# Manta-Network/manta-rs

Measured on AMD Instinct MI355X. Metric: G1 MSM Mscalar/s at 2^20, higher is better.
Workload: dtype u32; 1 GPU; 2^20 BLS12-381 G1 variable-base MSM per GPU, uniform scalars resident in HBM; curve=BLS12-381, log_n=20, window_bits=17, msms_in_flight=3

## Files before the change

include/mantagpu.h:

```cpp
#ifndef MANTAGPU_H
#define MANTAGPU_H
#include <stddef.h>
#include <stdint.h>

#ifdef __cplusplus
extern "C" {
#endif

typedef enum { MG_BN254 = 0, MG_BLS12_381 = 1 } mg_curve_t;

enum {
    MG_SUCCESS = 0,
    MG_ERROR_INVALID_ARGUMENT = 1,
    MG_ERROR_HIP = 2,
    MG_ERROR_OUT_OF_MEMORY = 3,
    MG_ERROR_DOMAIN_TOO_LARGE = 4,
    MG_ERROR_STATE = 5,
    MG_ERROR_CHECKSUM = 6
};

typedef struct mg_bases mg_bases;
typedef struct mg_msm_job mg_msm_job;
typedef struct mg_ctx mg_ctx;

int mg_init(int device);
const char *mg_strerror(int status);
const char *mg_last_error(void);
int mg_device_count(int *count);
int mg_malloc(void **dptr, size_t bytes);
int mg_free(void *dptr);
int mg_memcpy_h2d(void *dptr, const void *hptr, size_t bytes);
int mg_memcpy_d2h(void *hptr, const void *dptr, size_t bytes);
int mg_device_synchronize(void);
int mg_host_alloc(void **hptr, size_t bytes);
int mg_host_free(void *hptr);
int mg_set_kernel_timing(int on);
float mg_last_accumulate_ms(void);
float mg_last_accumulate_mhz(void);
int mg_clock_probe(unsigned iters, double *memtime_mhz, double *mad_issue_per_us_per_simd, double *ms);
int mg_last_ntt_ms(float out4[4]);
int mg_last_prove_phases_ms(float out10[10]);
int mg_last_pass_host_ms(float out3[3]);
int mg_hw_queues(int out2[2]);

int mg_bases_create(mg_curve_t curve, int group, const uint64_t *affine_mont, size_t n, int on_device,
                    int precompute_window_bits, mg_bases **out);
int mg_bases_create_sharded(mg_curve_t curve, int group, const uint64_t *affine_mont, size_t n, const int *devices,
                            int n_devices, int precompute_window_bits, mg_bases **out);
int mg_bases_num_shards(const mg_bases *bases);
int mg_bases_shard(const mg_bases *bases, int shard, int *device, size_t *lo, size_t *hi);
void mg_bases_destroy(mg_bases *bases);
size_t mg_bases_device_bytes(const mg_bases *bases);
int mg_msm(const mg_bases *bases, const uint64_t *scalars_canonical, size_t n, uint64_t *out_affine_mont);
#define MG_SCALARS_MONT 1
#define MG_SCALARS_SPARSE 2
int mg_msm_launch(const mg_bases *bases, const uint64_t *d_scalars, size_t n, int scalar_flags, int window_bits,
                  mg_msm_job **job);
int mg_msm_launch_sharded(const mg_bases *bases, const uint64_t *const *d_scalars_per_shard, int scalar_flags,
                          int window_bits, mg_msm_job **job);
int mg_msm_finish(mg_msm_job *job, uint64_t *out_affine_mont);
int mg_msm_result_to_device(mg_msm_job *job, uint64_t *d_out_xyzz, void *stream);
size_t mg_xyzz_limbs(mg_curve_t curve, int group);
int mg_xyzz_sum(mg_curve_t curve, int group, const uint64_t *xyzz, size_t n, uint64_t *out_affine_mont);
int mg_points_sum(mg_curve_t curve, int group, const uint64_t *affine_mont, size_t n, uint64_t *out_affine_mont);
int mg_fixed_base_mul(mg_curve_t curve, int group, const uint64_t *base_affine_mont, const uint64_t *d_scalars,
                      size_t n, uint64_t *d_out_affine_mont);
#define MG_EC_ADD_MIXED 0
#define MG_EC_ADD 1
#define MG_EC_DOUBLE 2
#define MG_EC_MUL 3
#define MG_EC_SUB_MIXED 4
#define MG_EC_MUL_FIXED 5
int mg_ec_elementwise(mg_curve_t curve, int group, int op, const uint64_t *a_affine, const uint64_t *b, size_t n,
                      uint64_t *out_affine);
#define MG_FIELD_ADD 0
#define MG_FIELD_SUB 1
#define MG_FIELD_MUL 2
#define MG_FIELD_SQR 3
#define MG_FIELD_NEG 4
#define MG_FIELD_FROM_CANONICAL 5
#define MG_FIELD_TO_CANONICAL 6
#define MG_FIELD_INV 7
int mg_field_op(int field, int op, int repr, int lazy_a, int lazy_b, const uint64_t *a, const uint64_t *b, size_t n,
                uint64_t *out);
#define MG_FPR_MUL 0
#define MG_FPR_SQR 1
#define MG_FPR_MUL_ADD 2
#define MG_FPR_SUB2_6 3
#define MG_FPR_SUB2_12 4
int mg_fpr_raw_op(int field, int op, int coding, const uint32_t *a, const uint32_t *b, const uint32_t *c, const uint32_t *d,
                  size_t n, uint32_t *out);
int mg_fpr_column_plan(int field, int kind, uint32_t *flush, uint64_t *peak, int *cols, int *limb_bits, int *flushed_routines);
int mg_msm_digits(mg_curve_t curve, const uint64_t *scalars, size_t batch, size_t n_scalars, int scalar_flags, int window_bits,
                  int table_mode, size_t n, const uint32_t *map, size_t n_sets, size_t set_len, int compact, uint32_t *keys,
                  uint32_t *vals, uint32_t *count, uint32_t layout[4]);
int mg_sort_pairs(const uint32_t *keys, const uint32_t *vals, size_t n, int end_bit, const uint32_t *count, uint32_t lowmask,
                  uint32_t inv_from, uint32_t *keys_out, uint32_t *vals_out);
int mg_group_ntt(mg_curve_t curve, int group, const uint64_t *points_affine, unsigned log_n, int inverse, uint64_t *out_affine);
int mg_point_serialize(mg_curve_t curve, int group, const uint64_t *affine_mont, int compressed, uint8_t *out);

int mg_ntt(mg_curve_t curve, uint64_t *data_mont, unsigned log_n, int inverse, int coset);
int mg_ntt_device(mg_curve_t curve, uint64_t *d_data_mont, unsigned log_n, int inverse, int coset);

typedef struct {
    uint64_t n_vars;
    uint64_t n_inputs;
    uint64_t h_len;
    const uint64_t *alpha_g1, *beta_g1, *delta_g1;
    const uint64_t *beta_g2, *delta_g2;
    const uint64_t *a_query;
    const uint64_t *b_g1_query;
    const uint64_t *b_g2_query;
    const uint64_t *h_query;
    const uint64_t *l_query;
} mg_pk_view;

typedef struct {
    const uint32_t *row_ptr;
    const uint32_t *col;
    const uint64_t *val;
    uint64_t nnz;
} mg_csr;

typedef struct mg_pk_out {
    uint64_t *alpha_g1, *beta_g1, *delta_g1;
    uint64_t *beta_g2, *gamma_g2, *delta_g2;
    uint64_t *gamma_abc_g1;
    uint64_t *a_query, *b_g1_query, *b_g2_query, *h_query, *l_query;
} mg_pk_out;
int mg_groth16_setup(mg_curve_t curve, const mg_csr *a, const mg_csr *b, const mg_csr *c, uint64_t num_constraints,
                     uint64_t n_vars, uint64_t n_inputs, const uint64_t *toxic_mont ,
                     const uint64_t *g1_generator, const uint64_t *g2_generator, const mg_pk_out *out);

int mg_qap_columns(mg_curve_t curve, int group, size_t n_terms, const uint64_t *const *bases_affine,
                   const mg_csr *const *mats, uint64_t m, uint64_t n_cols, uint32_t entries_per_lane,
                   uint64_t *out_affine);

typedef struct {
    uint64_t n_g1, n_g2;
    const uint64_t *tau_powers_g1, *tau_powers_g2, *alpha_tau_powers_g1, *beta_tau_powers_g1, *beta_g2;
} mg_kzg_view;

int mg_mpc_initialize(mg_curve_t curve, const mg_kzg_view *powers, const mg_csr *a, const mg_csr *b, const mg_csr *c,
                      uint64_t num_constraints, uint64_t n_vars, uint64_t n_inputs, uint64_t h_len,
                      const uint64_t *g1_generator, const uint64_t *g2_generator, const mg_pk_out *out);

int mg_ctx_create(mg_curve_t curve, const mg_pk_view *pk, mg_ctx **out);
#define MG_EXCHANGE_HOST 0u
#define MG_EXCHANGE_RCCL 1u
typedef struct mg_tuning {
    uint32_t struct_size;
    int32_t graph_mode;
    int32_t graph_mode_batch;
    int32_t prove_streams;
    int32_t linear_chains;
    int32_t coalesce_inflight;
    int32_t coalesce_gather_us;
    int32_t batch_inflight;
    int32_t queue_aware;
    int32_t msm_dedicated_queues;
    int32_t window_bits_narrow;
    int32_t window_bits_wide;
    int32_t window_bits_h;
    int32_t window_bits_g2;
    int64_t full_table_bytes;
} mg_tuning;
int mg_tuning_init(mg_tuning *t);
int mg_get_tuning(mg_tuning *t);
int mg_set_tuning(const mg_tuning *t);
const char *const *mg_tuning_env_names(void);

typedef struct mg_ctx_opts {
    uint32_t struct_size;
    uint32_t exchange;
    int64_t full_table_bytes;
    const int *devices;
    int32_t n_devices;
    int32_t shard, n_shards;
    uint32_t task_mask;
    const mg_tuning *tuning;
} mg_ctx_opts;
int mg_ctx_opts_init(mg_ctx_opts *opts);
int mg_ctx_create_ex(mg_curve_t curve, const mg_pk_view *pk, const mg_ctx_opts *opts , mg_ctx **out);
int mg_ctx_create_from_bytes_ex(mg_curve_t curve, const uint8_t *bytes, size_t len, const uint8_t *checksum32,
                                const mg_ctx_opts *opts, mg_ctx **out);
int mg_ctx_create_sharded(mg_curve_t curve, const mg_pk_view *pk, const int *devices, int n_devices, mg_ctx **out);
int mg_ctx_create_from_bytes_sharded(mg_curve_t curve, const uint8_t *bytes, size_t len, const int *devices,
                                     int n_devices, mg_ctx **out);
int mg_ctx_create_shard(mg_curve_t curve, const mg_pk_view *pk, int shard, int n_shards, mg_ctx **out);
#define MG_TASK_A 1u
#define MG_TASK_B_G1 2u
#define MG_TASK_B_G2 4u
#define MG_TASK_L 8u
#define MG_TASK_H 16u
int mg_ctx_create_task(mg_curve_t curve, const mg_pk_view *pk, unsigned task_mask, mg_ctx **out);
typedef struct mg_partials_job mg_partials_job;
size_t mg_partials_slot_limbs(const mg_ctx *ctx);
int mg_groth16_partials_launch(const mg_ctx *ctx, uint64_t k, const uint64_t *z_mont, uint64_t *d_out, void *stream,
                               mg_partials_job **job);
int mg_groth16_partials_finish(mg_partials_job *job);
int mg_groth16_assemble(const mg_ctx *ctx, uint64_t k, int n_parts, const uint64_t *parts, const uint64_t *r_mont,
                        const uint64_t *s_mont, uint8_t *proofs_out);
int mg_ctx_create_from_bytes(mg_curve_t curve, const uint8_t *bytes, size_t len, mg_ctx **out);
int mg_ctx_create_from_bytes_checked(mg_curve_t curve, const uint8_t *bytes, size_t len, const uint8_t checksum[32],
                                     mg_ctx **out);
int mg_blake3(const uint8_t *data, size_t len, uint8_t out32[32]);
int mg_blake2s256(const uint8_t *data, size_t len, uint8_t out32[32]);
int mg_blake2s(const uint8_t *data, size_t len, size_t out_len, uint8_t *out);
int mg_aes256_gcm(const uint8_t key[32], const uint8_t nonce[12], const uint8_t *in, size_t len, int decrypt, uint8_t *out,
                  int *ok);
int mg_ctx_set_r1cs(mg_ctx *ctx, const mg_csr *a, const mg_csr *b, const mg_csr *c, uint64_t num_constraints);
int mg_groth16_prove(const mg_ctx *ctx, const uint64_t *z_mont, const uint64_t r_mont[4], const uint64_t s_mont[4],
                     uint8_t *proof_out);
int mg_groth16_prove_batch(const mg_ctx *ctx, uint64_t k, const uint64_t *z_mont, const uint64_t *r_mont,
                           const uint64_t *s_mont, uint8_t *proofs_out);
int mg_witness_map(const mg_ctx *ctx, const uint64_t *z_mont, uint64_t *h_out_mont);
#define MG_R1CS_SATISFIED UINT64_MAX
int mg_ctx_r1cs_check(const mg_ctx *ctx, uint64_t k, const uint64_t *z_mont, uint64_t *first_unsatisfied,
                      uint64_t *n_unsatisfied);
int mg_r1cs_check(mg_curve_t curve, const mg_csr *a, const mg_csr *b, const mg_csr *c, uint64_t num_constraints,
                  uint64_t n_vars, uint64_t k, const uint64_t *z_mont, uint64_t *first_unsatisfied, uint64_t *n_unsatisfied);
uint64_t mg_ctx_domain_size(const mg_ctx *ctx);
int mg_ctx_table_bytes(const mg_ctx *ctx, uint64_t out2[2]);
uint64_t mg_ctx_num_variables(const mg_ctx *ctx);
uint64_t mg_ctx_num_inputs(const mg_ctx *ctx);
int mg_ctx_num_shards(const mg_ctx *ctx);
void mg_ctx_destroy(mg_ctx *ctx);

typedef struct mg_vk mg_vk;
int mg_vk_create(mg_curve_t curve, const uint64_t *alpha_g1, const uint64_t *beta_g2, const uint64_t *gamma_g2,
                 const uint64_t *delta_g2, const uint64_t *gamma_abc_g1, uint64_t n_inputs, mg_vk **out);
int mg_vk_create_from_bytes(mg_curve_t curve, const uint8_t *bytes, size_t len, mg_vk **out);
size_t mg_vk_encoded_size(const mg_vk *vk);
int mg_vk_encode(const mg_vk *vk, uint8_t *out);
int mg_vk_alpha_beta(const mg_vk *vk, uint8_t *out );
uint64_t mg_vk_num_inputs(const mg_vk *vk);
void mg_vk_destroy(mg_vk *vk);
int mg_groth16_verify(const mg_vk *vk, const uint64_t *inputs_mont, const uint64_t *proof_points, int *ok);
int mg_groth16_verify_batch(const mg_vk *vk, uint64_t k, const uint64_t *inputs_mont, const uint64_t *proof_points,
                            const uint64_t *rand128, int *ok);
#define MG_VERIFY_EACH_CHUNK 1024u
int mg_pairing_check_each(mg_curve_t curve, const uint64_t *g1_affine, const uint64_t *g2_affine, size_t group_size,
                          size_t n_groups, uint8_t *ok);
int mg_groth16_verify_each(const mg_vk *vk, uint64_t k, const uint64_t *inputs_mont, const uint64_t *proof_points,
                           uint8_t *ok);
int mg_pairing_check(mg_curve_t curve, const uint64_t *g1_affine, const uint64_t *g2_affine, size_t n, int *ok);
#define MG_PAIRING_MUL12 0
#define MG_PAIRING_SQR12 1
#define MG_PAIRING_CYC_SQR12 2
#define MG_PAIRING_ELL 3
// ... 144 lines not shown
```

manta_rs_amd/api.py:

```python
from __future__ import annotations

import ctypes
import os

import numpy as np

_HERE = os.path.dirname(os.path.abspath(__file__))
LIB_PATH = os.environ.get("MANTA_LIB") or os.path.join(_HERE, "lib", "libmantagpu.so")

BN254, BLS12_381 = 0, 1
FQ_LIMBS = {BN254: 4, BLS12_381: 6}


class MantaGpuError(RuntimeError):

    def __init__(self, status, where=""):
        self.status = status
        detail = LIB.mg_last_error().decode() if status == 2 else ""
        super().__init__(f"{where}: {LIB.mg_strerror(status).decode()} ({status}) {detail}")


def _load():
    if not os.path.exists(LIB_PATH):
        raise ImportError(
            f"{LIB_PATH} not found: the MI355X HIP library is the product and there is no CPU fallback. "
            "Run `python -c 'import __graft_entry__ as g; g.build()'` (or `make -C manta_rs_amd/csrc`).")
    try:
        import torch
    except Exception:
        pass
    lib = ctypes.CDLL(LIB_PATH, mode=ctypes.RTLD_GLOBAL)
    lib.mg_strerror.restype = ctypes.c_char_p
    lib.mg_last_error.restype = ctypes.c_char_p
    lib.mg_bases_device_bytes.restype = ctypes.c_size_t
    lib.mg_ctx_domain_size.restype = ctypes.c_uint64
    lib.mg_ctx_num_variables.restype = ctypes.c_uint64
    lib.mg_ctx_num_inputs.restype = ctypes.c_uint64
    lib.mg_last_accumulate_ms.restype = ctypes.c_float
    lib.mg_last_accumulate_mhz.restype = ctypes.c_float
    lib.mg_vk_encoded_size.restype = ctypes.c_size_t
    lib.mg_vk_num_inputs.restype = ctypes.c_uint64
    lib.mg_xyzz_limbs.restype = ctypes.c_size_t
    lib.mg_partials_slot_limbs.restype = ctypes.c_size_t
    return lib


LIB = _load()
_vp = ctypes.c_void_p
_sz = ctypes.c_size_t

EXPORTS = [
    "mg_init", "mg_strerror", "mg_last_error", "mg_device_count", "mg_malloc", "mg_free", "mg_memcpy_h2d",
    "mg_memcpy_d2h", "mg_device_synchronize", "mg_host_alloc", "mg_host_free", "mg_set_kernel_timing", "mg_last_accumulate_ms", "mg_bases_create", "mg_bases_destroy", "mg_bases_device_bytes",
    "mg_msm", "mg_msm_launch", "mg_msm_finish", "mg_points_sum", "mg_fixed_base_mul", "mg_ec_elementwise", "mg_point_serialize", "mg_ntt",
    "mg_msm_digits", "mg_sort_pairs",
    "mg_ntt_device", "mg_groth16_setup", "mg_ctx_create", "mg_ctx_create_from_bytes", "mg_ctx_set_r1cs", "mg_groth16_prove", "mg_groth16_prove_batch", "mg_witness_map", "mg_ctx_domain_size", "mg_ctx_table_bytes",
    "mg_ctx_destroy", "mg_bases_create_sharded", "mg_bases_num_shards", "mg_bases_shard", "mg_msm_launch_sharded",
    "mg_ctx_create_sharded", "mg_ctx_create_from_bytes_sharded", "mg_ctx_num_variables", "mg_ctx_num_inputs",
    "mg_ctx_num_shards", "mg_field_op", "mg_vk_create", "mg_vk_create_from_bytes", "mg_vk_encoded_size", "mg_vk_encode",
    "mg_vk_alpha_beta", "mg_vk_num_inputs", "mg_vk_destroy", "mg_groth16_verify", "mg_groth16_verify_batch", "mg_pairing_check", "mg_proof_decode", "mg_group_ntt",
    "mg_msm_result_to_device", "mg_xyzz_limbs", "mg_xyzz_sum", "mg_ctx_create_shard", "mg_partials_slot_limbs",
    "mg_groth16_partials_launch", "mg_groth16_partials_finish", "mg_groth16_assemble", "mg_blake3", "mg_ctx_create_from_bytes_checked",
    "mg_last_ntt_ms", "mg_hw_queues", "mg_last_prove_phases_ms", "mg_clock_probe", "mg_last_accumulate_mhz", "mg_ctx_create_task",
    "mg_ctx_opts_init", "mg_ctx_create_ex", "mg_ctx_create_from_bytes_ex", "mg_last_pass_host_ms",
    "mg_tuning_init", "mg_get_tuning", "mg_set_tuning", "mg_tuning_env_names",
    "mg_points_decode", "mg_points_check", "mg_points_encode", "mg_proofs_decode",
    "mg_ppot_points_decode", "mg_ppot_points_encode", "mg_blake2b512",
    "mg_poseidon_create", "mg_poseidon_destroy", "mg_poseidon_permute", "mg_poseidon_hash", "mg_poseidon_hash_device",
    "mg_merkle_tree", "mg_merkle_forest_roots", "mg_merkle_forest_append",
    "mg_edwards_decode", "mg_edwards_encode", "mg_edwards_check", "mg_edwards_mul", "mg_edwards_add",
    "mg_note_cipher_create", "mg_note_cipher_destroy", "mg_notes_encrypt", "mg_notes_decrypt",
    "mg_utxo_model_create", "mg_utxo_model_destroy", "mg_utxos_mint", "mg_utxos_open", "mg_viewing_keys",
    "mg_blake2s256", "mg_schnorr_challenges", "mg_signatures_verify", "mg_signatures_sign",
    "mg_blake2s", "mg_aes256_gcm", "mg_address_partitions", "mg_merkle_shard_indices",
    "mg_light_notes_encrypt", "mg_light_notes_open", "mg_outgoing_notes_encrypt", "mg_outgoing_notes_open",
    "mg_qap_columns", "mg_mpc_initialize", "mg_fpr_raw_op", "mg_fpr_column_plan",
    "mg_pairing_check_each", "mg_groth16_verify_each", "mg_pairing_op",
    "mg_ctx_r1cs_check", "mg_r1cs_check",
]


def _chk(rc, where):
    if rc != 0:
        raise MantaGpuError(rc, where)


def _p(a):
    return None if a is None else a.ctypes.data_as(_vp)


def _u64(a):
    return np.ascontiguousarray(a, dtype=np.uint64)


def _addr(x):
    if x is None:
        return None
    if isinstance(x, ctypes.c_void_p):
        return x
    if hasattr(x, "ptr"):
        return _addr(x.ptr)
    return _vp(int(x))


def init(device=0):
    _chk(LIB.mg_init(int(device)), "mg_init")


def device_count():
    c = ctypes.c_int(0)
    _chk(LIB.mg_device_count(ctypes.byref(c)), "mg_device_count")
    return c.value


def set_kernel_timing(on):
    _chk(LIB.mg_set_kernel_timing(int(bool(on))), "mg_set_kernel_timing")


def last_accumulate_ms():
    return float(LIB.mg_last_accumulate_ms())


def last_accumulate_mhz():
    return float(LIB.mg_last_accumulate_mhz())


def clock_probe(iters=200000):
    a, b, c = ctypes.c_double(0), ctypes.c_double(0), ctypes.c_double(0)
    _chk(LIB.mg_clock_probe(ctypes.c_uint(iters), ctypes.byref(a), ctypes.byref(b), ctypes.byref(c)), "mg_clock_probe")
    return a.value, b.value, c.value


def last_ntt_ms():
    v = (ctypes.c_float * 4)()
    _chk(LIB.mg_last_ntt_ms(v), "mg_last_ntt_ms")
    return [float(x) for x in v]


def hw_queues():
    v = (ctypes.c_int * 2)()
    _chk(LIB.mg_hw_queues(v), "mg_hw_queues")
    return int(v[0]), int(v[1])


def last_prove_phases_ms():
    v = (ctypes.c_float * 10)()
    _chk(LIB.mg_last_prove_phases_ms(v), "mg_last_prove_phases_ms")
    names = ("upload_z", "witness_map", "msm_a", "msm_b_g1", "msm_b_g2", "msm_l", "msm_h", "part_a_upload_to_join", "g2_chain_upload_to_end",
             "host_assembly_after_gpu")
    return {n: round(float(x), 4) for n, x in zip(names, v)}


def last_pass_host_ms():
    v = (ctypes.c_float * 3)()
    _chk(LIB.mg_last_pass_host_ms(v), "mg_last_pass_host_ms")
    return {"enqueue": round(float(v[0]), 4), "wait_gpu": round(float(v[1]), 4), "assemble": round(float(v[2]), 4)}


def synchronize():
    _chk(LIB.mg_device_synchronize(), "mg_device_synchronize")


class PinnedArray:

    def __init__(self, shape, dtype=np.uint64):
        self.nbytes = int(np.prod(shape)) * np.dtype(dtype).itemsize
        ptr = _vp()
        _chk(LIB.mg_host_alloc(ctypes.byref(ptr), _sz(self.nbytes)), "mg_host_alloc")
        self._ptr = ptr
        buf = (ctypes.c_uint8 * self.nbytes).from_address(ptr.value)
        self.array = np.frombuffer(buf, dtype=dtype).reshape(shape)

    @classmethod
    def like(cls, arr):
        arr = np.ascontiguousarray(arr)
        p = cls(arr.shape, arr.dtype)
        p.array[...] = arr
        return p

    def free(self):
        if self._ptr is not None and self._ptr.value:
            self.array = None
            LIB.mg_host_free(self._ptr)
            self._ptr = None

    def __del__(self):
        try:
            self.free()
        except Exception:
            pass


class DeviceBuffer:

    def __init__(self, nbytes):
        self.nbytes = int(nbytes)
        ptr = _vp()
        _chk(LIB.mg_malloc(ctypes.byref(ptr), _sz(self.nbytes)), "mg_malloc")
        self.ptr = ptr

    @classmethod
    def from_numpy(cls, arr):
        arr = np.ascontiguousarray(arr)
        b = cls(arr.nbytes)
        _chk(LIB.mg_memcpy_h2d(b.ptr, _p(arr), _sz(arr.nbytes)), "mg_memcpy_h2d")
        return b

    def to_numpy(self, dtype=np.uint64, shape=None):
# ... 142 lines not shown

def aes256_gcm_decrypt(key: bytes, nonce: bytes, sealed: bytes):
    key, nonce, sealed = bytes(key), bytes(nonce), bytes(sealed)
    if len(key) != 32 or len(nonce) != 12 or len(sealed) < 16:
        raise ValueError("aes256_gcm: a 32-byte key, a 12-byte nonce and at least the 16 bytes of a tag")
    out = ctypes.create_string_buffer(max(1, len(sealed) - 16))
    ok = ctypes.c_int(0)
    _chk(LIB.mg_aes256_gcm(key, nonce, sealed, _sz(len(sealed)), 1, out, ctypes.byref(ok)), "mg_aes256_gcm")
    return out.raw[:len(sealed) - 16], bool(ok.value)


def xyzz_limbs(curve, group) -> int:
    return int(LIB.mg_xyzz_limbs(curve, group))


def xyzz_sum(curve, group, xyzz) -> np.ndarray:
    pts = _u64(xyzz).reshape(-1, xyzz_limbs(curve, group))
    out = np.zeros(affine_limbs(curve, group), dtype=np.uint64)
    _chk(LIB.mg_xyzz_sum(curve, group, _p(pts), _sz(pts.shape[0]), _p(out)), "mg_xyzz_sum")
    return out


def points_sum(curve, group, points):
    pts = _u64(points)
    out = np.zeros(affine_limbs(curve, group), dtype=np.uint64)
    _chk(LIB.mg_points_sum(curve, group, _p(pts), _sz(pts.shape[0]), _p(out)), "mg_points_sum")
    return out


def fixed_base_mul(curve, group, base, d_scalars: DeviceBuffer, n) -> DeviceBuffer:
    out = DeviceBuffer(n * affine_limbs(curve, group) * 8)
    _chk(LIB.mg_fixed_base_mul(curve, group, _p(_u64(base)), d_scalars.ptr, _sz(n), out.ptr), "mg_fixed_base_mul")
    return out


EC_ADD_MIXED, EC_ADD, EC_DOUBLE, EC_MUL, EC_SUB_MIXED, EC_MUL_FIXED = range(6)


def group_ntt(curve, group, points, inverse=False) -> np.ndarray:
    pts = _u64(points)
    n = pts.shape[0]
    lg = n.bit_length() - 1
    assert 1 << lg == n and pts.shape[1] == affine_limbs(curve, group)
    out = np.zeros_like(pts)
    _chk(LIB.mg_group_ntt(curve, group, _p(pts), lg, int(bool(inverse)), _p(out)), "mg_group_ntt")
    return out


def ec_elementwise(curve, group, op, a, b=None) -> np.ndarray:
    a = _u64(a)
    n = a.shape[0]
    out = np.zeros_like(a)
    bb = _p(_u64(b)) if b is not None else None
    _chk(LIB.mg_ec_elementwise(curve, group, op, _p(a), bb, _sz(n), _p(out)), "mg_ec_elementwise")
    return out


FIELD_IDS = {"bn254_fr": 0, "bn254_fq": 1, "bls381_fr": 2, "bls381_fq": 3}
FIELD_OPS = {"add": 0, "sub": 1, "mul": 2, "sqr": 3, "neg": 4, "from_canonical": 5, "to_canonical": 6, "inv": 7}


def field_op(field, op, a, b=None, repr=0, lazy_a=0, lazy_b=0) -> np.ndarray:
    a = _u64(a)
    nl = 6 if field == "bls381_fq" else 4
    assert a.ndim == 2 and a.shape[1] == nl, a.shape
    out = np.zeros_like(a)
    bb = None if b is None else _u64(b)
    assert bb is None or bb.shape == a.shape
    _chk(LIB.mg_field_op(FIELD_IDS[field], FIELD_OPS[op], int(repr), int(lazy_a), int(lazy_b), _p(a), _p(bb), _sz(a.shape[0]),
                         _p(out)), "mg_field_op")
    return out


FPR_OPS = {"mul": 0, "sqr": 1, "mul_add": 2, "sub2_6": 3, "sub2_12": 4}
FPR_LIMBS = {"bn254_fr": (9, 29), "bn254_fq": (9, 29), "bls381_fr": (9, 29), "bls381_fq": (13, 30)}


def fpr_raw_op(field, op, a, b=None, c=None, d=None, chain=False) -> np.ndarray:
    K = FPR_LIMBS[field][0]
    arrs = [None if x is None else np.ascontiguousarray(x, dtype=np.uint32) for x in (a, b, c, d)]
    need = {"sqr": 1, "mul": 2, "sub2_6": 3, "sub2_12": 3, "mul_add": 4}[op]
    for x in arrs[:need]:
        assert x is not None and x.ndim == 2 and x.shape == arrs[0].shape and x.shape[1] == K, (op, None if x is None else x.shape)
    out = np.zeros_like(arrs[0])
    _chk(LIB.mg_fpr_raw_op(FIELD_IDS[field], FPR_OPS[op], int(bool(chain)), _p(arrs[0]), _p(arrs[1]), _p(arrs[2]), _p(arrs[3]),
                           _sz(arrs[0].shape[0]), _p(out)), "mg_fpr_raw_op")
    return out


PAIRING_OPS = {"mul12": 0, "sqr12": 1, "cyc_sqr12": 2, "ell": 3, "frob12_1": 4, "frob12_2": 5, "frob12_3": 6, "conj12": 7, "inv12": 8,
               "exp_by_x": 9, "final_exp": 10, "fq_inv_euclid": 11, "fq_half": 12, "fq2_mul": 13, "fq2_mul_xi": 14, "fq_lincomb": 15}
PAIRING_LINCOMB_OPERANDS = 10


def pairing_op(curve, op, a, b=None, coeffs=None) -> np.ndarray:
    N = 2 * FQ_LIMBS[curve]
    a = np.ascontiguousarray(a, dtype=np.uint32)
    n = a.shape[0]
    if op == "fq_lincomb":
        assert a.shape == (n, PAIRING_LINCOMB_OPERANDS, N), a.shape
        coeffs = np.ascontiguousarray(coeffs, dtype=np.int16)
        assert coeffs.shape == (n, PAIRING_LINCOMB_OPERANDS), coeffs.shape
        out = np.zeros((n, N), dtype=np.uint32)
    else:
        wa = {"fq_inv_euclid": N, "fq_half": N, "fq2_mul": 2 * N, "fq2_mul_xi": 2 * N}.get(op, 12 * N)
        assert a.shape == (n, wa), (op, a.shape)
        coeffs = None
        out = np.zeros_like(a)
    wb = {"mul12": 12 * N, "ell": 6 * N, "fq2_mul": 2 * N}.get(op)
    if wb is not None:
        b = np.ascontiguousarray(b, dtype=np.uint32)
        assert b.shape == (n, wb), (op, b.shape)
    else:
        b = None
    _chk(LIB.mg_pairing_op(curve, PAIRING_OPS[op], _p(a), _p(b), _p(coeffs), _sz(n), _p(out)), "mg_pairing_op")
    return out


def fpr_column_plan(field, kind) -> dict:
    flush, peak = np.zeros(25, dtype=np.uint32), np.zeros(25, dtype=np.uint64)
    cols, lb, fr = ctypes.c_int(0), ctypes.c_int(0), ctypes.c_int(0)
    _chk(LIB.mg_fpr_column_plan(FIELD_IDS[field], FPR_OPS[kind], _p(flush), _p(peak), ctypes.byref(cols), ctypes.byref(lb),
                                ctypes.byref(fr)), "mg_fpr_column_plan")
    return dict(flush=[int(x) for x in flush[:cols.value]], peak=[int(x) for x in peak[:cols.value]], limb_bits=lb.value,
                flushed_routines=bool(fr.value))


def _u32_buffer(a, n, name):
    out = np.zeros(n, dtype=np.uint32) if a is None else np.array(a, dtype=np.uint32).reshape(-1)
    assert out.shape == (n,), "%s: %d elements, expected %d" % (name, out.size, n)
    return out


def msm_digits(curve, scalars, c, n, mont=False, table_mode=0, map=None, n_sets=1, set_len=None, compact=False, keys=None, vals=None):
    sc = _u64(scalars)
    if sc.ndim == 2:
        sc = sc[None]
    assert sc.ndim == 3 and sc.shape[2] == 4, sc.shape
    batch, n_scalars = sc.shape[0], sc.shape[1]
    bits = 254 if curve == BN254 else 255
    W = (bits + c - 1) // c if c > 0 else 0
    size = batch * W * n
    k, v = _u32_buffer(keys, size, "keys"), _u32_buffer(vals, size, "vals")
    mp = None if map is None else np.ascontiguousarray(map, dtype=np.uint32)
    assert mp is None or mp.shape == (n,), mp.shape
    count = ctypes.c_uint32(0)
    layout = (ctypes.c_uint32 * 4)()
    _chk(LIB.mg_msm_digits(curve, _p(sc), _sz(batch), _sz(n_scalars), int(bool(mont)), int(c), int(table_mode), _sz(n), _p(mp), _sz(n_sets),
                           _sz(n if set_len is None else set_len), int(bool(compact)), _p(k), _p(v), ctypes.byref(count) if compact else None,
                           layout), "mg_msm_digits")
    assert layout[0] == W
    return dict(W=int(layout[0]), B=int(layout[1]), seg_keys=int(layout[2]), invalid=int(layout[3]), keys=k, vals=v,
                count=int(count.value) if compact else None)


def sort_pairs(keys, vals, end_bit, count=None, lowmask=0xFFFFFFFF, inv_from=0xFFFFFFFF, keys_out=None, vals_out=None):
    k = np.ascontiguousarray(keys, dtype=np.uint32).reshape(-1)
    v = np.ascontiguousarray(vals, dtype=np.uint32).reshape(-1)
    n = k.shape[0]
    assert v.shape == (n,)
    ko, vo = _u32_buffer(keys_out, n, "keys_out"), _u32_buffer(vals_out, n, "vals_out")
    cnt = None if count is None else ctypes.byref(ctypes.c_uint32(count))
    _chk(LIB.mg_sort_pairs(_p(k), _p(v), _sz(n), int(end_bit), cnt, ctypes.c_uint32(lowmask), ctypes.c_uint32(inv_from), _p(ko), _p(vo)),
         "mg_sort_pairs")
    return ko, vo


def point_serialize(curve, group, point, compressed=True):
    nb = FQ_LIMBS[curve] * 8 * (2 if group == 2 else 1) * (1 if compressed else 2)
    out = ctypes.create_string_buffer(nb)
    _chk(LIB.mg_point_serialize(curve, group, _p(_u64(point)), int(compressed), out), "mg_point_serialize")
    return out.raw


class Radix2EvaluationDomain:

    def __init__(self, curve, size):
        self.curve = curve
        self.log_size = max(0, (int(size) - 1).bit_length())
        self.size = 1 << self.log_size

    def _run(self, data, inverse, coset):
        d = np.array(data, dtype=np.uint64, copy=True)
        assert d.shape == (self.size, 4)
        _chk(LIB.mg_ntt(self.curve, _p(d), self.log_size, int(inverse), int(coset)), "mg_ntt")
        return d

    def fft(self, data):
        return self._run(data, False, False)

    def ifft(self, data):
        return self._run(data, True, False)

    def coset_fft(self, data):
        return self._run(data, False, True)

    def coset_ifft(self, data):
        return self._run(data, True, True)

    def fft_device(self, dbuf: DeviceBuffer, inverse=False, coset=False):
        _chk(LIB.mg_ntt_device(self.curve, dbuf.ptr, self.log_size, int(inverse), int(coset)), "mg_ntt_device")


class _PkView(ctypes.Structure):
    _fields_ = [("n_vars", ctypes.c_uint64), ("n_inputs", ctypes.c_uint64), ("h_len", ctypes.c_uint64)] + [
        (k, _vp) for k in ("alpha_g1", "beta_g1", "delta_g1", "beta_g2", "delta_g2", "a_query", "b_g1_query",
                           "b_g2_query", "h_query", "l_query")]


class _Csr(ctypes.Structure):
    _fields_ = [("row_ptr", _vp), ("col", _vp), ("val", _vp), ("nnz", ctypes.c_uint64)]


class R1CS:

    def __init__(self, curve, A, B, C, num_constraints, num_instance, z):
        self.curve, self.A, self.B, self.C = curve, A, B, C
        self.num_constraints, self.num_instance = int(num_constraints), int(num_instance)
        self.z = _u64(z)

    @classmethod
    def from_circuit(cls, c):
        return cls(c.curve, c.A, c.B, c.C, c.m, c.P, c.z)

    def which_is_unsatisfied(self):
        first, _ = r1cs_check(self.curve, self.A, self.B, self.C, self.num_constraints, self.z.size // 4, self.z)
        return None if first[0] < 0 else int(first[0])

    def is_satisfied(self) -> bool:
        return self.which_is_unsatisfied() is None


class _PkOut(ctypes.Structure):
    _fields_ = [(n, _vp) for n in ("alpha_g1", "beta_g1", "delta_g1", "beta_g2", "gamma_g2", "delta_g2", "gamma_abc_g1",
                                   "a_query", "b_g1_query", "b_g2_query", "h_query", "l_query")]


class ProvingKey:
    pass


def groth16_setup(r1cs: "R1CS", n_vars, toxic_mont, g1_generator, g2_generator) -> ProvingKey:
    curve, m, P, V = r1cs.curve, r1cs.num_constraints, r1cs.num_instance, int(n_vars)
    D = 1
    while D < m + P:
        D <<= 1
    w1, w2 = affine_limbs(curve, 1), affine_limbs(curve, 2)
    pk = ProvingKey()
    pk.curve, pk.V, pk.P, pk.D, pk.h_len = curve, V, P, D, D - 1
    shapes = {"alpha_g1": (1, w1), "beta_g1": (1, w1), "delta_g1": (1, w1), "beta_g2": (1, w2), "gamma_g2": (1, w2),
              "delta_g2": (1, w2), "gamma_abc_g1": (P, w1), "a_query": (V, w1), "b_g1_query": (V, w1),
              "b_g2_query": (V, w2), "h_query": (D - 1, w1), "l_query": (V - P, w1)}
    for k, sh in shapes.items():
        setattr(pk, k, np.zeros(sh, dtype=np.uint64))
    out = _PkOut(*[_p(getattr(pk, k)) for k, _ in _PkOut._fields_])
    ms = []
    for M in (r1cs.A, r1cs.B, r1cs.C):
        rp = np.ascontiguousarray(M.row_ptr, dtype=np.uint32)
        col = np.ascontiguousarray(M.col, dtype=np.uint32)
        val = _u64(M.val)
        ms.append((rp, col, val, _Csr(_p(rp), _p(col), _p(val), len(col))))
    tox = _u64(toxic_mont).reshape(5, 4)
    _chk(LIB.mg_groth16_setup(curve, ctypes.byref(ms[0][3]), ctypes.byref(ms[1][3]), ctypes.byref(ms[2][3]),
                              ctypes.c_uint64(m), ctypes.c_uint64(V), ctypes.c_uint64(P), _p(tox), _p(_u64(g1_generator)),
                              _p(_u64(g2_generator)), ctypes.byref(out)), "mg_groth16_setup")
    return pk


def _csr(M):
    rp = np.ascontiguousarray(M.row_ptr, dtype=np.uint32)
    col = np.ascontiguousarray(M.col, dtype=np.uint32)
    val = _u64(M.val)
    return (rp, col, val), _Csr(_p(rp), _p(col), _p(val), len(col))


R1CS_SATISFIED = (1 << 64) - 1


def _r1cs_verdicts(first, count):
    return np.where(first == np.uint64(R1CS_SATISFIED), np.int64(-1), first.astype(np.int64)), count.astype(np.int64)


def r1cs_check(curve, A, B, C, m, n_vars, zs):
    zs = _u64(zs)
    n_vars = int(n_vars)
    if n_vars > 0 and zs.size % (n_vars * 4):
        raise ValueError(f"assignments hold {zs.size} u64 words, no multiple of n_vars x 4 = {n_vars * 4}")
    k = zs.size // (n_vars * 4) if n_vars > 0 else 0
    keep = [_csr(M) for M in (A, B, C)]
    first, count = np.zeros(k, dtype=np.uint64), np.zeros(k, dtype=np.uint64)
    _chk(LIB.mg_r1cs_check(curve, ctypes.byref(keep[0][1]), ctypes.byref(keep[1][1]), ctypes.byref(keep[2][1]),
                           ctypes.c_uint64(int(m)), ctypes.c_uint64(n_vars), ctypes.c_uint64(k), _p(zs), _p(first), _p(count)),
         "mg_r1cs_check")
    return _r1cs_verdicts(first, count)


def qap_columns(curve, group, bases, mats, n_cols, entries_per_lane=0) -> np.ndarray:
    bases = [_u64(b) for b in bases]
    if len(bases) != len(mats):
        raise ValueError("qap_columns: one basis per matrix")
    m = len(mats[0].row_ptr) - 1 if mats else 0
    for b, M in zip(bases, mats):
        if b.ndim != 2 or b.shape != (m, affine_limbs(curve, group)) or len(M.row_ptr) != m + 1:
            raise ValueError("qap_columns: every basis is [m, limbs] and every matrix has m rows")
    keep = [_csr(M) for M in mats]
    bp = (ctypes.c_void_p * max(len(bases), 1))(*[b.ctypes.data for b in bases])
# ... 936 lines not shown
```

manta_rs_amd/csrc/capi.cpp:

```cpp
#include "../../include/mantagpu.h"
#include "engine.h"
#include "staging.h"
#include "tuning.h"
#include <cstddef>
#include "prover.h"
#include "verify.h"
#include "edwards.h"
#include "utxo.h"
#include "schnorr.h"
#include "light_note.h"
#include <cstring>
#include <new>
#include <vector>

using namespace mg;

struct BasesShard {
    GroupEngine *eng;
    BaseSet *bs;
    int device;
    size_t lo, hi;
};
struct mg_bases {
    std::vector<BasesShard> sh;
// ... 270 lines not shown
        hipSetDevice(j.device);
        int rc2 = j.eng->msm_finish(j.ws, &hp);
        if (rc2) j.eng->msm_abandon(j.ws);
        else e0->hp_add(&total, &hp);
        if (!rc) rc = rc2;
        j.eng->ws_release(j.ws);
        if (j.d_tmp) hipFree(j.d_tmp);
    }
    if (!rc && out_affine && e0) e0->hp_to_affine(&total, (u32 *)out_affine);
    delete job;
    return rc;
    MG_CATCH
}
MG_API int mg_msm_result_to_device(mg_msm_job *job, uint64_t *d_out_xyzz, void *stream) {
    MG_TRY
    if (!job || job->sh.size() != 1 || !d_out_xyzz) return MG_ERROR_INVALID_ARGUMENT;
    JobShard &j = job->sh[0];
    DeviceGuard guard;
    MG_HIP(hipSetDevice(j.device));
    int rc = j.eng->msm_fold_device(j.ws, (u32 *)d_out_xyzz, (size_t)j.eng->xyzz_words());
    if (rc) return rc;
    hipStream_t ms = msm_stream_of(j.ws);
    MG_HIP(hipEventRecord(j.ws->done, ms));
    if ((hipStream_t)stream != ms) MG_HIP(hipStreamWaitEvent((hipStream_t)stream, j.ws->done, 0));
    return MG_SUCCESS;
    MG_CATCH
}
MG_API size_t mg_xyzz_limbs(mg_curve_t curve, int group) {
    GroupEngine *e = get_engine((int)curve, group);
    return e ? (size_t)e->xyzz_words() / 2 : 0;
}
MG_API int mg_xyzz_sum(mg_curve_t curve, int group, const uint64_t *xyzz, size_t n, uint64_t *out_affine) {
    MG_TRY
    GroupEngine *e = get_engine((int)curve, group);
    if (!e || !xyzz || !out_affine) return MG_ERROR_INVALID_ARGUMENT;
    HostPoint acc, t;
    e->hp_set_inf(&acc);
    for (size_t i = 0; i < n; ++i) {
        e->hp_from_xyzz(&t, (const u32 *)xyzz + i * (size_t)e->xyzz_words());
        e->hp_add(&acc, &t);
    }
    e->hp_to_affine(&acc, (u32 *)out_affine);
    return MG_SUCCESS;
    MG_CATCH
}
MG_API int mg_msm(const mg_bases *b, const uint64_t *scalars, size_t n, uint64_t *out_affine) {
    MG_TRY
    if (!b || !scalars || !out_affine || b->sh.empty()) return MG_ERROR_INVALID_ARGUMENT;
    if (n > b->n) n = b->n;
    if (n == 0) {
        std::memset(out_affine, 0, (size_t)b->sh[0].eng->affine_words() * 4);
        return MG_SUCCESS;
    }
    mg_msm_job *job = nullptr;
    int rc = launch_shards(b, nullptr, scalars, n, 0, 0, &job);
    if (!rc) rc = mg_msm_finish(job, out_affine);
    return rc;
    MG_CATCH
}
MG_API int mg_points_sum(mg_curve_t curve, int group, const uint64_t *affine, size_t n, uint64_t *out_affine) {
    MG_TRY
    GroupEngine *e = get_engine((int)curve, group);
    if (!e || !affine || !out_affine) return MG_ERROR_INVALID_ARGUMENT;
    HostPoint acc, t;
    e->hp_set_inf(&acc);
    const u32 *w = (const u32 *)affine;
    for (size_t i = 0; i < n; ++i) {
        e->hp_from_affine(&t, w + i * (size_t)e->affine_words());
        e->hp_add(&acc, &t);
    }
    e->hp_to_affine(&acc, (u32 *)out_affine);
    return MG_SUCCESS;
    MG_CATCH
}
MG_API int mg_fixed_base_mul(mg_curve_t curve, int group, const uint64_t *base_affine, const uint64_t *d_scalars,
                             size_t n, uint64_t *d_out_affine) {
    MG_TRY
    GroupEngine *e = get_engine((int)curve, group);
    if (!e || !base_affine || !d_scalars || !d_out_affine || n == 0) return MG_ERROR_INVALID_ARGUMENT;
    return e->fixed_base_mul((const u32 *)base_affine, (const u32 *)d_scalars, n, (u32 *)d_out_affine, nullptr);
    MG_CATCH
}
MG_API int mg_ec_elementwise(mg_curve_t curve, int group, int op, const uint64_t *a_affine, const uint64_t *b,
                             size_t n, uint64_t *out_affine) {
    MG_TRY
    GroupEngine *e = get_engine((int)curve, group);
    if (!e) return MG_ERROR_INVALID_ARGUMENT;
    return e->ec_elementwise(op, (const u32 *)a_affine, (const u32 *)b, n, (u32 *)out_affine);
    MG_CATCH
}
MG_API int mg_group_ntt(mg_curve_t curve, int group, const uint64_t *points_affine, unsigned log_n, int inverse,
                        uint64_t *out_affine) {
    MG_TRY
    GroupEngine *e = get_engine((int)curve, group);
    FrEngine *fr = get_ntt_engine((int)curve);
    if (!e || !fr || !points_affine || !out_affine) return MG_ERROR_INVALID_ARGUMENT;
    const u32 *tw = nullptr;
    u64 ninv[4];
    int rc = fr->domain_twiddles(log_n, inverse != 0, &tw, ninv);
    if (rc) return rc;
    return e->group_ntt((const u32 *)points_affine, log_n, tw, inverse ? (const u32 *)ninv : nullptr, (u32 *)out_affine);
    MG_CATCH
}
MG_API int mg_point_serialize(mg_curve_t curve, int group, const uint64_t *affine, int compressed, uint8_t *out) {
    MG_TRY
    GroupEngine *e = get_engine((int)curve, group);
    if (!e || !affine || !out) return MG_ERROR_INVALID_ARGUMENT;
    HostPoint p;
    e->hp_from_affine(&p, (const u32 *)affine);
    e->hp_serialize(&p, out, compressed != 0);
    return MG_SUCCESS;
    MG_CATCH
}

namespace mg {
int field_op(int field, int op, int repr, int lazy_a, int lazy_b, const u32 *a, const u32 *b, size_t n, u32 *out);
}
MG_API int mg_field_op(int field, int op, int repr, int lazy_a, int lazy_b, const uint64_t *a, const uint64_t *b, size_t n,
                       uint64_t *out) {
    MG_TRY
    return field_op(field, op, repr, lazy_a, lazy_b, (const u32 *)a, (const u32 *)b, n, (u32 *)out);
    MG_CATCH
}

namespace mg {
int fpr_raw_op(int field, int op, int coding, const u32 *a, const u32 *b, const u32 *c, const u32 *d, size_t n, u32 *out);
int fpr_column_plan_host(int field, int kind, u32 *flush, u64 *peak, int *cols, int *limb_bits, int *flushed_routines);
}
MG_API int mg_fpr_raw_op(int field, int op, int coding, const uint32_t *a, const uint32_t *b, const uint32_t *c, const uint32_t *d, size_t n,
                         uint32_t *out) {
    MG_TRY
    return fpr_raw_op(field, op, coding, a, b, c, d, n, out);
    MG_CATCH
}
MG_API int mg_fpr_column_plan(int field, int kind, uint32_t *flush, uint64_t *peak, int *cols, int *limb_bits, int *flushed_routines) {
    MG_TRY
    return fpr_column_plan_host(field, kind, flush, peak, cols, limb_bits, flushed_routines);
    MG_CATCH
}

MG_API int mg_msm_digits(mg_curve_t curve, const uint64_t *scalars, size_t batch, size_t n_scalars, int scalar_flags, int window_bits,
                         int table_mode, size_t n, const uint32_t *map, size_t n_sets, size_t set_len, int compact, uint32_t *keys,
                         uint32_t *vals, uint32_t *count, uint32_t layout[4]) {
    MG_TRY
    GroupEngine *e = get_engine((int)curve, 1);
    const size_t lim = (size_t)1 << 31;
    if (!e || batch >= lim || n_scalars >= lim || n >= lim || n_sets >= lim || set_len >= lim || (scalar_flags & ~MG_SCALARS_MONT))
        return MG_ERROR_INVALID_ARGUMENT;
    const MsmDigitsCall c{(const u32 *)scalars, (u32)batch, (u32)n_scalars, (scalar_flags & MG_SCALARS_MONT) ? SCALARS_MONT : SCALARS_CANONICAL,
                          window_bits, table_mode, (u32)n, map, (u32)n_sets, (u32)set_len, compact != 0, keys, vals, count, layout};
    return e->msm_digits(c);
    MG_CATCH
}
MG_API int mg_sort_pairs(const uint32_t *keys, const uint32_t *vals, size_t n, int end_bit, const uint32_t *count, uint32_t lowmask,
                         uint32_t inv_from, uint32_t *keys_out, uint32_t *vals_out) {
    MG_TRY
    if (!keys || !vals || !keys_out || !vals_out || end_bit < 1 || end_bit > 32 || n >= ((size_t)1 << 32) || (count && *count > n))
        return MG_ERROR_INVALID_ARGUMENT;
    if (n == 0) return MG_SUCCESS;
    hipStream_t s = setup_stream();
    if (!s) return MG_ERROR_OUT_OF_MEMORY;
    const size_t pb = n * 4, tb = sort_pairs_temp_bytes(n);
    DevBlock m;
    if (const int rc = m.alloc({pb, pb, pb, pb, tb, count ? 4u : 0u}, "mg_sort_pairs")) return rc;
    const void *const src[5] = {keys, vals, keys_out, vals_out, count};
    hipError_t e = hipSuccess;
    for (int i = 0; i < 5 && e == hipSuccess; ++i)
        if (src[i]) e = hipMemcpyAsync(m.dev(i < 4 ? i : 5), src[i], i < 4 ? pb : 4, hipMemcpyHostToDevice, s);
    int rc = MG_OK;
    if (e == hipSuccess)
        rc = sort_pairs(m.dev<u32>(0), m.dev<u32>(2), m.dev<u32>(1), m.dev<u32>(3), n, end_bit, m.dev(4), tb, s, m.dev<u32>(5), lowmask, inv_from);
    if (e == hipSuccess && !rc) e = hipMemcpyAsync(keys_out, m.dev(2), pb, hipMemcpyDeviceToHost, s);
    if (e == hipSuccess && !rc) e = hipMemcpyAsync(vals_out, m.dev(3), pb, hipMemcpyDeviceToHost, s);
    const hipError_t e2 = hipStreamSynchronize(s);
    if (e == hipSuccess) e = e2;
    return rc ? rc : e == hipSuccess ? MG_SUCCESS : hip_status(e, "mg_sort_pairs");
    MG_CATCH
}

MG_API int mg_ntt_device(mg_curve_t curve, uint64_t *d_data, unsigned log_n, int inverse, int coset) {
    MG_TRY
    if (!d_data) return MG_ERROR_INVALID_ARGUMENT;
    NttEngine *n = get_ntt_engine((int)curve);
    if (!n) return MG_ERROR_INVALID_ARGUMENT;
    int rc = n->transform((u32 *)d_data, log_n, inverse != 0, coset != 0, setup_stream());
    if (rc) return rc;
    MG_HIP(setup_sync());
    return MG_SUCCESS;
    MG_CATCH
}
MG_API int mg_ntt(mg_curve_t curve, uint64_t *data, unsigned log_n, int inverse, int coset) {
    MG_TRY
    if (!data || log_n > 32) return MG_ERROR_INVALID_ARGUMENT;
    const size_t bytes = ((size_t)1 << log_n) * 32;
    DevBlock m;
    int rc = m.alloc({bytes}, "mg_ntt");
    if (rc) return rc;
    void *d = m.dev(0);
    if (memcpy_sync(d, data, bytes, hipMemcpyHostToDevice) != hipSuccess) rc = MG_ERROR_HIP;
    if (!rc) rc = mg_ntt_device(curve, (uint64_t *)d, log_n, inverse, coset);
    if (!rc && memcpy_sync(data, d, bytes, hipMemcpyDeviceToHost) != hipSuccess) rc = MG_ERROR_HIP;
    return rc;
    MG_CATCH
}

struct mg_ctx {
    Prover *p;
};
MG_API int mg_ctx_create(mg_curve_t curve, const mg_pk_view *pk, mg_ctx **out) {
    MG_TRY
    if (!pk || !out) return MG_ERROR_INVALID_ARGUMENT;
    Prover *p = nullptr;
    int rc = prover_create((int)curve, pk, &p);
    if (rc) return rc;
    *out = new mg_ctx{p};
    return MG_SUCCESS;
    MG_CATCH
}
MG_API int mg_ctx_create_sharded(mg_curve_t curve, const mg_pk_view *pk, const int *devices, int n_devices, mg_ctx **out) {
    MG_TRY
    if (!pk || !out || !devices) return MG_ERROR_INVALID_ARGUMENT;
    Prover *p = nullptr;
    int rc = prover_create_sharded((int)curve, pk, devices, n_devices, &p);
    if (rc) return rc;
    *out = new mg_ctx{p};
    return MG_SUCCESS;
    MG_CATCH
}
MG_API int mg_ctx_create_shard(mg_curve_t curve, const mg_pk_view *pk, int shard, int n_shards, mg_ctx **out) {
    MG_TRY
    if (!out || shard < 0 || n_shards < 1) return MG_ERROR_INVALID_ARGUMENT;
    Prover *p = nullptr;
    int rc = prover_create_shard((int)curve, pk, (u32)shard, (u32)n_shards, &p);
    if (rc) return rc;
    *out = new mg_ctx{p};
    return MG_SUCCESS;
    MG_CATCH
}
MG_API int mg_ctx_create_task(mg_curve_t curve, const mg_pk_view *pk, unsigned task_mask, mg_ctx **out) {
    MG_TRY
    if (!out) return MG_ERROR_INVALID_ARGUMENT;
    Prover *p = nullptr;
    int rc = prover_create_task((int)curve, pk, (u32)task_mask, &p);
    if (rc) return rc;
    *out = new mg_ctx{p};
    return MG_SUCCESS;
    MG_CATCH
}
static_assert(sizeof(mg_tuning) == sizeof(Tuning) && offsetof(mg_tuning, full_table_bytes) == offsetof(Tuning, full_table_bytes) &&
                  offsetof(mg_tuning, window_bits_g2) == offsetof(Tuning, window_bits_g2),
              "mg_tuning (mantagpu.h) and mg::Tuning (tuning.h) are the same struct");
static int tuning_from_abi(const mg_tuning *in, Tuning &t) {
    if (!in || in->struct_size < 8 || in->struct_size > 4096) return MG_ERROR_INVALID_ARGUMENT;
    t = tuning();
    std::memcpy(&t, in, std::min<size_t>(in->struct_size, sizeof(t)));
    return normalize_tuning(t) == MG_OK ? MG_SUCCESS : MG_ERROR_INVALID_ARGUMENT;
}
MG_API int mg_tuning_init(mg_tuning *t) {
    if (!t) return MG_ERROR_INVALID_ARGUMENT;
    const Tuning d = tuning_defaults();
    std::memcpy(t, &d, sizeof(d));
    return MG_SUCCESS;
}
MG_API int mg_get_tuning(mg_tuning *t) {
    MG_TRY
    if (!t) return MG_ERROR_INVALID_ARGUMENT;
    const Tuning d = tuning();
    std::memcpy(t, &d, sizeof(d));
    return MG_SUCCESS;
    MG_CATCH
}
MG_API int mg_set_tuning(const mg_tuning *t) {
    MG_TRY
    Tuning v;
    const int rc = tuning_from_abi(t, v);
    if (rc) return rc;
    return set_tuning(v) == MG_OK ? MG_SUCCESS : MG_ERROR_INVALID_ARGUMENT;
    MG_CATCH
}
MG_API const char *const *mg_tuning_env_names(void) { return tuning_env_names(); }
static int opts_from_abi(const mg_ctx_opts *in, ProverOptions &o, Tuning &tn) {
    if (!in) return MG_SUCCESS;
    mg_ctx_opts t;
    mg_ctx_opts_init(&t);
    if (in->struct_size < 8 || in->struct_size > 4096) return MG_ERROR_INVALID_ARGUMENT;
    std::memcpy(&t, in, std::min<size_t>(in->struct_size, sizeof(t)));
    if (t.n_devices < 0 || (t.n_devices > 0 && !t.devices) || t.shard < 0 || t.n_shards < 0) return MG_ERROR_INVALID_ARGUMENT;
    o.devices = t.n_devices > 0 ? t.devices : nullptr;
    o.n_devices = t.n_devices;
    o.shard = (u32)t.shard;
    o.n_shards = t.n_shards > 0 ? (u32)t.n_shards : 1;
    o.task_mask = t.task_mask ? t.task_mask : 0x1f;
    o.full_table_bytes = t.full_table_bytes;
    o.exchange = (int)t.exchange;
    if (t.tuning) {
        const int rc = tuning_from_abi(t.tuning, tn);
        if (rc) return rc;
        o.tuning = &tn;
    }
    return MG_SUCCESS;
}
MG_API int mg_ctx_opts_init(mg_ctx_opts *o) {
    if (!o) return MG_ERROR_INVALID_ARGUMENT;
    std::memset(o, 0, sizeof(*o));
    o->struct_size = (uint32_t)sizeof(*o);
    o->exchange = MG_EXCHANGE_HOST;
// ... 575 lines not shown
```

manta_rs_amd/csrc/engine.h:

```cpp
#pragma once
#include <hip/hip_runtime.h>
#include "status.h"
#include <shared_mutex>
#include <atomic>
#include <cstddef>
#include <cstdint>
#include <mutex>
#include <vector>

namespace mg {

typedef uint32_t u32;
typedef uint64_t u64;

#ifdef MG_NO_PRIO
#define MG_PRIO_HIGH() ((void)0)
#else
#define MG_PRIO_HIGH() __builtin_amdgcn_s_setprio(3)
#endif
#define MG_PRIO_FOR(F) MG_PRIO_HIGH()

void set_last_hip_error(hipError_t e, const char *expr, const char *file, int line);
inline int hip_status(hipError_t e, const char *what, const char *file = __builtin_FILE(), int line = __builtin_LINE()) {
    set_last_hip_error(e, what, file, line);
    return e == hipErrorOutOfMemory ? MG_ERR_OOM : MG_ERR_HIP;
}
#define MG_HIP(expr)                                                                                              \
    do {                                                                                                          \
        hipError_t e_ = (expr);                                                                                   \
        if (e_ != hipSuccess) return mg::hip_status(e_, #expr);                                                   \
    } while (0)
void set_last_error_text(const char *text);
void set_kernel_timing(bool on);
bool kernel_timing();
struct LastTimes {
    float accumulate_ms = 0.f;
    float accumulate_mhz = 0.f;
    float ntt_ms[4] = {};
    float pass_host_ms[3] = {};
    float prove_ms[10] = {};
};
LastTimes &last_times();
constexpr int MAX_DEVICES = 16;
int current_device();
std::shared_mutex &capture_mutex();
struct HeavyOp {
    HeavyOp();
    ~HeavyOp();
    HeavyOp(const HeavyOp &) = delete;
    HeavyOp &operator=(const HeavyOp &) = delete;
};
hipStream_t setup_stream();
inline hipError_t memcpy_sync(void *dst, const void *src, size_t bytes, hipMemcpyKind kind) {
    hipStream_t s = setup_stream();
    if (!s) return hipErrorOutOfMemory;
    const hipError_t e = hipMemcpyAsync(dst, src, bytes, kind, s);
    return e == hipSuccess ? hipStreamSynchronize(s) : e;
}
inline hipError_t setup_sync() {
    hipStream_t s = setup_stream();
    return s ? hipStreamSynchronize(s) : hipErrorOutOfMemory;
}
inline int sync_status(hipStream_t s, hipError_t e, const char *what, const char *file = __builtin_FILE(), int line = __builtin_LINE()) {
    const hipError_t e2 = hipStreamSynchronize(s);
    if (e == hipSuccess) e = e2;
    return e == hipSuccess ? MG_OK : hip_status(e, what, file, line);
}
hipStream_t stream_pool_get();
void stream_pool_put(hipStream_t s);
hipStream_t stream_pool_get_normal();
void stream_pool_put_normal(hipStream_t s);
struct GraphClient {
    GraphClient();
    ~GraphClient();
    GraphClient(const GraphClient &) = delete;
    GraphClient &operator=(const GraphClient &) = delete;
};
int graph_clients_alive();
hipStream_t stream_pool_get_dedicated();
void stream_pool_put_dedicated(hipStream_t s);
struct StreamSet {
    hipStream_t main = nullptr, g2 = nullptr, z3 = nullptr;
    int id = -1, dev = 0;
    bool z3_high = false;
};
bool stream_sets_ready();
int stream_queue_counts(int *normal, int *high);
bool stream_set_acquire(StreamSet &s, bool z3_high);
void stream_set_release(StreamSet &s);
int streams_share_queue(hipStream_t a, hipStream_t b, unsigned *mem, unsigned *token_counter);
const char *last_error_string();

struct DeviceScope {
    int prev = 0;
    bool switched = false;
    explicit DeviceScope(int dev) {
        if (hipGetDevice(&prev) == hipSuccess && prev != dev) switched = hipSetDevice(dev) == hipSuccess;
    }
    ~DeviceScope() {
        if (switched) hipSetDevice(prev);
    }
    DeviceScope(const DeviceScope &) = delete;
    DeviceScope &operator=(const DeviceScope &) = delete;
};

struct DeviceGuard {
    int prev = 0;
    DeviceGuard() { hipGetDevice(&prev); }
    ~DeviceGuard() { hipSetDevice(prev); }
    DeviceGuard(const DeviceGuard &) = delete;
    DeviceGuard &operator=(const DeviceGuard &) = delete;
};

struct DevBuf {
    void *p = nullptr;
    size_t cap = 0;
    int reserve(size_t bytes);
    void release();
    template <class T> T *as() const { return (T *)p; }
};

enum { SCALARS_CANONICAL = 0, SCALARS_MONT = 1, SCALARS_WORK = 2 };

struct MsmPlan {
    int c = 0;
    int W = 0;
    u32 B = 0;
    int Wb = 0;
    bool precomp = false;
    bool full = false;
    u32 L = 0;
};

struct BaseSet {
    int curve = 0, group = 1;
    int device = 0;
    size_t n = 0;
    size_t n_orig = 0;
    u32 *d_map = nullptr;
    u32 *d_pts = nullptr;
    int pre_c = 0, pre_W = 0;
    bool full = false;
    u32 n_sets = 1;
    size_t set_len = 0;
    static constexpr u32 MAX_SETS = 4;
    u32 set_first[MAX_SETS + 1] = {};
    size_t bytes = 0;
};

enum MsmTailKind : u32 { TAIL_WINDOW_SUMS = 0, TAIL_X_SUMS = 1, TAIL_TWO_LEVELS = 2 };
struct MsmTail {
    static constexpr int MAX_EXTRA = 8;
    MsmTailKind kind = TAIL_WINDOW_SUMS;
    u32 T1 = 0, nP = 0, segs = 0;
    u32 tail_shift = 0, n_extra = 0, extra_shift[MAX_EXTRA] = {};
    size_t extra_off_pts = 0;
    const u32 *d_tail = nullptr;
};

struct MsmWorkspace {
    DevBuf keys_in, keys_out, vals_in, vals_out, sort_tmp, buckets, pkeys[2], ppts[2], redA, redS, misc;
    DevBuf count;
    DevBuf front, extra;
    DevBuf folded;
    unsigned long long *h_clk = nullptr;
    DevBuf scratch;
    void *h_stage = nullptr;
    size_t h_stage_cap = 0;
    hipStream_t stream = nullptr;
    hipStream_t run_on = nullptr;
    hipStream_t solo = nullptr;
    bool use_solo = false;
    hipStream_t side_stream = nullptr;
    hipEvent_t side_fork = nullptr, side_join = nullptr;
    hipEvent_t done = nullptr;
    hipEvent_t t0 = nullptr, t1 = nullptr;
    bool timed = false;
    bool in_graph_slot = false;
    bool capturing = false;
    bool notify = false;
    u32 *h_flag = nullptr;
    u32 *d_token = nullptr;
    float accumulate_ms = 0.f;
    MsmPlan plan;
    MsmTail tail;
    u32 batch = 1;
    int pending = 0;
    int device = 0;
    ~MsmWorkspace();
};

inline hipStream_t msm_stream_of(const MsmWorkspace *ws) {
    return ws->run_on ? ws->run_on : (ws->use_solo && ws->solo ? ws->solo : ws->stream);
}

struct MsmDigitsCall {
    const u32 *scalars;
    u32 batch, n_scalars;
    int scalar_mode, c, table_mode;
    u32 n;
    const u32 *map;
    u32 n_sets, set_len;
    bool compact;
    u32 *keys, *vals;
    u32 *count;
    u32 *layout;
};

struct QapEntries {
    const u32 *col;
    const u32 *src;
    const u64 *val;
    size_t n;
};

struct HostPoint {
    u64 w[4 * 12];
};

class GroupEngine {
  public:
    virtual ~GroupEngine() {}
    virtual int curve() const = 0;
    virtual int group() const = 0;
    virtual int affine_words() const = 0;
    virtual int xyzz_words() const = 0;
    virtual int scalar_bits() const = 0;
    virtual int base_record_bytes() const = 0;

    virtual int bases_create(const u32 *pts, size_t n, bool src_on_device, int precompute_c, BaseSet **out,
                             bool drop_infinity = false, u32 n_sets = 1) = 0;
    virtual void bases_destroy(BaseSet *) = 0;

    virtual MsmPlan plan_for(const BaseSet *bs, size_t n, int c_override, u32 batch = 1) const = 0;
    virtual int msm_launch(const BaseSet *bs, const u32 *d_scalars, size_t n, int scalar_mode, int c_override,
                           MsmWorkspace *ws, u32 batch = 1, size_t scalar_stride_words = 0, bool sparse = false) = 0;
    virtual int msm_finish(MsmWorkspace *ws, HostPoint *out, bool already_synced = false) = 0;

    virtual int msm_fold_device(MsmWorkspace *ws, u32 *d_out, size_t out_stride_words, hipStream_t on = nullptr) = 0;
    virtual int msm_digits(const MsmDigitsCall &c) = 0;

    virtual void hp_set_inf(HostPoint *p) const = 0;
    virtual void hp_from_affine(HostPoint *p, const u32 *affine_words) const = 0;
    virtual void hp_from_xyzz(HostPoint *p, const u32 *xyzz_words) const = 0;
    virtual void hp_add(HostPoint *acc, const HostPoint *o) const = 0;
    virtual void hp_neg(HostPoint *p) const = 0;
    virtual void hp_mul(HostPoint *p, const u64 *k4) const = 0;
    virtual void hp_mul2(const HostPoint *p, const u64 *k1, const HostPoint *q, const u64 *k2, HostPoint *out) const = 0;
    virtual void *hp_table_create(const HostPoint *base) const = 0;
    virtual void hp_table_mul(const void *table, const u64 *k4, HostPoint *out) const = 0;
    virtual void hp_table_free(void *table) const = 0;
    virtual void hp_to_affine(const HostPoint *p, u32 *affine_words) const = 0;
    virtual void hp_serialize(const HostPoint *p, unsigned char *out, bool compressed) const = 0;
    virtual int point_bytes(bool compressed) const = 0;

    virtual int fixed_base_mul(const u32 *base_affine_host, const u32 *d_scalars, size_t n, u32 *d_out_affine,
                               hipStream_t s) = 0;
    virtual int ec_elementwise(int op, const u32 *a_host, const u32 *b_host, size_t n, u32 *out_affine_host) = 0;
    virtual int ec_mul_xyzz_begin(const u32 *a_affine_host, const u32 *k_canonical_host, size_t n, MsmWorkspace *ws,
                                  const u32 *glv_beta_std = nullptr) = 0;
    virtual const u32 *ec_mul_xyzz_device(MsmWorkspace *ws, size_t n, bool glv = false) const = 0;
    virtual int group_ntt(const u32 *in_affine_host, unsigned lg, const u32 *d_twiddles_mont, const u32 *n_inv_canonical,
                          u32 *out_affine_host) = 0;
    virtual int group_ntt_device(const u32 *d_in_affine, unsigned lg, const u32 *d_twiddles_mont, const u32 *n_inv_canonical,
                                 u32 *d_out_affine) = 0;
    virtual int sub_device(const u32 *d_a_affine, const u32 *d_b_affine, size_t n, u32 *d_out_affine) = 0;
    virtual int qap_columns(const u32 *d_bases_affine, size_t n_bases, const QapEntries &entries, u64 n_cols, u32 entries_per_lane,
                            u32 *out_affine_host) = 0;
    virtual void scalar_one_mont(u64 out[4]) const = 0;
    virtual u64 qap_max_columns() const = 0;

    MsmWorkspace *ws_acquire();
    void ws_release(MsmWorkspace *);
    static void msm_abandon(MsmWorkspace *ws) {
        hipStreamSynchronize(msm_stream_of(ws));
        if (ws->side_stream) hipStreamSynchronize(ws->side_stream);
        ws->pending = 0;
    }

    static constexpr size_t MAX_IDLE_WS = 24;

  protected:
    std::mutex ws_mu_;
    std::vector<MsmWorkspace *> ws_free_;
};

GroupEngine *make_engine_bn254_g1();
GroupEngine *make_engine_bn254_g2();
GroupEngine *make_engine_bls381_g1();
GroupEngine *make_engine_bls381_g2();
GroupEngine *get_engine(int curve, int group);

size_t sort_pairs_temp_bytes(size_t n);
bool sort_pairs_takes_device_count(int end_bit);
int sort_pairs(const u32 *keys_in, u32 *keys_out, const u32 *vals_in, u32 *vals_out, size_t n, int end_bit,
               void *tmp, size_t tmp_bytes, hipStream_t s, const u32 *d_count = nullptr, u32 lowmask = 0xffffffffu,
               u32 inv_from = 0xffffffffu);

}
```

manta_rs_amd/csrc/msm_digits.h:

```cpp
#pragma once
#include "msm_common.h"

namespace mg {

template <class FrC>
__global__ __launch_bounds__(1024) void digits_kernel(const u32 *__restrict__ scalars, u32 n, int c, int W, u32 B,
                                                     int precomp, u32 tstride, int mont, u32 invalid,
                                                     u32 *__restrict__ keys, u32 *__restrict__ vals,
                                                     const u32 *__restrict__ map, u32 n_scalars,
                                                     size_t scalar_stride, u32 seg_keys, u32 *__restrict__ count,
                                                     u32 n_sets = 1, u32 set_len = 0, u32 i_first = 0) {
    MG_PRIO_HIGH();
    const u32 i = i_first + blockIdx.x * blockDim.x + threadIdx.x;
    scalars += (size_t)blockIdx.y * scalar_stride;
    u32 src = (i < n) ? (map ? map[i] : i) : 0xffffffffu;
    u32 set = 0;
    if (n_sets > 1 && i < n) {
        set = src / set_len;
        src -= set * set_len;
    }
    const u32 key0 = (blockIdx.y * n_sets + set) * seg_keys;
    const bool have = i < n && src < n_scalars;
    u32 s[8] = {0, 0, 0, 0, 0, 0, 0, 0};
    if (have && mont == 2) {
        typedef FpR<FrC> R;
        const Fp<FrC> f = R::load(scalars + (size_t)src * R::K).to_canonical();
#pragma unroll
        for (int j = 0; j < 8; ++j) s[j] = f.v[j];
    } else if (have) {
        const uint4 *p = reinterpret_cast<const uint4 *>(scalars + (size_t)src * 8);
        uint4 a = p[0], b = p[1];
        s[0] = a.x, s[1] = a.y, s[2] = a.z, s[3] = a.w, s[4] = b.x, s[5] = b.y, s[6] = b.z, s[7] = b.w;
        if (mont) {
            Fp<FrC> f;
#pragma unroll
            for (int j = 0; j < 8; ++j) f.v[j] = s[j];
            f = Fp<FrC>::from_mont(f);
#pragma unroll
            for (int j = 0; j < 8; ++j) s[j] = f.v[j];
        }
    }
    for (int it = 0; it < 6; ++it) {
        u32 t[8], bw = 0;
#pragma unroll
        for (int j = 0; j < 8; ++j) {
            const u64 d = (u64)s[j] - FrC::P[j] - bw;
            t[j] = (u32)d;
            bw = (u32)(d >> 63);
        }
        if (!__any(!bw)) break;
        if (!bw) {
#pragma unroll
            for (int j = 0; j < 8; ++j) s[j] = t[j];
        }
    }
    u32 flip = 0;
    {
        u32 t[8], bw = 0;
#pragma unroll
        for (int j = 0; j < 8; ++j) {
            const u64 d = (u64)FrC::P[j] - s[j] - bw;
            t[j] = (u32)d;
            bw = (u32)(d >> 63);
        }
        bool lt = false;
#pragma unroll
        for (int j = 0; j < 8; ++j) lt = t[j] != s[j] ? t[j] < s[j] : lt;
        if (!bw && lt) {
            flip = 1;
#pragma unroll
            for (int j = 0; j < 8; ++j) s[j] = t[j];
        }
    }
    const u32 mask = (1u << c) - 1;
    auto next_digit = [&](u32 (&t)[8], u32 &carry, u32 &neg) -> u32 {
        u32 d = (t[0] & mask) + carry;
#pragma unroll
        for (int j = 0; j < 7; ++j) t[j] = __funnelshift_r(t[j], t[j + 1], c);
        t[7] >>= c;
        neg = d > B;
        carry = neg;
        return neg ? (1u << c) - d : d;
    };
    if (!count) {
        if (i >= n) return;
        keys += (size_t)blockIdx.y * W * n;
        vals += (size_t)blockIdx.y * W * n;
        u32 carry = 0, neg;
        for (int w = 0; w < W; ++w) {
            const u32 d = next_digit(s, carry, neg);
            const size_t o = (size_t)w * n + i;
            keys[o] = d ? key0 + (precomp == 2 ? 0u : precomp ? (d - 1) : ((u32)w * B + d - 1)) : invalid;
            vals[o] = d ? ((precomp == 2 ? ((u32)w * tstride + i) * B + (d - 1) : precomp ? ((u32)w * tstride + i) : i) | ((neg ^ flip) << 31)) : 0;
        }
        return;
    }
    const int lane = threadIdx.x & 63;
    u32 total = 0;
    {
        u32 t[8], carry = 0, neg;
#pragma unroll
        for (int j = 0; j < 8; ++j) t[j] = s[j];
        for (int w = 0; w < W; ++w) total += (u32)__popcll(__ballot(next_digit(t, carry, neg) != 0));
    }
    __shared__ u32 wave_tot[16], block_base;
    const int wv = threadIdx.x >> 6, nwv = blockDim.x >> 6;
    if (lane == 0) wave_tot[wv] = total;
    __syncthreads();
    if (threadIdx.x == 0) {
        u32 t = 0;
        for (int q = 0; q < nwv; ++q) t += wave_tot[q];
        block_base = t ? atomicAdd(count, t) : 0;
    }
    __syncthreads();
    u32 base = block_base;
    for (int q = 0; q < wv; ++q) base += wave_tot[q];
    const unsigned long long lt = (1ull << lane) - 1ull;
    u32 carry = 0, neg;
    for (int w = 0; w < W; ++w) {
        const u32 d = next_digit(s, carry, neg);
        const unsigned long long m = __ballot(d != 0);
        if (d) {
            const u32 o = base + (u32)__popcll(m & lt);
            keys[o] = key0 + (precomp == 2 ? 0u : precomp ? (d - 1) : ((u32)w * B + d - 1));
            vals[o] = (precomp == 2 ? ((u32)w * tstride + i) * B + (d - 1) : precomp ? ((u32)w * tstride + i) : i) | ((neg ^ flip) << 31);
        }
        base += (u32)__popcll(m);
    }
}

}
```

manta_rs_amd/csrc/msm_engine.h:

```cpp
#pragma once
#include "group_ops.h"
#include "msm_digits.h"
#include "msm_accumulate.h"
#include "msm_reduce.h"
#include "qap_columns.h"

namespace mg {


static __global__ __launch_bounds__(256) void stage_and_notify_kernel(const u32 *__restrict__ src0, u32 *__restrict__ dst0, u32 n0,
                                                                      const u32 *__restrict__ src1, u32 *__restrict__ dst1, u32 n1,
                                                                      u32 *__restrict__ flag) {
    for (u32 i = threadIdx.x; i < n0; i += 256) dst0[i] = src0[i];
    for (u32 i = threadIdx.x; i < n1; i += 256) dst1[i] = src1[i];
    __threadfence_system();
    __syncthreads();
    if (threadIdx.x == 0 && flag) {
        __atomic_store_n(flag, 1u, __ATOMIC_RELEASE);
        __threadfence_system();
    }
}
struct ZeroRanges {
    u32 *p[3];
    u32 n[3];
};
template <class F> __global__ __launch_bounds__(256) void zero_ranges(ZeroRanges r) {
    const u32 stride = gridDim.x * 256u, i0 = blockIdx.x * 256u + threadIdx.x;
#pragma unroll
    for (int t = 0; t < 3; ++t)
        for (u32 i = i0; i < r.n[t]; i += stride) r.p[t][i] = 0u;
}

static int ab_knob_in(const char *name, int lo, int hi, int dflt) {
    const int v = ab_knob(name, dflt);
    return v < lo ? lo : (v > hi ? hi : v);
}
struct MsmKnobs {
    int msm_L = ab_knob("MANTA_MSM_L", 0);
    int acc_round_waves = ab_knob("MANTA_ACC_ROUND_WAVES", -1);
    int coop_tiles = ab_knob("MANTA_COOP_TILES", 64);
    u32 coop_waves = (u32)ab_knob("MANTA_COOP_WAVES", 512);
    u32 merge_g = [](int v) { return (u32)(v >= 1 && v <= 64 ? v : 0); }(ab_knob("MANTA_MERGE_G", 0));
    int lgS0 = ab_knob_in("MANTA_RED_S0", 1, 8, 2), lgS = ab_knob_in("MANTA_RED_S", -1, 8, -1), lgSP = ab_knob_in("MANTA_RED_SP", 1, 8, 3);
    u32 min_items = (u32)ab_knob_in("MANTA_RED_MIN", 128, 1 << 30, 16384);
    u32 min_items_batch = (u32)ab_knob_in("MANTA_RED_MIN_BATCH", 128, 1 << 30, ab_knob("MANTA_RED_MIN", -1) >= 0 ? (int)min_items : 2048);
    bool side = ab_knob_in("MANTA_RED_SIDE", 0, 1, 1) != 0;
    bool sort_low = ab_knob("MANTA_SORT_LOW", 1) != 0;
    int acc_single = ab_knob("MANTA_ACC_SINGLE", 1);
    u32 digits_threads = [](int v) { return (u32)(v == 256 || v == 512 || v == 1024 ? v : 256); }(ab_knob("MANTA_DIGITS_THREADS", 0));
    bool z3_sort = ab_knob("MANTA_Z3_SORT", 0) != 0;
};
static const MsmKnobs &msm_knobs() {
    static const MsmKnobs k;
    return k;
}

template <class Curve, int CURVE_ID, int GROUP> class GroupEngineT : public GroupOpsT<Curve, CURVE_ID, GROUP> {
  public:
    typedef GroupOpsT<Curve, CURVE_ID, GROUP> Ops;
    using typename Ops::F;
    using typename Ops::FIO;
    using typename Ops::HP;
    using typename Ops::FrC;
    using Ops::AW;
    using Ops::XW;
    using Ops::AW_IO;
    using Ops::XW_IO;
    using Ops::hp;
    static constexpr bool SAME = std::is_same<F, FIO>::value;
    static constexpr int AWS = SAME ? AW : (AW + 7) / 8 * 8;

    int base_record_bytes() const override { return AWS * 4; }

    int bases_create(const u32 *pts_in, size_t n_in, bool src_on_device, int pre_c, BaseSet **out,
                     bool drop_infinity = false, u32 n_sets = 1) override {
        if (!pts_in || !n_in || !out || n_sets == 0 || n_in % n_sets) return MG_ERR_ARG;
        const u32 *pts = pts_in;
        size_t n = n_in;
        std::vector<u32> compact, map;
        if (drop_infinity && !src_on_device && compact_infinity(pts_in, n_in, compact, map)) {
            pts = compact.data();
            n = map.size();
        }
        prime_occupancy();
        BaseSet *bs = new BaseSet();
        struct Guard {
            GroupEngineT *eng;
            BaseSet *bs;
            u32 *win_pts;
            ~Guard() {
                if (win_pts) hipFree(win_pts);
                if (bs) eng->bases_destroy(bs);
            }
        } guard{this, bs, nullptr};
        bs->curve = CURVE_ID;
        bs->group = GROUP;
        bs->device = current_device();
        bs->n = n;
        bs->n_orig = n_in;
        bs->n_sets = n_sets;
        bs->set_len = n_in / n_sets;
        set_query_ranges(bs, map.data(), map.size());
        if (!map.empty()) {
            if (hipMalloc((void **)&bs->d_map, map.size() * 4) != hipSuccess ||
                memcpy_sync(bs->d_map, map.data(), map.size() * 4, hipMemcpyHostToDevice) != hipSuccess)
                return MG_ERR_OOM;
        }
        const bool full = pre_c < 0;
        if (full) pre_c = -pre_c;
        int W = 1;
        if (pre_c > 0) {
            W = windows_of(pre_c);
            bs->pre_c = pre_c;
            bs->pre_W = W;
            bs->full = full;
        }
        const u32 FB = full ? 1u << (pre_c - 1) : 1u;
        if (full && (pre_c < 2 || pre_c > 12 || (size_t)W * n * FB >= ((size_t)1 << 31))) return MG_ERR_ARG;
        bs->bytes = (size_t)W * n * FB * AWS * 4;
        hipError_t e = hipMalloc((void **)&bs->d_pts, bs->bytes);
        u32 *&win_pts = guard.win_pts;
        if (e == hipSuccess && full) e = hipMalloc((void **)&win_pts, (size_t)W * n * AWS * 4);
        if (e != hipSuccess) return hip_failure(e, "hipMalloc(bases)", MG_ERR_OOM);
        u32 *const dst = full ? win_pts : bs->d_pts;
        int rc;
        if ((rc = upload_bases(pts, n, src_on_device, dst)) || (W > 1 && (rc = precompute_windows(dst, n, pre_c, W))) ||
            (full && (rc = expand_full_tables(win_pts, bs->d_pts, n, W, FB))))
            return rc;
        guard.bs = nullptr;
        *out = bs;
        return MG_OK;
    }
    static void set_query_ranges(BaseSet *bs, const u32 *map, size_t map_len) {
        const size_t n = bs->n;
        const u32 n_sets = bs->n_sets;
        if (n_sets <= 1 || n_sets > BaseSet::MAX_SETS) return;
        for (u32 q = 0; q <= n_sets; ++q) {
            const size_t first = (size_t)q * bs->set_len;
            bs->set_first[q] = !map_len ? (u32)(first < n ? first : n) : (u32)(std::lower_bound(map, map + map_len, (u32)first) - map);
        }
        bs->set_first[n_sets] = (u32)n;
    }
    static int windows_of(int c) { return (FrC::BITS + c - 1) / c; }
    static int hip_failure(hipError_t e, const char *what, int rc) { set_last_hip_error(e, what, __FILE__, __LINE__); return rc; }
    static bool compact_infinity(const u32 *pts, size_t n, std::vector<u32> &compact, std::vector<u32> &map) {
        auto finite = [&](size_t i) { return std::any_of(pts + i * AW_IO, pts + (i + 1) * AW_IO, [](u32 x) { return x != 0; }); };
        size_t kept = 0;
        for (size_t i = 0; i < n; ++i) kept += finite(i);
        if (kept == n) return false;
        compact.reserve(kept * AW_IO), map.reserve(kept);
        for (size_t i = 0; i < n; ++i)
            if (finite(i)) compact.insert(compact.end(), pts + i * AW_IO, pts + (i + 1) * AW_IO), map.push_back((u32)i);
        if (!kept) compact.assign(AW_IO, 0u), map.assign(1, 0u);
        return true;
    }
    int upload_bases(const u32 *pts, size_t n, bool src_on_device, u32 *dst) {
        hipError_t e = hipSuccess;
        if (SAME) {
            e = memcpy_sync(dst, pts, n * AW * 4, src_on_device ? hipMemcpyDeviceToDevice : hipMemcpyHostToDevice);
        } else {
            u32 *stage = nullptr;
            const u32 *src = pts;
            if (!src_on_device) {
                e = hipMalloc((void **)&stage, n * AW_IO * 4);
                if (e == hipSuccess) e = memcpy_sync(stage, pts, n * AW_IO * 4, hipMemcpyHostToDevice);
                src = stage;
            }
            if (e == hipSuccess) {
                hipLaunchKernelGGL((bases_to_internal<F>), dim3(cdiv(n, 256)), dim3(256), 0, setup_stream(), src, n, dst, (u32)AWS);
                e = setup_sync();
            }
            if (stage) hipFree(stage);
        }
        return e == hipSuccess ? MG_OK : hip_failure(e, "upload/convert bases", MG_ERR_HIP);
    }
    int precompute_windows(u32 *dst, size_t n, int pre_c, int W) {
        u32 *tmp = nullptr;
        const size_t cnt = (size_t)(W - 1) * n;
        hipError_t e = hipMalloc((void **)&tmp, cnt * XW * 4);
        if (e != hipSuccess) return hip_failure(e, "hipMalloc(precompute tmp)", MG_ERR_OOM);
        hipLaunchKernelGGL((precompute_chain<F>), dim3(cdiv(n, 256)), dim3(256), 0, setup_stream(), dst, (u32)AWS, (u32)n,
                           pre_c, W, tmp);
        xyzz_to_affine_launch<F>(setup_stream(), tmp, cnt, dst + n * AWS, AWS);
        e = setup_sync();
        hipFree(tmp);
        return e == hipSuccess ? MG_OK : hip_failure(e, "precompute kernels", MG_ERR_HIP);
    }
    int expand_full_tables(const u32 *win_pts, u32 *final_pts, size_t n, int W, u32 FB) {
        const size_t pairs = (size_t)W * n;
        size_t slice = ((size_t)512 << 20) / ((size_t)FB * XW * 4);
        if (slice < 256) slice = 256;
        if (slice > pairs) slice = pairs;
        u32 *tmp = nullptr;
        hipError_t e = hipMalloc((void **)&tmp, slice * FB * XW * 4);
        constexpr int KBF = 64;
        for (size_t j0 = 0; e == hipSuccess && j0 < pairs; j0 += slice) {
            const size_t cntp = pairs - j0 < slice ? pairs - j0 : slice;
            hipLaunchKernelGGL((full_table_chain<F>), dim3(cdiv(cntp, 256)), dim3(256), 0, setup_stream(), win_pts, (u32)AWS, j0, (u32)cntp, FB,
                               tmp);
            xyzz_to_affine_launch<F, KBF>(setup_stream(), tmp, cntp * FB, final_pts + j0 * FB * AWS, AWS);
            e = hipGetLastError();
        }
        if (e == hipSuccess) e = setup_sync();
        else (void)setup_sync();
        if (tmp) hipFree(tmp);
        return e == hipSuccess ? MG_OK : hip_status(e, "full-table kernels");
    }
    void bases_destroy(BaseSet *bs) override {
        if (!bs) return;
        if (bs->d_map) hipFree(bs->d_map);
        if (bs->d_pts) hipFree(bs->d_pts);
        delete bs;
    }

    MsmPlan plan_for(const BaseSet *bs, size_t n, int c_override, u32 batch = 1) const override {
        MsmPlan p;
        if (bs->pre_c > 0) {
            p.c = bs->pre_c;
            p.W = bs->pre_W;
            p.precomp = true;
            p.full = bs->full;
            p.Wb = 1;
        } else {
            int lg = 0;
            while (((size_t)1 << lg) < n) ++lg;
            int c = c_override > 0 ? c_override : (lg <= 8 ? 5 : lg <= 12 ? 8 : lg <= 15 ? 10 : lg <= 18 ? 12 : lg <= 19 ? 14 : 16);
            p.c = c;
            p.W = windows_of(c);
            p.Wb = p.W;
        }
        p.B = 1u << (p.c - 1);
        const size_t M = n * (size_t)p.W * batch;
        size_t L;
        if (M < ((size_t)8 << 20)) {
            L = M / (192 * 1024);
            if (L < 6) L = 6;
            if (p.full) L = 3;
        } else {
            const size_t round = 128 * 1024, lmax = batch > 1 ? 96 : 192;
            const size_t rounds = (M + round * lmax - 1) / (round * lmax);
            L = (M + round * rounds - 1) / (round * rounds);
        }
        if (msm_knobs().msm_L > 0) L = (size_t)msm_knobs().msm_L;
        p.L = (u32)L;
        return p;
    }

    u32 acc_round_lanes(bool batched, bool single = false) {
        const int knob = msm_knobs().acc_round_waves;
        if (knob == 0) return 0;
        const int dev = current_device();
        if (dev < 0 || dev >= 64 || !occ_[dev].cus.load(std::memory_order_acquire)) return 0;
        u32 w = single && occ_[dev].blocks_single ? occ_[dev].blocks_single : occ_[dev].blocks;
        if (knob > 0) w = (u32)knob < w ? (u32)knob : w;
        else if (batched && w > 2) w = 2;
        return w * 256u * occ_[dev].cus.load(std::memory_order_relaxed);
    }
    struct Occ {
        u32 blocks = 0, blocks_single = 0;
        std::atomic<u32> cus{0};
    } occ_[64];
    void prime_occupancy() {
        const int dev = current_device();
        if (dev < 0 || dev >= 64 || occ_[dev].cus.load(std::memory_order_acquire)) return;
        int nb = 0, cus = 0;
        if (hipOccupancyMaxActiveBlocksPerMultiprocessor(&nb, accumulate_chunks<F, false>, 256, 0) != hipSuccess ||
            hipDeviceGetAttribute(&cus, hipDeviceAttributeMultiprocessorCount, dev) != hipSuccess || nb < 1 || cus < 1) {
            (void)hipGetLastError();
            return;
        }
        int nbs = 0;
        if (hipFuncSetAttribute(reinterpret_cast<const void *>(&accumulate_single<F>), hipFuncAttributeMaxDynamicSharedMemorySize,
                                (int)AccSingle<F>::LDS_BYTES) != hipSuccess ||
// ... 51 lines not shown
            int lo = 0, hi = 0;
            if (hipDeviceGetStreamPriorityRange(&lo, &hi) != hipSuccess ||
                hipStreamCreateWithPriority(&side_stream_, hipStreamNonBlocking, hi) != hipSuccess)
                side_stream_ = nullptr;
        }
        return side_stream_;
    }
    std::mutex side_mu_;
    hipStream_t side_stream_ = nullptr;

    int msm_launch(const BaseSet *bs, const u32 *d_scalars, size_t n, int scalar_mode, int c_override,
                   MsmWorkspace *ws, u32 batch = 1, size_t scalar_stride_words = 0, bool sparse = false) override {
        if (!bs || !d_scalars || !ws || n == 0 || n > bs->n_orig || batch == 0 || batch > 65535) return MG_ERR_ARG;
        if (bs->curve != CURVE_ID || bs->group != GROUP) return MG_ERR_ARG;
        const u32 nsets = bs->n_sets;
        if (nsets > 1 && n > bs->set_len) return MG_ERR_ARG;
        const size_t n_scalars = n;
        if (bs->d_map || n > bs->n || nsets > 1) n = bs->n;
        Launch r{bs, d_scalars, ws, msm_stream_of(ws), nullptr, n, n_scalars, scalar_stride_words, scalar_mode, batch, nsets, batch > 1,
                 sparse, plan_for(bs, n, c_override, batch)};
        int rc;
        if ((rc = launch_reserve(r))) return rc;
        launch_digits(r);
        if ((rc = launch_sort(r)) || (rc = launch_accumulate(r))) return rc;
        launch_merge(r);
        if ((rc = launch_front_levels(r)) || (rc = launch_scan_tail(r)) || (rc = launch_stage(r))) return rc;
        if (!ws->capturing) MG_HIP(hipEventRecord(ws->done, r.s));
        MG_HIP(hipGetLastError());
        ws->plan = r.pl, ws->tail = r.tail, ws->batch = r.batch;
        ws->pending = 1;
        return MG_OK;
    }

    static int stage_reserve(MsmWorkspace *ws, size_t bytes) {
        if (ws->h_stage_cap >= bytes) return MG_OK;
        if (ws->h_stage) hipHostFree(ws->h_stage);
        ws->h_stage = nullptr;
        ws->h_stage_cap = 0;
        size_t cap = bytes < 65536 ? 65536 : bytes;
        MG_HIP(hipHostMalloc(&ws->h_stage, cap, hipHostMallocDefault));
        ws->h_stage_cap = cap;
        return MG_OK;
    }

    int msm_finish(MsmWorkspace *ws, HostPoint *out, bool already_synced = false) override {
        if (!ws || !ws->pending) return MG_ERR_STATE;
        if (!already_synced) MG_HIP(hipEventSynchronize(ws->done));
        ws->pending = 0;
        if (ws->timed && !already_synced) {
            float ms = 0.f;
            if (hipEventElapsedTime(&ms, ws->t0, ws->t1) == hipSuccess) last_times().accumulate_ms = ms;
            const unsigned long long ck[2] = {((volatile unsigned long long *)ws->h_clk)[0], ((volatile unsigned long long *)ws->h_clk)[1]};
            int khz = 0, dev = 0;
            if (ck[1] && hipGetDevice(&dev) == hipSuccess &&
                hipDeviceGetAttribute(&khz, hipDeviceAttributeWallClockRate, dev) == hipSuccess)
                last_times().accumulate_mhz = (float)((double)ck[0] / (double)ck[1] * (double)khz / 1e3);
        }
        const MsmPlan &pl = ws->plan;
        const MsmTail &t = ws->tail;
        const u32 Wb = (u32)pl.Wb, segs = t.segs, T1 = t.T1, nP = t.nP;
        const u32 *st = (const u32 *)ws->h_stage;
        for (u32 q = 0; q < ws->batch; ++q) {
            HP total = HP::inf();
            for (int w = (int)((q + 1) * Wb) - 1; w >= (int)(q * Wb); --w) {
                HP win;
                if (t.kind == TAIL_WINDOW_SUMS) {
                    win = HP::from_xyzz_words(st + (size_t)w * XW_IO);
                } else if (t.kind == TAIL_X_SUMS) {
                    const HP X = HP::from_xyzz_words(st + ((size_t)w * 2 + 0) * XW_IO);
                    const HP sumS = HP::from_xyzz_words(st + ((size_t)w * 2 + 1) * XW_IO);
                    win = HP::add(sumS, HP::mul_pow2(X, 6));
                } else {
                    const u32 *A1 = st + ((size_t)w * T1) * XW_IO;
                    const u32 *S1 = st + ((size_t)segs * T1 + (size_t)w * T1) * XW_IO;
                    const u32 *P0 = st + ((size_t)segs * 2 * T1 + (size_t)w * nP) * XW_IO;
                    HP sumS = HP::inf(), run = HP::inf(), uA = HP::inf();
                    for (int u = (int)T1 - 1; u >= 0; --u) {
                        sumS = HP::add(sumS, HP::from_xyzz_words(S1 + (size_t)u * XW_IO));
                        if (u >= 1) {
                            run = HP::add(run, HP::from_xyzz_words(A1 + (size_t)u * XW_IO));
                            uA = HP::add(uA, run);
                        }
                    }
                    HP X = HP::add(sumS, HP::mul_pow2(uA, 6));
                    HP sumP = HP::inf();
                    for (u32 u = 0; u < nP; ++u) sumP = HP::add(sumP, HP::from_xyzz_words(P0 + (size_t)u * XW_IO));
                    win = HP::add(sumP, HP::mul_pow2(X, 6));
                }
                if (t.tail_shift) win = HP::mul_pow2(win, t.tail_shift);
                for (u32 e = 0; e < t.n_extra; ++e) {
                    const HP x = HP::from_xyzz_words(st + (t.extra_off_pts + (size_t)e * segs + (size_t)w) * XW_IO);
                    win = HP::add(win, t.extra_shift[e] ? HP::mul_pow2(x, t.extra_shift[e]) : x);
                }
                if (w != (int)((q + 1) * Wb) - 1) total = HP::mul_pow2(total, (unsigned)pl.c);
                total = HP::add(total, win);
            }
            hp(out + q) = total;
        }
        return MG_OK;
    }

    int msm_fold_device(MsmWorkspace *ws, u32 *d_out, size_t out_stride_words, hipStream_t on = nullptr) override {
        if (!ws || !ws->pending || !d_out || !ws->tail.d_tail) return MG_ERR_STATE;
        const MsmTail &t = ws->tail;
        if (ws->plan.Wb != 1) return MG_ERR_STATE;
        FoldDesc d{t.d_tail, ws->extra.as<u32>(), t.kind, t.T1, t.nP, t.segs, t.n_extra, t.tail_shift, {}};
        for (u32 e = 0; e < t.n_extra; ++e) d.extra_shift[e] = t.extra_shift[e];
        hipLaunchKernelGGL((fold_windows<F>), dim3(ws->batch), dim3(64), 0, on ? on : msm_stream_of(ws), d, d_out, out_stride_words);
        MG_HIP(hipGetLastError());
        return MG_OK;
    }

    int msm_digits(const MsmDigitsCall &c) override {
        if (!c.scalars || !c.keys || !c.vals || !c.layout || (c.compact && !c.count) || c.n == 0 || c.n_scalars == 0 || c.batch == 0 ||
            c.batch > 65535 || (c.scalar_mode != SCALARS_CANONICAL && c.scalar_mode != SCALARS_MONT) || c.table_mode < 0 ||
            c.table_mode > 2 || c.c < 1 || c.c > 24 || (c.table_mode == 2 && (c.c < 2 || c.c > 12)) || c.n_sets == 0 || c.set_len == 0)
            return MG_ERR_ARG;
        BaseSet bs;
        bs.curve = CURVE_ID, bs.group = GROUP, bs.device = current_device();
        bs.n = c.n, bs.n_orig = (size_t)c.n_sets * c.set_len, bs.n_sets = c.n_sets, bs.set_len = c.set_len;
        if (c.table_mode) bs.pre_c = c.c, bs.pre_W = windows_of(c.c), bs.full = c.table_mode == 2;
        if (bs.n > bs.n_orig || (!c.map && bs.n != bs.n_orig) || c.n_scalars > bs.n_orig || (c.n_sets > 1 && c.n_scalars > c.set_len))
            return MG_ERR_ARG;
        for (size_t i = 0; c.map && i < c.n; ++i)
            if (c.map[i] >= bs.n_orig) return MG_ERR_ARG;
        if (!c.map || std::is_sorted(c.map, c.map + c.n)) set_query_ranges(&bs, c.map, c.map ? c.n : 0);
        Launch r{&bs, nullptr, nullptr, nullptr, nullptr, c.n, c.n_scalars, (size_t)c.n_scalars * 8, c.scalar_mode, c.batch, c.n_sets, c.batch > 1,
                 c.compact, plan_for(&bs, c.n, c.c, c.batch)};
        if (const int rc = key_layout(r)) return rc;
        c.layout[0] = (u32)r.pl.W, c.layout[1] = r.pl.B, c.layout[2] = r.seg_keys, c.layout[3] = r.invalid;
        hipStream_t s = r.s = setup_stream();
        if (!s) return MG_ERR_OOM;
        const size_t sb = (size_t)c.batch * c.n_scalars * 32, pb = r.M * 4;
        DevBlock m;
        if (const int rc = m.alloc({sb, c.map ? (size_t)c.n * 4 : 0, pb, pb, c.compact ? 4u : 0u}, "mg_msm_digits")) return rc;
        u32 *const d_keys = m.dev<u32>(2), *const d_vals = m.dev<u32>(3);
        r.d_scalars = m.dev<u32>(0), bs.d_map = m.dev<u32>(1), r.d_count = m.dev<u32>(4);
        const u32 zero = 0;
        hipError_t e = hipMemcpyAsync(m.dev(0), c.scalars, sb, hipMemcpyHostToDevice, s);
        if (e == hipSuccess && c.map) e = hipMemcpyAsync(bs.d_map, c.map, (size_t)c.n * 4, hipMemcpyHostToDevice, s);
        if (e == hipSuccess) e = hipMemcpyAsync(d_keys, c.keys, pb, hipMemcpyHostToDevice, s);
        if (e == hipSuccess) e = hipMemcpyAsync(d_vals, c.vals, pb, hipMemcpyHostToDevice, s);
        if (e == hipSuccess && c.compact) e = hipMemcpyAsync(r.d_count, &zero, 4, hipMemcpyHostToDevice, s);
        if (e == hipSuccess) {
            enqueue_digits(r, d_keys, d_vals);
            e = hipGetLastError();
        }
        if (e == hipSuccess) e = hipMemcpyAsync(c.keys, d_keys, pb, hipMemcpyDeviceToHost, s);
        if (e == hipSuccess) e = hipMemcpyAsync(c.vals, d_vals, pb, hipMemcpyDeviceToHost, s);
        if (e == hipSuccess && c.compact) e = hipMemcpyAsync(c.count, r.d_count, 4, hipMemcpyDeviceToHost, s);
        const int rc = sync_status(s, e, "mg_msm_digits");
        bs.d_map = nullptr;
        return rc;
    }

    void scalar_one_mont(u64 out[4]) const override {
        const host::HFp<FrC> one = host::HFp<FrC>::one();
        std::memcpy(out, one.v, 32);
    }
    u64 qap_max_columns() const override { return ((u64)1 << 32) / XWM - 2; }
    static u32 qap_entries_per_lane(size_t N) {
        const size_t l = N / (128 * 1024);
        return (u32)(l < 4 ? 4 : l > 64 ? 64 : l);
    }
    int qap_columns(const u32 *d_bases, size_t n_bases, const QapEntries &en, u64 n_cols, u32 entries_per_lane,
                    u32 *out_affine_host) override {
        const size_t N = en.n;
        if (!out_affine_host || n_cols == 0 || n_cols > qap_max_columns() || N >= ((size_t)1 << 31) ||
            (N && (!d_bases || !n_bases || !en.col || !en.src || !en.val)))
            return MG_ERR_ARG;
        for (size_t e = 0; e < N; ++e)
            if (en.col[e] >= n_cols || en.src[e] >= n_bases) return MG_ERR_ARG;
        const size_t out_bytes = (size_t)n_cols * AW_IO * 4;
        if (N == 0) {
            std::memset(out_affine_host, 0, out_bytes);
            return MG_OK;
        }
        hipStream_t st = setup_stream();
        if (!st) return MG_ERR_OOM;
        const u32 L = entries_per_lane ? entries_per_lane : qap_entries_per_lane(N);
        const u32 T = cdiv(N, L), waves1 = cdiv((size_t)2 * T, 64), invalid = (u32)n_cols;
        int end_bit = 1;
        while (end_bit < 32 && ((u64)1 << end_bit) < n_cols) ++end_bit;
        std::vector<u32> ids(N);
        for (size_t e = 0; e < N; ++e) ids[e] = (u32)e;
        const size_t sort_bytes = sort_pairs_temp_bytes(N);
        enum { SRC, VAL, KEYS, IDS, SKEYS, SIDS, SORT, PROD, PK0, PP0, PK1, PP1, SUMS, STD, AFF };
        DevBlock m;
        if (const int rc = m.alloc({N * 4, N * 32, N * 4, N * 4, N * 4, N * 4, sort_bytes, N * XW * 4, (size_t)2 * T * 4,
                                    (size_t)2 * T * XW * 4, (size_t)2 * waves1 * 4, (size_t)2 * waves1 * XW * 4,
                                    (size_t)(n_cols + 1) * XW * 4, (size_t)n_cols * XW_IO * 4, out_bytes},
                                   "qap_columns"))
            return rc;
        std::vector<u32> stage((size_t)n_cols * AW_IO);
        hipError_t e = hipMemcpyAsync(m.dev(SRC), en.src, N * 4, hipMemcpyHostToDevice, st);
        if (e == hipSuccess) e = hipMemcpyAsync(m.dev(VAL), en.val, N * 32, hipMemcpyHostToDevice, st);
        if (e == hipSuccess) e = hipMemcpyAsync(m.dev(KEYS), en.col, N * 4, hipMemcpyHostToDevice, st);
        if (e == hipSuccess) e = hipMemcpyAsync(m.dev(IDS), ids.data(), N * 4, hipMemcpyHostToDevice, st);
        int rc = MG_OK;
        if (e == hipSuccess) {
            u32 *const sums = m.dev<u32>(SUMS);
            ZeroRanges zr{};
            zr.p[0] = sums, zr.n[0] = (u32)((size_t)(n_cols + 1) * XW);
            hipLaunchKernelGGL((zero_ranges<F>), dim3(zr.n[0] > 256u * 1024u ? 1024u : cdiv(zr.n[0], 256)), dim3(256), 0, st, zr);
            rc = sort_pairs(m.dev<u32>(KEYS), m.dev<u32>(SKEYS), m.dev<u32>(IDS), m.dev<u32>(SIDS), N, end_bit, m.dev(SORT), sort_bytes, st);
            if (!rc) {
                hipLaunchKernelGGL((qap_entry_kernel<F, FrC>), dim3(cdiv(N, 256)), dim3(256), 0, st, m.dev<u32>(SIDS), (u32)N, m.dev<u32>(SRC),
                                   m.dev<u32>(VAL), d_bases, m.dev<u32>(PROD));
                hipLaunchKernelGGL((qap_segsum_kernel<F>), dim3(cdiv(T, 256)), dim3(256), 0, st, m.dev<u32>(SKEYS), m.dev<u32>(PROD), (u32)N, L,
                                   invalid, sums, m.dev<u32>(PK0), m.dev<u32>(PP0), T);
                u32 *pk[2] = {m.dev<u32>(PK0), m.dev<u32>(PK1)}, *pp[2] = {m.dev<u32>(PP0), m.dev<u32>(PP1)};
                merge_levels(st, pk, pp, 2 * T, merge_g1(N), invalid, sums, (u32 *)nullptr);
                hipLaunchKernelGGL((group_scale_store_kernel<F>), dim3(cdiv(n_cols, 256)), dim3(256), 0, st, sums, (const u32 *)nullptr,
                                   (size_t)n_cols, m.dev<u32>(STD));
                xyzz_to_affine_launch<FIO>(st, m.dev<u32>(STD), (size_t)n_cols, m.dev<u32>(AFF), AW_IO);
                e = hipGetLastError();
                if (e == hipSuccess) e = hipMemcpyAsync(stage.data(), m.dev(AFF), out_bytes, hipMemcpyDeviceToHost, st);
            }
        }
        const int synced = sync_status(st, e, "qap_columns");
        if (rc || synced) return rc ? rc : synced;
        std::memcpy(out_affine_host, stage.data(), out_bytes);
        return MG_OK;
    }

  private:
    struct Launch {
        const BaseSet *bs;
        const u32 *d_scalars;
        MsmWorkspace *ws;
        hipStream_t s, side;
        size_t n, n_scalars, scalar_stride_words;
        int scalar_mode;
        u32 batch, nsets;
        bool batched_pass, sparse;
        MsmPlan pl;
        size_t M;
        int end_bit;
        u32 KB, seg_keys, nb, invalid, T, sort_mask = 0xffffffffu, sort_inv = 0xffffffffu;
        bool direct, per_query, acc_single;
        u32 *d_count;
        const u32 *skeys, *svals;
        u32 parts;
        const u32 *rin;
        u32 rstride, roff, rn;
        MsmTail tail;
    };

    static int key_layout(Launch &r) {
        const MsmPlan &pl = r.pl;
        r.M = r.n * (size_t)pl.W * r.batch;
        r.KB = pl.full ? 1u : pl.B;
        if (r.M >= (1ull << 31) || (size_t)r.batch * r.nsets * pl.Wb * r.KB >= (1ull << 24)) return MG_ERR_ARG;
        if ((size_t)pl.W * r.bs->n * (pl.full ? pl.B : 1u) >= (1ull << 31)) return MG_ERR_ARG;
        r.seg_keys = (u32)pl.Wb * r.KB;
        r.nb = r.batch * r.nsets * r.seg_keys;
        r.invalid = r.nb;
        return MG_OK;
    }

    int launch_reserve(Launch &r) {
        MsmWorkspace *const ws = r.ws; const MsmPlan &pl = r.pl;
        int rc;
        if ((rc = key_layout(r))) return rc;
        const size_t M = r.M;
        if (pl.full) r.sparse = true;
        const u32 seg_keys = r.seg_keys, nb = r.nb, invalid = r.invalid;
        if ((rc = ws->keys_in.reserve(M * 4)) || (rc = ws->keys_out.reserve(M * 4)) ||
            (rc = ws->vals_in.reserve(M * 4)) || (rc = ws->vals_out.reserve(M * 4)))
            return rc;
        if ((rc = ws->sort_tmp.reserve(sort_pairs_temp_bytes(M))) || (rc = ws->buckets.reserve((size_t)(nb + 1) * XW * 4))) return rc;
        const u32 T = r.T = cdiv(M, pl.L);
        if ((rc = ws->pkeys[0].reserve((size_t)2 * T * 4)) || (rc = ws->ppts[0].reserve((size_t)2 * T * XW * 4)))
            return rc;
        const u32 waves1 = cdiv((size_t)2 * T, 64);
        if ((rc = ws->pkeys[1].reserve((size_t)2 * waves1 * 4)) ||
            (rc = ws->ppts[1].reserve((size_t)2 * waves1 * XW * 4)))
            return rc;

        int end_bit = 1;
        while ((1u << end_bit) <= invalid) ++end_bit;
        int end_bit_real = 1;
        while (nb > 1 && (1u << end_bit_real) <= nb - 1) ++end_bit_real;
        if ((end_bit + 7) / 8 > (end_bit_real + 7) / 8) r.sparse = true;
        if (r.sparse) end_bit = end_bit_real;
        if (msm_knobs().sort_low && !r.sparse && r.batch > 1 && r.nsets == 1 && (seg_keys & (seg_keys - 1)) == 0) {
            int eb = 1;
            while ((1u << eb) <= seg_keys) ++eb;
            if ((eb + 7) / 8 < (end_bit + 7) / 8) r.sort_mask = seg_keys - 1, r.sort_inv = invalid, end_bit = eb;
        }
        r.end_bit = end_bit;
        if (r.sparse && sort_pairs_takes_device_count(end_bit)) {
            if ((rc = ws->count.reserve(256))) return rc;
            r.d_count = ws->count.as<u32>();
        }
#ifdef MG_NO_DIRECT
        r.direct = false;
#else
        r.direct = nb == 1;
#endif
        if (r.direct && ((rc = ws->redA.reserve((size_t)XWM * 4)) || (rc = ws->redS.reserve((size_t)XWM * 4)))) return rc;
        ws->timed = kernel_timing() && !ws->capturing;
        if (ws->timed && !ws->h_clk) MG_HIP(hipHostMalloc((void **)&ws->h_clk, 64, hipHostMallocDefault));
        return MG_OK;
    }
    static constexpr int XWM = XW > XW_IO ? XW : XW_IO;

    void launch_digits(Launch &r) {
        MsmWorkspace *const ws = r.ws; hipStream_t s = r.s;
        ZeroRanges zr{};
        zr.p[0] = r.d_count, zr.n[0] = r.d_count ? 1u : 0u;
        zr.p[1] = r.direct ? ws->redS.as<u32>() : ws->buckets.as<u32>();
        zr.n[1] = r.direct ? (u32)XWM : (u32)((size_t)(r.nb + 1) * XW);
        zr.p[2] = ws->timed ? (u32 *)ws->h_clk : nullptr, zr.n[2] = ws->timed ? 4u : 0u;
        const u32 most = zr.n[1] > 4u ? zr.n[1] : 4u;
        hipLaunchKernelGGL((zero_ranges<F>), dim3(most > 256u * 1024u ? 1024u : cdiv(most, 256)), dim3(256), 0, s, zr);
        enqueue_digits(r, ws->keys_in.as<u32>(), ws->vals_in.as<u32>());
        r.batch *= r.nsets;
    }
    static void enqueue_digits(Launch &r, u32 *keys, u32 *vals) {
        const MsmPlan &pl = r.pl; const BaseSet *const bs = r.bs; hipStream_t s = r.s;
        const u32 dthreads = r.d_count ? msm_knobs().digits_threads : 256u;
        const u32 nsets = r.nsets;
        r.per_query = pl.full && nsets > 1 && nsets <= BaseSet::MAX_SETS && r.batch == 1 && r.d_count && !msm_knobs().z3_sort &&
                      bs->set_first[nsets] == (u32)bs->n;
        if (r.per_query) {
            for (u32 q = 0; q < nsets; ++q) {
                const u32 lo = bs->set_first[q], hi = bs->set_first[q + 1];
                if (hi <= lo) continue;
                hipLaunchKernelGGL((digits_kernel<FrC>), dim3(cdiv(hi - lo, dthreads), 1), dim3(dthreads), 0, s, r.d_scalars, hi, pl.c,
                                   pl.W, pl.B, 2, (u32)bs->n, r.scalar_mode, r.invalid, keys, vals,
                                   (const u32 *)bs->d_map, (u32)r.n_scalars, r.scalar_stride_words, r.seg_keys, r.d_count, nsets,
                                   (u32)bs->set_len, lo);
            }
        } else
            hipLaunchKernelGGL((digits_kernel<FrC>), dim3(cdiv(r.n, dthreads), r.batch), dim3(dthreads), 0, s, r.d_scalars, (u32)r.n,
                               pl.c, pl.W, pl.B, pl.full ? 2 : (pl.precomp ? 1 : 0), (u32)bs->n, r.scalar_mode, r.invalid,
                               keys, vals, (const u32 *)bs->d_map, (u32)r.n_scalars,
                               r.scalar_stride_words, r.seg_keys, r.d_count, nsets, (u32)bs->set_len);
    }

    int launch_sort(Launch &r) {
        MsmWorkspace *const ws = r.ws;
        const bool no_sort = (r.nb == 1 || r.per_query) && r.d_count;
        r.skeys = no_sort ? ws->keys_in.as<u32>() : ws->keys_out.as<u32>();
        r.svals = no_sort ? ws->vals_in.as<u32>() : ws->vals_out.as<u32>();
        return no_sort ? MG_OK
                       : sort_pairs(ws->keys_in.as<u32>(), ws->keys_out.as<u32>(), ws->vals_in.as<u32>(), ws->vals_out.as<u32>(), r.M,
                                    r.end_bit, ws->sort_tmp.p, sort_pairs_temp_bytes(r.M), r.s, r.d_count, r.sort_mask, r.sort_inv);
    }

    int launch_accumulate(Launch &r) {
        MsmWorkspace *const ws = r.ws; const MsmPlan &pl = r.pl; const BaseSet *const bs = r.bs; hipStream_t s = r.s;
        u32 Tl = r.T, adapt = 0;
        u32 Lk = pl.L;
        const bool acc_single_on = ((msm_knobs().acc_single >> (GROUP - 1)) & 1) != 0;
        const int dev_now = current_device();
        const bool acc_single = r.acc_single = r.nb == 1 && r.d_count && acc_single_on && !(kernel_timing() && !ws->capturing) &&
                                               dev_now >= 0 && dev_now < 64 && occ_[dev_now].cus.load(std::memory_order_acquire) &&
                                               occ_[dev_now].blocks_single;
        if (r.d_count) {
            const u32 tgt = acc_round_lanes(r.batched_pass, acc_single);
            if (tgt && Tl > tgt) Tl = tgt, adapt = 1;
            else if (tgt && !r.batched_pass && pl.L > 6) adapt = 1;
            if (adapt && Lk > 6) Lk = 6;
        }
        const u32 M = (u32)r.M, invalid = r.invalid;
        if (ws->timed) MG_HIP(hipEventRecord(ws->t0, s));
#ifdef MG_CALIBRATION
        static const bool gather_only = std::getenv("MANTA_ACC_GATHER_ONLY") != nullptr;
        if (gather_only)
            hipLaunchKernelGGL((gather_only_chunks<F>), dim3(cdiv(r.T, 256)), dim3(256), 0, s, ws->keys_out.as<u32>(),
                               ws->vals_out.as<u32>(), M, pl.L, invalid, bs->d_pts, (u32)AWS, ws->pkeys[0].as<u32>(), r.T,
                               (const u32 *)r.d_count);
        else
#endif
        if (acc_single)
            hipLaunchKernelGGL((accumulate_single<F>), dim3(cdiv(Tl, 256)), dim3(256), AccSingle<F>::LDS_BYTES, s, r.svals, M, Lk, bs->d_pts, (u32)AWS,
                               ws->pkeys[0].as<u32>(), ws->ppts[0].as<u32>(), Tl, (const u32 *)r.d_count, adapt, invalid);
        else
        if (ws->timed)
            hipLaunchKernelGGL((accumulate_chunks<F, true>), dim3(cdiv(Tl, 256)), dim3(256), 0, s, r.skeys,
                               r.svals, M, Lk, invalid, bs->d_pts, (u32)AWS, ws->buckets.as<u32>(),
                               ws->pkeys[0].as<u32>(), ws->ppts[0].as<u32>(), Tl, (const u32 *)r.d_count, ws->h_clk, adapt);
        else
            hipLaunchKernelGGL((accumulate_chunks<F, false>), dim3(cdiv(Tl, 256)), dim3(256), 0, s, r.skeys,
                               r.svals, M, Lk, invalid, bs->d_pts, (u32)AWS, ws->buckets.as<u32>(),
                               ws->pkeys[0].as<u32>(), ws->ppts[0].as<u32>(), Tl, (const u32 *)r.d_count, (unsigned long long *)nullptr, adapt);
        if (ws->timed) MG_HIP(hipEventRecord(ws->t1, s));
        r.parts = acc_single ? cdiv(Tl, 256) : 2 * Tl;
        return MG_OK;
    }

    void launch_merge(Launch &r) {
        MsmWorkspace *const ws = r.ws;
        u32 *pk[2] = {ws->pkeys[0].as<u32>(), ws->pkeys[1].as<u32>()}, *pp[2] = {ws->ppts[0].as<u32>(), ws->ppts[1].as<u32>()};
        merge_levels(r.s, pk, pp, r.parts, r.acc_single ? 2u : merge_g1(r.M), r.invalid, ws->buckets.as<u32>(),
                     r.direct ? ws->redS.as<u32>() : (u32 *)nullptr);
    }
    static void merge_levels(hipStream_t st, u32 *const pkeys[2], u32 *const ppts[2], u32 cnt, u32 G0, u32 invalid, u32 *buckets,
                             u32 *std_final) {
        int src = 0;
        for (int level = 0;; ++level) {
            u32 G = level == 0 ? G0 : 2;
            if (cnt <= 512) G = cnt <= 64 ? 1 : cdiv(cnt, 64);
            const u32 waves = cdiv(cdiv(cnt, G), 64);
            const int fin = waves == 1;
            merge_partials_launch(st, waves, pkeys[src], ppts[src], cnt, G, invalid, fin, buckets, pkeys[1 - src], ppts[1 - src], std_final);
            if (fin) break;
            cnt = 2 * waves;
            src ^= 1;
        }
    }

    int launch_front_levels(Launch &r) {
        MsmWorkspace *const ws = r.ws; const MsmPlan &pl = r.pl; hipStream_t s = r.s; MsmTail &t = r.tail;
        const u32 segs = t.segs = r.batch * (u32)pl.Wb;
        r.rin = ws->buckets.as<u32>(), r.rstride = r.KB, r.roff = 0, r.rn = r.KB;
        const MsmKnobs &rk = msm_knobs();
        const int lgS_eff = rk.lgS >= 0 ? rk.lgS : 3;
        const u32 min_items = r.batched_pass ? rk.min_items_batch : rk.min_items;
        if (lgS_eff <= 0 || r.rn < min_items) return MG_OK;
        hipStreamCaptureStatus cst = hipStreamCaptureStatusNone;
        const bool being_captured = hipStreamIsCapturing(s, &cst) != hipSuccess || cst != hipStreamCaptureStatusNone;
        if (!ws->capturing && !ws->run_on && !ws->in_graph_slot && !being_captured && rk.side) {
            if (!(r.side = engine_side_stream())) return MG_ERR_HIP;
            if (!ws->side_fork) {
                MG_HIP(hipEventCreateWithFlags(&ws->side_fork, hipEventDisableTiming));
                MG_HIP(hipEventCreateWithFlags(&ws->side_join, hipEventDisableTiming));
            }
            ws->side_stream = r.side;
        }
        for (int pass = 0; pass < 2; ++pass) {
            size_t used = 0;
            auto take = [&](size_t pts) {
                u32 *p = pass ? ws->front.as<u32>() + used * XW : nullptr;
                used += pts;
                return p;
            };
            const u32 *in = ws->buckets.as<u32>();
            u32 stride = pl.B, off = 0, n = pl.B, shift = 0, ne = 0;
            while (n >= min_items && ne < (u32)MsmTail::MAX_EXTRA) {
                const int lg = (size_t)segs * n >= ((size_t)1 << 18) ? rk.lgS0 : (rk.lgS < 0 && n >= (1u << 16) ? 4 : lgS_eff);
                const u32 lanes = cdiv(n, 1u << lg);
                u32 *A = take((size_t)segs * lanes), *Sx = take((size_t)segs * lanes);
                if (pass) serial_reduce_launch(s, (size_t)segs * lanes, in, stride, off, n, 1u << lg, lanes, A, Sx);
                hipStream_t ps = r.side ? r.side : s;
                if (pass && r.side) {
                    MG_HIP(hipEventRecord(ws->side_fork, s));
                    MG_HIP(hipStreamWaitEvent(r.side, ws->side_fork, 0));
                }
                const u32 *pin = Sx;
                u32 pcnt = lanes;
                while (pcnt > 64) {
                    int plg = rk.lgSP;
                    while (plg > 1 && (pcnt >> plg) < 32 && pcnt > 64u << 1) --plg;
                    const u32 pl2 = cdiv(pcnt, 1u << plg);
                    u32 *tp = take((size_t)segs * pl2);
                    if (pass) serial_reduce_launch(ps, (size_t)segs * pl2, pin, pcnt, 0u, pcnt, 1u << plg, pl2, tp, (u32 *)nullptr);
                    pin = tp;
                    pcnt = pl2;
                }
                if (pass)
                    tile_reduce_launch(ps, segs, true, pin, pcnt, 0u, pcnt, 1u, ws->extra.as<u32>() + (size_t)ne * segs * XW_IO,
                                       (u32 *)nullptr, 1);
                t.extra_shift[ne++] = shift;
                shift += lg;
                in = A, stride = lanes, off = 1, n = lanes - 1;
            }
            int rc;
            if (pass) r.rin = in, r.rstride = stride, r.roff = off, r.rn = n, t.tail_shift = shift, t.n_extra = ne;
            else if ((rc = ws->front.reserve(used * XW * 4)) || (rc = ws->extra.reserve((size_t)MsmTail::MAX_EXTRA * segs * XW_IO * 4)))
                return rc;
        }
        return MG_OK;
    }

    int launch_scan_tail(Launch &r) {
        MsmWorkspace *const ws = r.ws; hipStream_t s = r.s; MsmTail &t = r.tail;
        const u32 segs = t.segs, T0 = cdiv(r.rn, 64);
        int rc;
        if (r.direct) {
            t.extra_off_pts = segs;
        } else if (T0 == 1) {
            if ((rc = ws->redA.reserve((size_t)segs * XWM * 4)) || (rc = ws->redS.reserve((size_t)segs * XWM * 4))) return rc;
            tile_reduce_launch(s, segs, r.rn > 1, r.rin, r.rstride, r.roff, r.rn, 1u, ws->redA.as<u32>(), ws->redS.as<u32>(), 1);
            t.extra_off_pts = segs;
        } else if (T0 <= 64) {
            if ((rc = ws->redA.reserve((size_t)segs * T0 * XW * 4)) || (rc = ws->redS.reserve((size_t)segs * T0 * XW * 4)) ||
                (rc = ws->misc.reserve((size_t)segs * 2 * XW_IO * 4)))
                return rc;
            tile_reduce_launch(s, segs * T0, true, r.rin, r.rstride, r.roff, r.rn, T0, ws->redA.as<u32>(), ws->redS.as<u32>(), 0);
            reduce_level1_launch(s, segs, ws->redA.as<u32>(), ws->redS.as<u32>(), T0, ws->misc.as<u32>());
            t.kind = TAIL_X_SUMS;
            t.extra_off_pts = (size_t)segs * 2;
        } else {
// ... 45 lines not shown
```

manta_rs_amd/csrc/sort.hip:

```cpp
#include "engine.h"
#include <cstdlib>

namespace mg {

static constexpr int SORT_TILE = 4096;
static constexpr int SORT_ITEMS = 16;

__device__ __forceinline__ u32 sort_key(u32 k, u32 lowmask, u32 inv_from) {
    return (k >= inv_from && lowmask != 0xffffffffu) ? lowmask + 1u : (k & lowmask);
}

__global__ __launch_bounds__(256) void radix_hist(const u32 *__restrict__ keys, u32 M, int shift, u32 ntiles,
                                                  u32 *__restrict__ hist, const u32 *__restrict__ count, u32 lowmask, u32 inv_from) {
    MG_PRIO_HIGH();
    if (count) M = *count;
    if ((size_t)blockIdx.x * SORT_TILE >= M) {
        hist[(size_t)threadIdx.x * ntiles + blockIdx.x] = 0;
        return;
    }
    __shared__ u32 cnt[256];
    cnt[threadIdx.x] = 0;
    __syncthreads();
    const size_t base = (size_t)blockIdx.x * SORT_TILE;
#pragma unroll
    for (int j = 0; j < SORT_ITEMS; ++j) {
        const size_t e = base + (size_t)j * 256 + threadIdx.x;
        if (e < M) atomicAdd(&cnt[(sort_key(keys[e], lowmask, inv_from) >> shift) & 255u], 1u);
    }
    __syncthreads();
    hist[(size_t)threadIdx.x * ntiles + blockIdx.x] = cnt[threadIdx.x];
}

__global__ __launch_bounds__(256) void radix_scan_rows(u32 *__restrict__ hist, u32 ntiles, u32 *__restrict__ totals) {
    MG_PRIO_HIGH();
    __shared__ u32 part[256];
    u32 *row = hist + (size_t)blockIdx.x * ntiles;
    const u32 per = (ntiles + 255) / 256;
    const u32 lo = threadIdx.x * per, hi = lo + per < ntiles ? lo + per : ntiles;
    u32 s = 0;
    for (u32 i = lo; i < hi; ++i) s += row[i];
    part[threadIdx.x] = s;
    __syncthreads();
    for (int d = 1; d < 256; d <<= 1) {
        const u32 v = threadIdx.x >= (u32)d ? part[threadIdx.x - d] : 0;
        __syncthreads();
        part[threadIdx.x] += v;
        __syncthreads();
    }
    u32 run = threadIdx.x ? part[threadIdx.x - 1] : 0;
    for (u32 i = lo; i < hi; ++i) {
        const u32 c = row[i];
        row[i] = run;
        run += c;
    }
    if (threadIdx.x == 255) totals[blockIdx.x] = part[255];
}
__global__ __launch_bounds__(256) void radix_scan_totals(u32 *__restrict__ totals) {
    MG_PRIO_HIGH();
    __shared__ u32 part[256];
    const u32 mine = totals[threadIdx.x];
    part[threadIdx.x] = mine;
    __syncthreads();
    for (int d = 1; d < 256; d <<= 1) {
        const u32 v = threadIdx.x >= (u32)d ? part[threadIdx.x - d] : 0;
        __syncthreads();
        part[threadIdx.x] += v;
        __syncthreads();
    }
    totals[threadIdx.x] = part[threadIdx.x] - mine;
}

#ifndef MG_SCATTER_MASKS
#define MG_SCATTER_MASKS 1
#endif

template <bool IDENT>
__global__ __launch_bounds__(256) void radix_scatter(const u32 *__restrict__ keys_in, const u32 *__restrict__ vals_in,
                                                     u32 *__restrict__ keys_out, u32 *__restrict__ vals_out, u32 M,
                                                     int shift, u32 ntiles, const u32 *__restrict__ hist,
                                                     const u32 *__restrict__ totals, const u32 *__restrict__ count, u32 lowmask,
                                                     u32 inv_from) {
    MG_PRIO_HIGH();
    if (count) M = *count;
    if ((size_t)blockIdx.x * SORT_TILE >= M) return;
    __shared__ u32 wcount[4][256];
    __shared__ u32 gbase[256];
    typedef unsigned long long __attribute__((may_alias)) lane_mask;
    __shared__ __attribute__((aligned(8))) u32 tile[2 * SORT_TILE];
    u32 *const sk = tile, *const sv = tile + SORT_TILE;
    lane_mask *const masks = (lane_mask *)tile;
    constexpr int HALF = SORT_ITEMS / 2;
    const int wave = threadIdx.x >> 6, lane = threadIdx.x & 63;
    const auto digit = [&](u32 key) { return ((IDENT ? key : sort_key(key, lowmask, inv_from)) >> shift) & 255u; };
#pragma unroll
    for (int w = 0; w < 4; ++w) {
        wcount[w][threadIdx.x] = 0;
        if (MG_SCATTER_MASKS) masks[w * 256 + threadIdx.x] = 0;
    }
    __syncthreads();
    const u32 tile0 = blockIdx.x * (u32)SORT_TILE;
    const u32 base = tile0 + (u32)wave * (SORT_ITEMS * 64) + (u32)lane;
    const u32 left = M - tile0 > (u32)SORT_TILE ? (u32)SORT_TILE : M - tile0;
    const u32 mine = (u32)wave * (SORT_ITEMS * 64) + (u32)lane;
    u32 k[SORT_ITEMS], rk2[HALF];
#pragma unroll
    for (int j = 0; j < SORT_ITEMS; ++j) {
        const bool valid = mine + (u32)j * 64 < left;
        k[j] = valid ? keys_in[(size_t)base + (size_t)j * 64] : 0u;
    }
#if MG_SCATTER_MASKS
    lane_mask *const wmask = masks + wave * 256;
    const unsigned long long lane_bit = 1ull << lane;
    unsigned long long none = 0;
    asm volatile("" : "+v"(none));
#pragma unroll
    for (int j = 0; j < SORT_ITEMS; ++j) {
        const bool valid = mine + (u32)j * 64 < left;
        const u32 d = digit(k[j]);
        if (valid) __hip_atomic_fetch_or(&wmask[d], lane_bit, __ATOMIC_RELAXED, __HIP_MEMORY_SCOPE_WAVEFRONT);
        __builtin_amdgcn_fence(__ATOMIC_ACQ_REL, "wavefront");
        __builtin_amdgcn_wave_barrier();
        const unsigned long long peers = __hip_atomic_load(&wmask[d], __ATOMIC_RELAXED, __HIP_MEMORY_SCOPE_WAVEFRONT);
        const u32 before = wcount[wave][d];
        const u32 lo = (u32)peers, hi = (u32)(peers >> 32);
        const u32 rank = __builtin_amdgcn_mbcnt_hi(hi, __builtin_amdgcn_mbcnt_lo(lo, before));
        const bool first = valid && rank == before;
        if (j & 1)
            rk2[j >> 1] |= rank << 16;
        else
            rk2[j >> 1] = rank;
        asm volatile("" : "+v"(rk2[j >> 1]));
        __builtin_amdgcn_fence(__ATOMIC_ACQ_REL, "wavefront");
        __builtin_amdgcn_wave_barrier();
        if (first) {
            wcount[wave][d] = (u32)__builtin_popcount(hi) + ((u32)__builtin_popcount(lo) + before);
            __hip_atomic_store(&wmask[d], none, __ATOMIC_RELAXED, __HIP_MEMORY_SCOPE_WAVEFRONT);
        }
        __builtin_amdgcn_fence(__ATOMIC_ACQ_REL, "wavefront");
        __builtin_amdgcn_wave_barrier();
    }
#else
    const unsigned long long lt_mask = (1ull << lane) - 1ull;
#pragma unroll
    for (int j = 0; j < SORT_ITEMS; ++j) {
        const bool valid = mine + (u32)j * 64 < left;
        const u32 d = digit(k[j]);
        unsigned long long peers = __ballot(valid);
#pragma unroll
        for (int b = 0; b < 8; ++b) {
            const bool bit = (d >> b) & 1u;
            const unsigned long long bb = __ballot(bit);
            peers &= bit ? bb : ~bb;
        }
        const u32 before = wcount[wave][d];
        const u32 r = (u32)__popcll(peers & lt_mask);
        if (j & 1)
            rk2[j >> 1] |= (before + r) << 16;
        else
            rk2[j >> 1] = before + r;
        asm volatile("" : "+v"(rk2[j >> 1]));
        if (valid && r == 0) wcount[wave][d] = before + (u32)__popcll(peers);
    }
#endif
#pragma unroll
    for (int j = 0; j < SORT_ITEMS; ++j) asm volatile("" : "+v"(k[j]));
    u32 v[SORT_ITEMS];
#pragma unroll
    for (int j = 0; j < SORT_ITEMS; ++j) v[j] = mine + (u32)j * 64 < left ? vals_in[(size_t)base + (size_t)j * 64] : 0u;
    __syncthreads();
    {
        const u32 d = threadIdx.x;
        const u32 c0 = wcount[0][d], c1 = wcount[1][d], c2 = wcount[2][d], c3 = wcount[3][d];
        const u32 tot = c0 + c1 + c2 + c3;
        gbase[d] = tot;
        __syncthreads();
        for (int s = 1; s < 256; s <<= 1) {
            const u32 x = d >= (u32)s ? gbase[d - s] : 0;
            __syncthreads();
            gbase[d] += x;
            __syncthreads();
        }
        const u32 loc = gbase[d] - tot;
        __syncthreads();
        wcount[0][d] = loc;
        wcount[1][d] = loc + c0;
        wcount[2][d] = loc + c0 + c1;
        wcount[3][d] = loc + c0 + c1 + c2;
        gbase[d] = hist[(size_t)d * ntiles + blockIdx.x] + totals[d] - loc;
    }
    __syncthreads();
#pragma unroll
    for (int j = 0; j < SORT_ITEMS; ++j) {
        if (mine + (u32)j * 64 < left) {
            const u32 rank = (j & 1) ? rk2[j >> 1] >> 16 : rk2[j >> 1] & 0xffffu;
            const u32 lp = wcount[wave][digit(k[j])] + rank;
            sk[lp] = k[j];
            sv[lp] = v[j];
        }
    }
    __syncthreads();
    for (u32 t = threadIdx.x; t < left; t += 256) {
        const u32 kk = sk[t];
        const u32 pos = gbase[digit(kk)] + t;
        keys_out[pos] = kk;
        vals_out[pos] = sv[t];
    }
}

size_t sort_pairs_temp_bytes(size_t n) {
    const size_t ntiles = (n + SORT_TILE - 1) / SORT_TILE;
    return 2 * n * 4  + 256 * ntiles * 4 + 256 * 4 + 256;
}

bool sort_pairs_takes_device_count(int end_bit) { return end_bit >= 1 && end_bit <= 32; }

int sort_pairs(const u32 *keys_in, u32 *keys_out, const u32 *vals_in, u32 *vals_out, size_t n, int end_bit,
               void *tmp, size_t tmp_bytes, hipStream_t s, const u32 *d_count, u32 lowmask, u32 inv_from) {
    if (n == 0) return MG_OK;
    if (end_bit < 1 || end_bit > 32 || n >= (1ull << 32) || tmp_bytes < sort_pairs_temp_bytes(n)) return MG_ERR_ARG;
    const u32 M = (u32)n;
    const u32 ntiles = (u32)((n + SORT_TILE - 1) / SORT_TILE);
    const int passes = (end_bit + 7) / 8;
    u32 *tk = (u32 *)tmp, *tv = tk + n, *hist = tv + n, *totals = hist + (size_t)256 * ntiles;
    const u32 *ik = keys_in, *iv = vals_in;
    for (int p = 0; p < passes; ++p) {
        const bool to_out = ((passes - 1 - p) % 2) == 0;
        u32 *ok = to_out ? keys_out : tk, *ov = to_out ? vals_out : tv;
        hipLaunchKernelGGL(radix_hist, dim3(ntiles), dim3(256), 0, s, ik, M, 8 * p, ntiles, hist, d_count, lowmask, inv_from);
        hipLaunchKernelGGL(radix_scan_rows, dim3(256), dim3(256), 0, s, hist, ntiles, totals);
        hipLaunchKernelGGL(radix_scan_totals, dim3(1), dim3(256), 0, s, totals);
        hipLaunchKernelGGL(lowmask == 0xffffffffu ? radix_scatter<true> : radix_scatter<false>, dim3(ntiles), dim3(256), 0, s, ik, iv, ok, ov, M,
                           8 * p, ntiles, hist, totals, d_count, lowmask, inv_from);
        ik = ok;
        iv = ov;
    }
    MG_HIP(hipGetLastError());
    return MG_OK;
}

}
```

rust/mantagpu-sys/src/lib.rs:

```rust
#![no_std]
#![allow(non_camel_case_types)]

use core::ffi::{c_char, c_float, c_int, c_uint, c_void};

pub type mg_curve_t = c_int;
pub const MG_BN254: mg_curve_t = 0;
pub const MG_BLS12_381: mg_curve_t = 1;

pub const MG_SUCCESS: c_int = 0;
pub const MG_ERROR_INVALID_ARGUMENT: c_int = 1;
pub const MG_ERROR_HIP: c_int = 2;
pub const MG_ERROR_OUT_OF_MEMORY: c_int = 3;
pub const MG_ERROR_DOMAIN_TOO_LARGE: c_int = 4;
pub const MG_ERROR_STATE: c_int = 5;
pub const MG_ERROR_CHECKSUM: c_int = 6;
pub const MG_R1CS_SATISFIED: u64 = u64::MAX;
pub const MG_TASK_A: c_uint = 1;
pub const MG_TASK_B_G1: c_uint = 2;
pub const MG_TASK_B_G2: c_uint = 4;
pub const MG_TASK_L: c_uint = 8;
pub const MG_TASK_H: c_uint = 16;

pub const MG_SCALARS_MONT: c_int = 1;
pub const MG_SCALARS_SPARSE: c_int = 2;
// ... 185 lines not shown
}

extern "C" {
    pub fn mg_init(device: c_int) -> c_int;
    pub fn mg_strerror(status: c_int) -> *const c_char;
    pub fn mg_last_error() -> *const c_char;
    pub fn mg_device_count(count: *mut c_int) -> c_int;
    pub fn mg_malloc(dptr: *mut *mut c_void, bytes: usize) -> c_int;
    pub fn mg_free(dptr: *mut c_void) -> c_int;
    pub fn mg_memcpy_h2d(dptr: *mut c_void, hptr: *const c_void, bytes: usize) -> c_int;
    pub fn mg_memcpy_d2h(hptr: *mut c_void, dptr: *const c_void, bytes: usize) -> c_int;
    pub fn mg_device_synchronize() -> c_int;
    pub fn mg_host_alloc(hptr: *mut *mut c_void, bytes: usize) -> c_int;
    pub fn mg_host_free(hptr: *mut c_void) -> c_int;
    pub fn mg_set_kernel_timing(on: c_int) -> c_int;
    pub fn mg_last_accumulate_ms() -> c_float;
    pub fn mg_last_accumulate_mhz() -> c_float;
    pub fn mg_clock_probe(iters: c_uint, memtime_mhz: *mut f64, mad_issue_per_us_per_simd: *mut f64, ms: *mut f64) -> c_int;
    pub fn mg_last_ntt_ms(out4: *mut c_float) -> c_int;
    pub fn mg_hw_queues(out2: *mut c_int) -> c_int;
    pub fn mg_last_prove_phases_ms(out10: *mut c_float) -> c_int;
    pub fn mg_last_pass_host_ms(out3: *mut c_float) -> c_int;

    pub fn mg_bases_create(
        curve: mg_curve_t,
        group: c_int,
        affine_mont: *const u64,
        n: usize,
        on_device: c_int,
        precompute_window_bits: c_int,
        out: *mut *mut mg_bases,
    ) -> c_int;
    pub fn mg_bases_create_sharded(
        curve: mg_curve_t,
        group: c_int,
        affine_mont: *const u64,
        n: usize,
        devices: *const c_int,
        n_devices: c_int,
        precompute_window_bits: c_int,
        out: *mut *mut mg_bases,
    ) -> c_int;
    pub fn mg_bases_num_shards(bases: *const mg_bases) -> c_int;
    pub fn mg_bases_shard(bases: *const mg_bases, shard: c_int, device: *mut c_int, lo: *mut usize, hi: *mut usize) -> c_int;
    pub fn mg_bases_destroy(bases: *mut mg_bases);
    pub fn mg_bases_device_bytes(bases: *const mg_bases) -> usize;
    pub fn mg_msm(bases: *const mg_bases, scalars_canonical: *const u64, n: usize, out_affine_mont: *mut u64) -> c_int;
    pub fn mg_msm_launch(
        bases: *const mg_bases,
        d_scalars: *const u64,
        n: usize,
        scalar_flags: c_int,
        window_bits: c_int,
        job: *mut *mut mg_msm_job,
    ) -> c_int;
    pub fn mg_msm_launch_sharded(
        bases: *const mg_bases,
        d_scalars_per_shard: *const *const u64,
        scalar_flags: c_int,
        window_bits: c_int,
        job: *mut *mut mg_msm_job,
    ) -> c_int;
    pub fn mg_msm_finish(job: *mut mg_msm_job, out_affine_mont: *mut u64) -> c_int;
    pub fn mg_msm_result_to_device(job: *mut mg_msm_job, d_out_xyzz: *mut u64, stream: *mut c_void) -> c_int;
    pub fn mg_xyzz_limbs(curve: mg_curve_t, group: c_int) -> usize;
    pub fn mg_xyzz_sum(curve: mg_curve_t, group: c_int, xyzz: *const u64, n: usize, out_affine_mont: *mut u64) -> c_int;
    pub fn mg_points_sum(curve: mg_curve_t, group: c_int, affine_mont: *const u64, n: usize, out_affine_mont: *mut u64) -> c_int;
    pub fn mg_fixed_base_mul(
        curve: mg_curve_t,
        group: c_int,
        base_affine_mont: *const u64,
        d_scalars: *const u64,
        n: usize,
        d_out_affine_mont: *mut u64,
    ) -> c_int;
    pub fn mg_ec_elementwise(
        curve: mg_curve_t,
        group: c_int,
        op: c_int,
        a_affine: *const u64,
        b: *const u64,
        n: usize,
        out_affine: *mut u64,
    ) -> c_int;
    pub fn mg_field_op(
        field: c_int,
        op: c_int,
        repr: c_int,
        lazy_a: c_int,
        lazy_b: c_int,
        a: *const u64,
        b: *const u64,
        n: usize,
        out: *mut u64,
    ) -> c_int;
    pub fn mg_fpr_raw_op(
        field: c_int,
        op: c_int,
        coding: c_int,
        a: *const u32,
        b: *const u32,
        c: *const u32,
        d: *const u32,
        n: usize,
        out: *mut u32,
    ) -> c_int;
    pub fn mg_pairing_op(
        curve: mg_curve_t,
        op: c_int,
        a: *const u32,
        b: *const u32,
        coeffs: *const i16,
        n: usize,
        out: *mut u32,
    ) -> c_int;
    pub fn mg_fpr_column_plan(
        field: c_int,
        kind: c_int,
        flush: *mut u32,
        peak: *mut u64,
        cols: *mut c_int,
        limb_bits: *mut c_int,
        flushed_routines: *mut c_int,
    ) -> c_int;
    pub fn mg_msm_digits(
        curve: mg_curve_t,
        scalars: *const u64,
        batch: usize,
        n_scalars: usize,
        scalar_flags: c_int,
        window_bits: c_int,
        table_mode: c_int,
        n: usize,
        map: *const u32,
        n_sets: usize,
        set_len: usize,
        compact: c_int,
        keys: *mut u32,
        vals: *mut u32,
        count: *mut u32,
        layout: *mut u32,
    ) -> c_int;
    pub fn mg_sort_pairs(
        keys: *const u32,
        vals: *const u32,
        n: usize,
        end_bit: c_int,
        count: *const u32,
        lowmask: u32,
        inv_from: u32,
        keys_out: *mut u32,
        vals_out: *mut u32,
    ) -> c_int;
    pub fn mg_group_ntt(
        curve: mg_curve_t,
        group: c_int,
        points_affine: *const u64,
        log_n: c_uint,
        inverse: c_int,
        out_affine: *mut u64,
    ) -> c_int;
    pub fn mg_point_serialize(curve: mg_curve_t, group: c_int, affine_mont: *const u64, compressed: c_int, out: *mut u8) -> c_int;

    pub fn mg_ntt(curve: mg_curve_t, data_mont: *mut u64, log_n: c_uint, inverse: c_int, coset: c_int) -> c_int;
    pub fn mg_ntt_device(curve: mg_curve_t, d_data_mont: *mut u64, log_n: c_uint, inverse: c_int, coset: c_int) -> c_int;

    pub fn mg_groth16_setup(
        curve: mg_curve_t,
        a: *const mg_csr,
        b: *const mg_csr,
        c: *const mg_csr,
        num_constraints: u64,
        n_vars: u64,
        n_inputs: u64,
        toxic_mont: *const u64,
        g1_generator: *const u64,
        g2_generator: *const u64,
        out: *const mg_pk_out,
    ) -> c_int;
    pub fn mg_qap_columns(
        curve: mg_curve_t,
        group: c_int,
        n_terms: usize,
        bases_affine: *const *const u64,
        mats: *const *const mg_csr,
        m: u64,
        n_cols: u64,
        entries_per_lane: u32,
        out_affine: *mut u64,
    ) -> c_int;
    pub fn mg_mpc_initialize(
        curve: mg_curve_t,
        powers: *const mg_kzg_view,
        a: *const mg_csr,
        b: *const mg_csr,
        c: *const mg_csr,
        num_constraints: u64,
        n_vars: u64,
        n_inputs: u64,
        h_len: u64,
        g1_generator: *const u64,
        g2_generator: *const u64,
        out: *const mg_pk_out,
    ) -> c_int;
    pub fn mg_ctx_create(curve: mg_curve_t, pk: *const mg_pk_view, out: *mut *mut mg_ctx) -> c_int;
    pub fn mg_tuning_init(t: *mut mg_tuning) -> c_int;
    pub fn mg_get_tuning(t: *mut mg_tuning) -> c_int;
    pub fn mg_set_tuning(t: *const mg_tuning) -> c_int;
    pub fn mg_tuning_env_names() -> *const *const c_char;
    pub fn mg_ctx_opts_init(opts: *mut mg_ctx_opts) -> c_int;
    pub fn mg_ctx_create_ex(curve: mg_curve_t, pk: *const mg_pk_view, opts: *const mg_ctx_opts, out: *mut *mut mg_ctx) -> c_int;
    pub fn mg_ctx_create_from_bytes_ex(
        curve: mg_curve_t,
        bytes: *const u8,
        len: usize,
        checksum32: *const u8,
        opts: *const mg_ctx_opts,
        out: *mut *mut mg_ctx,
    ) -> c_int;
    pub fn mg_ctx_create_sharded(
        curve: mg_curve_t,
        pk: *const mg_pk_view,
        devices: *const c_int,
        n_devices: c_int,
        out: *mut *mut mg_ctx,
    ) -> c_int;
    pub fn mg_ctx_create_shard(curve: mg_curve_t, pk: *const mg_pk_view, shard: c_int, n_shards: c_int, out: *mut *mut mg_ctx) -> c_int;
    pub fn mg_ctx_create_task(curve: mg_curve_t, pk: *const mg_pk_view, task_mask: c_uint, out: *mut *mut mg_ctx) -> c_int;
    pub fn mg_partials_slot_limbs(ctx: *const mg_ctx) -> usize;
    pub fn mg_groth16_partials_launch(
        ctx: *const mg_ctx,
        k: u64,
        z_mont: *const u64,
        d_out: *mut u64,
        stream: *mut c_void,
        job: *mut *mut mg_partials_job,
    ) -> c_int;
    pub fn mg_groth16_partials_finish(job: *mut mg_partials_job) -> c_int;
    pub fn mg_groth16_assemble(
        ctx: *const mg_ctx,
        k: u64,
        n_parts: c_int,
        parts: *const u64,
        r_mont: *const u64,
        s_mont: *const u64,
        proofs_out: *mut u8,
    ) -> c_int;
    pub fn mg_ctx_create_from_bytes(curve: mg_curve_t, bytes: *const u8, len: usize, out: *mut *mut mg_ctx) -> c_int;
    pub fn mg_ctx_create_from_bytes_checked(
        curve: mg_curve_t,
        bytes: *const u8,
        len: usize,
        checksum: *const u8,
        out: *mut *mut mg_ctx,
    ) -> c_int;
    pub fn mg_blake3(data: *const u8, len: usize, out32: *mut u8) -> c_int;
    pub fn mg_blake2s256(data: *const u8, len: usize, out32: *mut u8) -> c_int;
    pub fn mg_blake2s(data: *const u8, len: usize, out_len: usize, out: *mut u8) -> c_int;
    pub fn mg_aes256_gcm(
        key: *const u8,
        nonce: *const u8,
        input: *const u8,
        len: usize,
        decrypt: c_int,
        out: *mut u8,
        ok: *mut c_int,
    ) -> c_int;
    pub fn mg_ctx_create_from_bytes_sharded(
        curve: mg_curve_t,
        bytes: *const u8,
        len: usize,
        devices: *const c_int,
        n_devices: c_int,
        out: *mut *mut mg_ctx,
    ) -> c_int;
    pub fn mg_ctx_set_r1cs(ctx: *mut mg_ctx, a: *const mg_csr, b: *const mg_csr, c: *const mg_csr, num_constraints: u64) -> c_int;
    pub fn mg_groth16_prove(ctx: *const mg_ctx, z_mont: *const u64, r_mont: *const u64, s_mont: *const u64, proof_out: *mut u8) -> c_int;
    pub fn mg_groth16_prove_batch(
        ctx: *const mg_ctx,
        k: u64,
        z_mont: *const u64,
        r_mont: *const u64,
        s_mont: *const u64,
        proofs_out: *mut u8,
    ) -> c_int;
    pub fn mg_witness_map(ctx: *const mg_ctx, z_mont: *const u64, h_out_mont: *mut u64) -> c_int;
    pub fn mg_ctx_r1cs_check(ctx: *const mg_ctx, k: u64, z_mont: *const u64, first_unsatisfied: *mut u64, n_unsatisfied: *mut u64) -> c_int;
    pub fn mg_r1cs_check(
        curve: mg_curve_t,
        a: *const mg_csr,
        b: *const mg_csr,
        c: *const mg_csr,
        num_constraints: u64,
        n_vars: u64,
        k: u64,
        z_mont: *const u64,
        first_unsatisfied: *mut u64,
        n_unsatisfied: *mut u64,
    ) -> c_int;
    pub fn mg_ctx_domain_size(ctx: *const mg_ctx) -> u64;
    pub fn mg_ctx_table_bytes(ctx: *const mg_ctx, out2: *mut u64) -> c_int;
    pub fn mg_ctx_num_variables(ctx: *const mg_ctx) -> u64;
    pub fn mg_ctx_num_inputs(ctx: *const mg_ctx) -> u64;
    pub fn mg_ctx_num_shards(ctx: *const mg_ctx) -> c_int;
    pub fn mg_ctx_destroy(ctx: *mut mg_ctx);

// ... 284 lines not shown
```

Baseline: 478.8 Mscalar/s.

## Fuse scalar digit extraction into the first radix-sort pass for dense MSM

Adds a dense front end for single-batch, single-set MSM: a histogram kernel and a scatter kernel recompute signed window digits straight from the scalars. The first radix pass runs on those digits without first writing and re-reading the full keys/vals arrays. The scatter tile logic moves into a shared header so the sort and the new digit path can use it, and sort_pairs can now start at a later pass. This cuts one full round trip of W*n key/value pairs through HBM plus one sort pass. In exchange, scalar folding and digit decomposition are done twice, once in the histogram and once in the scatter.

```diff
diff --git a/include/mantagpu.h b/include/mantagpu.h
--- a/include/mantagpu.h
+++ b/include/mantagpu.h
@@ -96,6 +96,9 @@
                   uint32_t *vals, uint32_t *count, uint32_t layout[4]);
 int mg_sort_pairs(const uint32_t *keys, const uint32_t *vals, size_t n, int end_bit, const uint32_t *count, uint32_t lowmask,
                   uint32_t inv_from, uint32_t *keys_out, uint32_t *vals_out);
+int mg_msm_dense_front_applies(size_t batch, size_t n_sets, int windows, int table_mode, int sparse);
+int mg_msm_dense_front(mg_curve_t curve, const uint64_t *scalars, size_t n_scalars, int scalar_flags, int window_bits, size_t n,
+                       const uint32_t *map, size_t set_len, uint32_t *keys, uint32_t *vals, uint32_t layout[4]);
 int mg_group_ntt(mg_curve_t curve, int group, const uint64_t *points_affine, unsigned log_n, int inverse, uint64_t *out_affine);
 int mg_point_serialize(mg_curve_t curve, int group, const uint64_t *affine_mont, int compressed, uint8_t *out);
 
diff --git a/manta_rs_amd/api.py b/manta_rs_amd/api.py
--- a/manta_rs_amd/api.py
+++ b/manta_rs_amd/api.py
@@ -53,7 +53,7 @@
     "mg_init", "mg_strerror", "mg_last_error", "mg_device_count", "mg_malloc", "mg_free", "mg_memcpy_h2d",
     "mg_memcpy_d2h", "mg_device_synchronize", "mg_host_alloc", "mg_host_free", "mg_set_kernel_timing", "mg_last_accumulate_ms", "mg_bases_create", "mg_bases_destroy", "mg_bases_device_bytes",
     "mg_msm", "mg_msm_launch", "mg_msm_finish", "mg_points_sum", "mg_fixed_base_mul", "mg_ec_elementwise", "mg_point_serialize", "mg_ntt",
-    "mg_msm_digits", "mg_sort_pairs",
+    "mg_msm_digits", "mg_sort_pairs", "mg_msm_dense_front_applies", "mg_msm_dense_front",
     "mg_ntt_device", "mg_groth16_setup", "mg_ctx_create", "mg_ctx_create_from_bytes", "mg_ctx_set_r1cs", "mg_groth16_prove", "mg_groth16_prove_batch", "mg_witness_map", "mg_ctx_domain_size", "mg_ctx_table_bytes",
     "mg_ctx_destroy", "mg_bases_create_sharded", "mg_bases_num_shards", "mg_bases_shard", "mg_msm_launch_sharded",
     "mg_ctx_create_sharded", "mg_ctx_create_from_bytes_sharded", "mg_ctx_num_variables", "mg_ctx_num_inputs",
@@ -502,6 +502,24 @@
     assert layout[0] == W
     return dict(W=int(layout[0]), B=int(layout[1]), seg_keys=int(layout[2]), invalid=int(layout[3]), keys=k, vals=v,
                 count=int(count.value) if compact else None)
+
+
+def msm_dense_front_applies(batch, n_sets, windows, table_mode, sparse):
+    return bool(LIB.mg_msm_dense_front_applies(_sz(batch), _sz(n_sets), int(windows), int(table_mode), int(bool(sparse))))
+
+
+def msm_dense_front(curve, scalars, c, n, mont=False, map=None, set_len=None, keys=None, vals=None):
+    sc = _u64(scalars)
+    assert sc.ndim == 2 and sc.shape[1] == 4, sc.shape
+    bits = 254 if curve == BN254 else 255
+    W = (bits + c - 1) // c if c > 0 else 0
+    k, v = _u32_buffer(keys, W * n, "keys"), _u32_buffer(vals, W * n, "vals")
+    mp = None if map is None else np.ascontiguousarray(map, dtype=np.uint32)
+    assert mp is None or mp.shape == (n,), mp.shape
+    layout = (ctypes.c_uint32 * 4)()
+    _chk(LIB.mg_msm_dense_front(curve, _p(sc), _sz(sc.shape[0]), int(bool(mont)), int(c), _sz(n), _p(mp), _sz(n if set_len is None else set_len),
+                                _p(k), _p(v), layout), "mg_msm_dense_front")
+    return dict(W=int(layout[0]), B=int(layout[1]), seg_keys=int(layout[2]), inf_index=int(layout[3]), keys=k, vals=v)
 
 
 def sort_pairs(keys, vals, end_bit, count=None, lowmask=0xFFFFFFFF, inv_from=0xFFFFFFFF, keys_out=None, vals_out=None):
diff --git a/manta_rs_amd/csrc/capi.cpp b/manta_rs_amd/csrc/capi.cpp
--- a/manta_rs_amd/csrc/capi.cpp
+++ b/manta_rs_amd/csrc/capi.cpp
@@ -446,6 +446,21 @@
     return e->msm_digits(c);
     MG_CATCH
 }
+MG_API int mg_msm_dense_front_applies(size_t batch, size_t n_sets, int windows, int table_mode, int sparse) {
+    const size_t lim = (size_t)1 << 31;
+    return batch < lim && n_sets < lim && msm_dense_front_applies((u32)batch, (u32)n_sets, windows, table_mode, sparse != 0) ? 1 : 0;
+}
+MG_API int mg_msm_dense_front(mg_curve_t curve, const uint64_t *scalars, size_t n_scalars, int scalar_flags, int window_bits, size_t n,
+                              const uint32_t *map, size_t set_len, uint32_t *keys, uint32_t *vals, uint32_t layout[4]) {
+    MG_TRY
+    GroupEngine *e = get_engine((int)curve, 1);
+    const size_t lim = (size_t)1 << 31;
+    if (!e || n_scalars >= lim || n >= lim || set_len >= lim || (scalar_flags & ~MG_SCALARS_MONT)) return MG_ERROR_INVALID_ARGUMENT;
+    const MsmDigitsCall c{(const u32 *)scalars, 1u, (u32)n_scalars, (scalar_flags & MG_SCALARS_MONT) ? SCALARS_MONT : SCALARS_CANONICAL,
+                          window_bits, 1, (u32)n, map, 1u, (u32)set_len, false, keys, vals, nullptr, layout};
+    return e->msm_dense_front(c);
+    MG_CATCH
+}
 MG_API int mg_sort_pairs(const uint32_t *keys, const uint32_t *vals, size_t n, int end_bit, const uint32_t *count, uint32_t lowmask,
                          uint32_t inv_from, uint32_t *keys_out, uint32_t *vals_out) {
     MG_TRY
diff --git a/manta_rs_amd/csrc/engine.h b/manta_rs_amd/csrc/engine.h
--- a/manta_rs_amd/csrc/engine.h
+++ b/manta_rs_amd/csrc/engine.h
@@ -140,6 +140,7 @@
     u32 *d_map = nullptr;
     u32 *d_pts = nullptr;
     int pre_c = 0, pre_W = 0;
+    bool inf_record = false;
     bool full = false;
     u32 n_sets = 1;
     size_t set_len = 0;
@@ -194,6 +195,11 @@
     return ws->run_on ? ws->run_on : (ws->use_solo && ws->solo ? ws->solo : ws->stream);
 }
 
+constexpr int MSM_DENSE_MAX_WINDOWS = 16;
+inline bool msm_dense_front_applies(u32 batch, u32 n_sets, int windows, int table_mode, bool sparse) {
+    return batch == 1 && n_sets == 1 && table_mode == 1 && windows >= 1 && windows <= MSM_DENSE_MAX_WINDOWS && !sparse;
+}
+
 struct MsmDigitsCall {
     const u32 *scalars;
     u32 batch, n_scalars;
@@ -239,6 +245,7 @@
 
     virtual int msm_fold_device(MsmWorkspace *ws, u32 *d_out, size_t out_stride_words, hipStream_t on = nullptr) = 0;
     virtual int msm_digits(const MsmDigitsCall &c) = 0;
+    virtual int msm_dense_front(const MsmDigitsCall &c) = 0;
 
     virtual void hp_set_inf(HostPoint *p) const = 0;
     virtual void hp_from_affine(HostPoint *p, const u32 *affine_words) const = 0;
@@ -291,10 +298,15 @@
 GroupEngine *make_engine_bls381_g2();
 GroupEngine *get_engine(int curve, int group);
 
-size_t sort_pairs_temp_bytes(size_t n);
+struct SortScratch {
+    u32 *keys, *vals, *hist, *totals;
+};
+size_t sort_pairs_temp_bytes(size_t n, size_t tiles1 = 0);
+SortScratch sort_scratch(void *tmp, size_t n, size_t tiles1 = 0);
+void sort_scan_hist(const SortScratch &t, u32 ntiles, hipStream_t s);
 bool sort_pairs_takes_device_count(int end_bit);
 int sort_pairs(const u32 *keys_in, u32 *keys_out, const u32 *vals_in, u32 *vals_out, size_t n, int end_bit,
                void *tmp, size_t tmp_bytes, hipStream_t s, const u32 *d_count = nullptr, u32 lowmask = 0xffffffffu,
-               u32 inv_from = 0xffffffffu);
-
-}
+               u32 inv_from = 0xffffffffu, int first_pass = 0, size_t tiles1 = 0);
+
+}
diff --git a/manta_rs_amd/csrc/msm_digits.h b/manta_rs_amd/csrc/msm_digits.h
--- a/manta_rs_amd/csrc/msm_digits.h
+++ b/manta_rs_amd/csrc/msm_digits.h
@@ -1,7 +1,78 @@
 #pragma once
 #include "msm_common.h"
+#include "sort_scatter.h"
 
 namespace mg {
+
+template <class FrC, bool WORK = true>
+__device__ __forceinline__ void folded_scalar(const u32 *__restrict__ scalars, u32 src, bool have, int mont, u32 (&s)[8], u32 &flip) {
+#pragma unroll
+    for (int j = 0; j < 8; ++j) s[j] = 0;
+    if (WORK && have && mont == 2) {
+        typedef FpR<FrC> R;
+        const Fp<FrC> f = R::load(scalars + (size_t)src * R::K).to_canonical();
+#pragma unroll
+        for (int j = 0; j < 8; ++j) s[j] = f.v[j];
+    } else if (have) {
+        const uint4 *p = reinterpret_cast<const uint4 *>(scalars + (size_t)src * 8);
+        uint4 a = p[0], b = p[1];
+        s[0] = a.x, s[1] = a.y, s[2] = a.z, s[3] = a.w, s[4] = b.x, s[5] = b.y, s[6] = b.z, s[7] = b.w;
+        if (mont) {
+            Fp<FrC> f;
+#pragma unroll
+            for (int j = 0; j < 8; ++j) f.v[j] = s[j];
+            f = Fp<FrC>::from_mont(f);
+#pragma unroll
+            for (int j = 0; j < 8; ++j) s[j] = f.v[j];
+        }
+    }
+    for (int it = 0; it < 6; ++it) {
+        u32 t[8], bw = 0;
+#pragma unroll
+        for (int j = 0; j < 8; ++j) {
+            const u64 d = (u64)s[j] - FrC::P[j] - bw;
+            t[j] = (u32)d;
+            bw = (u32)(d >> 63);
+        }
+        if (!__any(!bw)) break;
+        if (!bw) {
+#pragma unroll
+            for (int j = 0; j < 8; ++j) s[j] = t[j];
+        }
+    }
+    flip = 0;
+    {
+        u32 t[8], bw = 0;
+#pragma unroll
+        for (int j = 0; j < 8; ++j) {
+            const u64 d = (u64)FrC::P[j] - s[j] - bw;
+            t[j] = (u32)d;
+            bw = (u32)(d >> 63);
+        }
+        bool lt = false;
+#pragma unroll
+        for (int j = 0; j < 8; ++j) lt = t[j] != s[j] ? t[j] < s[j] : lt;
+        if (!bw && lt) {
+            flip = 1;
+#pragma unroll
+            for (int j = 0; j < 8; ++j) s[j] = t[j];
+        }
+    }
+}
+struct DigitWalk {
+    int c;
+    u32 B, carry = 0;
+    __device__ __forceinline__ DigitWalk(int c_, u32 B_) : c(c_), B(B_) {}
+    __device__ __forceinline__ u32 next(u32 (&t)[8], u32 &neg) {
+        const u32 d = (t[0] & ((1u << c) - 1)) + carry;
+#pragma unroll
+        for (int j = 0; j < 7; ++j) t[j] = __funnelshift_r(t[j], t[j + 1], c);
+        t[7] >>= c;
+        neg = d > B;
+        carry = neg;
+        return neg ? (1u << c) - d : d;
+    }
+};
 
 template <class FrC>
 __global__ __launch_bounds__(1024) void digits_kernel(const u32 *__restrict__ scalars, u32 n, int c, int W, u32 B,
@@ -21,74 +92,17 @@
     }
     const u32 key0 = (blockIdx.y * n_sets + set) * seg_keys;
     const bool have = i < n && src < n_scalars;
-    u32 s[8] = {0, 0, 0, 0, 0, 0, 0, 0};
-    if (have && mont == 2) {
-        typedef FpR<FrC> R;
-        const Fp<FrC> f = R::load(scalars + (size_t)src * R::K).to_canonical();
-#pragma unroll
-        for (int j = 0; j < 8; ++j) s[j] = f.v[j];
-    } else if (have) {
-        const uint4 *p = reinterpret_cast<const uint4 *>(scalars + (size_t)src * 8);
-        uint4 a = p[0], b = p[1];
-        s[0] = a.x, s[1] = a.y, s[2] = a.z, s[3] = a.w, s[4] = b.x, s[5] = b.y, s[6] = b.z, s[7] = b.w;
-        if (mont) {
-            Fp<FrC> f;
-#pragma unroll
-            for (int j = 0; j < 8; ++j) f.v[j] = s[j];
-            f = Fp<FrC>::from_mont(f);
-#pragma unroll
-            for (int j = 0; j < 8; ++j) s[j] = f.v[j];
-        }
-    }
-    for (int it = 0; it < 6; ++it) {
-        u32 t[8], bw = 0;
-#pragma unroll
-        for (int j = 0; j < 8; ++j) {
-            const u64 d = (u64)s[j] - FrC::P[j] - bw;
-            t[j] = (u32)d;
-            bw = (u32)(d >> 63);
-        }
-        if (!__any(!bw)) break;
-        if (!bw) {
-#pragma unroll
-            for (int j = 0; j < 8; ++j) s[j] = t[j];
-        }
-    }
-    u32 flip = 0;
-    {
-        u32 t[8], bw = 0;
-#pragma unroll
-        for (int j = 0; j < 8; ++j) {
-            const u64 d = (u64)FrC::P[j] - s[j] - bw;
-            t[j] = (u32)d;
-            bw = (u32)(d >> 63);
-        }
-        bool lt = false;
-#pragma unroll
-        for (int j = 0; j < 8; ++j) lt = t[j] != s[j] ? t[j] < s[j] : lt;
-        if (!bw && lt) {
-            flip = 1;
-#pragma unroll
-            for (int j = 0; j < 8; ++j) s[j] = t[j];
-        }
-    }
-    const u32 mask = (1u << c) - 1;
-    auto next_digit = [&](u32 (&t)[8], u32 &carry, u32 &neg) -> u32 {
-        u32 d = (t[0] & mask) + carry;
-#pragma unroll
-        for (int j = 0; j < 7; ++j) t[j] = __funnelshift_r(t[j], t[j + 1], c);
-        t[7] >>= c;
-        neg = d > B;
-        carry = neg;
-        return neg ? (1u << c) - d : d;
-    };
+    u32 s[8];
+    u32 flip;
+    folded_scalar<FrC>(scalars, src, have, mont, s, flip);
+    DigitWalk walk(c, B);
+    u32 neg;
     if (!count) {
         if (i >= n) return;
         keys += (size_t)blockIdx.y * W * n;
         vals += (size_t)blockIdx.y * W * n;
-        u32 carry = 0, neg;
         for (int w = 0; w < W; ++w) {
-            const u32 d = next_digit(s, carry, neg);
+            const u32 d = walk.next(s, neg);
             const size_t o = (size_t)w * n + i;
             keys[o] = d ? key0 + (precomp == 2 ? 0u : precomp ? (d - 1) : ((u32)w * B + d - 1)) : invalid;
             vals[o] = d ? ((precomp == 2 ? ((u32)w * tstride + i) * B + (d - 1) : precomp ? ((u32)w * tstride + i) : i) | ((neg ^ flip) << 31)) : 0;
@@ -98,10 +112,11 @@
     const int lane = threadIdx.x & 63;
     u32 total = 0;
     {
-        u32 t[8], carry = 0, neg;
+        u32 t[8];
 #pragma unroll
         for (int j = 0; j < 8; ++j) t[j] = s[j];
-        for (int w = 0; w < W; ++w) total += (u32)__popcll(__ballot(next_digit(t, carry, neg) != 0));
+        DigitWalk count_walk(c, B);
+        for (int w = 0; w < W; ++w) total += (u32)__popcll(__ballot(count_walk.next(t, neg) != 0));
     }
     __shared__ u32 wave_tot[16], block_base;
     const int wv = threadIdx.x >> 6, nwv = blockDim.x >> 6;
@@ -116,9 +131,8 @@
     u32 base = block_base;
     for (int q = 0; q < wv; ++q) base += wave_tot[q];
     const unsigned long long lt = (1ull << lane) - 1ull;
-    u32 carry = 0, neg;
     for (int w = 0; w < W; ++w) {
-        const u32 d = next_digit(s, carry, neg);
+        const u32 d = walk.next(s, neg);
         const unsigned long long m = __ballot(d != 0);
         if (d) {
             const u32 o = base + (u32)__popcll(m & lt);
@@ -129,4 +143,67 @@
     }
 }
 
-}
+struct DenseFront {
+    const u32 *scalars, *map;
+    u32 n, n_scalars;
+    int c, W, mont;
+    u32 B, tstride, inf_index;
+};
+static_assert(MSM_DENSE_MAX_WINDOWS == SORT_ITEMS, "a lane's items are its scalar's windows");
+static constexpr u32 DIGIT_ZERO = 1u << 30, DIGIT_NEG = 1u << 31;
+template <class FrC, class Each> __device__ __forceinline__ bool dense_digit_words(const DenseFront &a, Each each) {
+    const u32 i = blockIdx.x * 256u + threadIdx.x;
+    const u32 src = i < a.n ? (a.map ? a.map[i] : i) : 0xffffffffu;
+    u32 s[8];
+    u32 flip;
+    folded_scalar<FrC, false>(a.scalars, src, i < a.n && src < a.n_scalars, a.mont, s, flip);
+    DigitWalk walk(a.c, a.B);
+#pragma unroll
+    for (int j = 0; j < SORT_ITEMS; ++j) {
+        if (j >= a.W) break;
+        u32 neg;
+        const u32 d = walk.next(s, neg);
+        each(j, d ? (d - 1) | ((neg ^ flip) << 31) : DIGIT_ZERO);
+    }
+    return i < a.n;
+}
+template <class FrC>
+__global__ __launch_bounds__(256) void digits_hist(DenseFront a, u32 ntiles, u32 *__restrict__ hist) {
+    MG_PRIO_HIGH();
+    __shared__ u32 cnt[256];
+    cnt[threadIdx.x] = 0;
+    __syncthreads();
+    const bool lane_valid = blockIdx.x * 256u + threadIdx.x < a.n;
+    dense_digit_words<FrC>(a, [&](int, u32 word) {
+        if (lane_valid) atomicAdd(&cnt[word & 255u], 1u);
+    });
+    __syncthreads();
+    hist[(size_t)threadIdx.x * ntiles + blockIdx.x] = cnt[threadIdx.x];
+}
+template <class FrC> struct DigitPairs {
+    const DenseFront &a;
+    u32 left, i;
+    __device__ __forceinline__ bool valid(int j) const { return i < a.n && j < a.W; }
+    __device__ __forceinline__ void keys(u32 (&k)[SORT_ITEMS]) const {
+#pragma unroll
+        for (int j = 0; j < SORT_ITEMS; ++j) k[j] = 0;
+        dense_digit_words<FrC>(a, [&](int j, u32 word) { k[j] = word; });
+    }
+    __device__ __forceinline__ void vals(u32 (&v)[SORT_ITEMS], const u32 (&k)[SORT_ITEMS]) const {
+#pragma unroll
+        for (int j = 0; j < SORT_ITEMS; ++j) v[j] = (k[j] & DIGIT_ZERO) ? a.inf_index : (((u32)j * a.tstride + i) | (k[j] & DIGIT_NEG));
+    }
+    __device__ __forceinline__ u32 digit(u32 word) const { return word & 255u; }
+    __device__ __forceinline__ u32 key(u32 word) const { return word & 0x00ffffffu; }
+};
+template <class FrC>
+__global__ __launch_bounds__(256) void digits_scatter(DenseFront a, u32 ntiles, const u32 *__restrict__ hist,
+                                                      const u32 *__restrict__ totals, u32 *__restrict__ keys_out,
+                                                      u32 *__restrict__ vals_out) {
+    MG_PRIO_HIGH();
+    const u32 first = blockIdx.x * 256u, lanes = a.n - first > 256u ? 256u : a.n - first;
+    const DigitPairs<FrC> in{a, lanes * (u32)a.W, first + threadIdx.x};
+    radix_scatter_tile(in, keys_out, vals_out, ntiles, hist, totals);
+}
+
+}
diff --git a/manta_rs_amd/csrc/msm_engine.h b/manta_rs_amd/csrc/msm_engine.h
--- a/manta_rs_amd/csrc/msm_engine.h
+++ b/manta_rs_amd/csrc/msm_engine.h
@@ -49,6 +49,7 @@
     int acc_single = ab_knob("MANTA_ACC_SINGLE", 1);
     u32 digits_threads = [](int v) { return (u32)(v == 256 || v == 512 || v == 1024 ? v : 256); }(ab_knob("MANTA_DIGITS_THREADS", 0));
     bool z3_sort = ab_knob("MANTA_Z3_SORT", 0) != 0;
+    bool dense_front = ab_knob_in("MANTA_DENSE_FRONT", 0, 1, 1) != 0;
 };
 static const MsmKnobs &msm_knobs() {
     static const MsmKnobs k;
@@ -117,8 +118,14 @@
         }
         const u32 FB = full ? 1u << (pre_c - 1) : 1u;
         if (full && (pre_c < 2 || pre_c > 12 || (size_t)W * n * FB >= ((size_t)1 << 31))) return MG_ERR_ARG;
-        bs->bytes = (size_t)W * n * FB * AWS * 4;
+        bs->inf_record = pre_c > 0 && !full;
+        if (bs->inf_record && (size_t)W * n + 1 >= ((size_t)1 << 31)) return MG_ERR_ARG;
+        bs->bytes = ((size_t)W * n * FB + (bs->inf_record ? 1u : 0u)) * AWS * 4;
         hipError_t e = hipMalloc((void **)&bs->d_pts, bs->bytes);
+        if (e == hipSuccess && bs->inf_record) {
+            const std::vector<u32> zero(AWS, 0u);
+            e = memcpy_sync(bs->d_pts + (size_t)W * n * AWS, zero.data(), (size_t)AWS * 4, hipMemcpyHostToDevice);
+        }
         u32 *&win_pts = guard.win_pts;
         if (e == hipSuccess && full) e = hipMalloc((void **)&win_pts, (size_t)W * n * AWS * 4);
         if (e != hipSuccess) return hip_failure(e, "hipMalloc(bases)", MG_ERR_OOM);
@@ -476,6 +483,46 @@
         const int rc = sync_status(s, e, "mg_msm_digits");
         bs.d_map = nullptr;
         return rc;
+    }
+
+    int msm_dense_front(const MsmDigitsCall &c) override {
+        if (!c.scalars || !c.keys || !c.vals || !c.layout || c.n == 0 || c.n_scalars == 0 || c.c < 1 || c.c > 24 || c.set_len == 0 ||
+            (c.scalar_mode != SCALARS_CANONICAL && c.scalar_mode != SCALARS_MONT) ||
+            !msm_dense_front_applies(c.batch, c.n_sets, windows_of(c.c), c.table_mode, c.compact))
+            return MG_ERR_ARG;
+        BaseSet bs;
+        bs.curve = CURVE_ID, bs.group = GROUP, bs.device = current_device();
+        bs.n = c.n, bs.n_orig = c.set_len, bs.set_len = c.set_len;
+        bs.pre_c = c.c, bs.pre_W = windows_of(c.c), bs.inf_record = true;
+        if (bs.n > bs.n_orig || (!c.map && bs.n != bs.n_orig) || c.n_scalars > bs.n_orig) return MG_ERR_ARG;
+        for (size_t i = 0; c.map && i < c.n; ++i)
+            if (c.map[i] >= bs.n_orig) return MG_ERR_ARG;
+        Launch r{&bs, nullptr, nullptr, nullptr, nullptr, c.n, c.n_scalars, 0, c.scalar_mode, 1, 1, false, false, plan_for(&bs, c.n, c.c, 1)};
+        if (const int rc = key_layout(r)) return rc;
+        r.end_bit = 1;
+        while (r.nb > 1 && (1u << r.end_bit) <= r.nb - 1) ++r.end_bit;
+        c.layout[0] = (u32)r.pl.W, c.layout[1] = r.pl.B, c.layout[2] = r.seg_keys, c.layout[3] = (u32)((size_t)r.pl.W * c.n);
+        hipStream_t s = r.s = setup_stream();
+        if (!s) return MG_ERR_OOM;
+        const size_t sb = (size_t)c.n_scalars * 32, pb = r.M * 4;
+        DevBlock m;
+        if (const int rc = m.alloc({sb, c.map ? (size_t)c.n * 4 : 0, pb, pb, sort_pairs_temp_bytes(r.M, cdiv(c.n, 256))}, "mg_msm_dense_front"))
+            return rc;
+        r.d_scalars = m.dev<u32>(0), bs.d_map = c.map ? m.dev<u32>(1) : nullptr;
+        hipError_t e = hipMemcpyAsync(m.dev(0), c.scalars, sb, hipMemcpyHostToDevice, s);
+        if (e == hipSuccess && c.map) e = hipMemcpyAsync(bs.d_map, c.map, (size_t)c.n * 4, hipMemcpyHostToDevice, s);
+        if (e == hipSuccess) e = hipMemcpyAsync(m.dev(2), c.keys, pb, hipMemcpyHostToDevice, s);
+        if (e == hipSuccess) e = hipMemcpyAsync(m.dev(3), c.vals, pb, hipMemcpyHostToDevice, s);
+        int rc = MG_OK;
+        if (e == hipSuccess) {
+            rc = enqueue_dense_front(r, m.dev(4), m.dev<u32>(2), m.dev<u32>(3));
+            e = hipGetLastError();
+        }
+        if (e == hipSuccess && !rc) e = hipMemcpyAsync(c.keys, m.dev(2), pb, hipMemcpyDeviceToHost, s);
+        if (e == hipSuccess && !rc) e = hipMemcpyAsync(c.vals, m.dev(3), pb, hipMemcpyDeviceToHost, s);
+        const int synced = sync_status(s, e, "mg_msm_dense_front");
+        bs.d_map = nullptr;
+        return rc ? rc : synced;
     }
 
     void scalar_one_mont(u64 out[4]) const override {
@@ -563,6 +610,7 @@
         int end_bit;
         u32 KB, seg_keys, nb, invalid, T, sort_mask = 0xffffffffu, sort_inv = 0xffffffffu;
         bool direct, per_query, acc_single;
+        bool dense;
         u32 *d_count;
         const u32 *skeys, *svals;
         u32 parts;
@@ -576,7 +624,7 @@
         r.M = r.n * (size_t)pl.W * r.batch;
         r.KB = pl.full ? 1u : pl.B;
         if (r.M >= (1ull << 31) || (size_t)r.batch * r.nsets * pl.Wb * r.KB >= (1ull << 24)) return MG_ERR_ARG;
-        if ((size_t)pl.W * r.bs->n * (pl.full ? pl.B : 1u) >= (1ull << 31)) return MG_ERR_ARG;
+        if ((size_t)pl.W * r.bs->n * (pl.full ? pl.B : 1u) + (pl.precomp && !pl.full ? 1u : 0u) >= (1ull << 31)) return MG_ERR_ARG;
         r.seg_keys = (u32)pl.Wb * r.KB;
         r.nb = r.batch * r.nsets * r.seg_keys;
         r.invalid = r.nb;
@@ -588,12 +636,19 @@
         int rc;
         if ((rc = key_layout(r))) return rc;
         const size_t M = r.M;
+        hipStreamCaptureStatus cst = hipStreamCaptureStatusNone;
+        const bool stand_alone = !ws->capturing && !ws->run_on && !ws->in_graph_slot &&
+                                 hipStreamIsCapturing(r.s, &cst) == hipSuccess && cst == hipStreamCaptureStatusNone;
+        r.dense = msm_knobs().dense_front && stand_alone && r.bs->inf_record && r.scalar_mode != SCALARS_WORK &&
+                  msm_dense_front_applies(r.batch, r.nsets, pl.W, pl.full ? 2 : (pl.precomp ? 1 : 0), r.sparse);
         if (pl.full) r.sparse = true;
         const u32 seg_keys = r.seg_keys, nb = r.nb, invalid = r.invalid;
-        if ((rc = ws->keys_in.reserve(M * 4)) || (rc = ws->keys_out.reserve(M * 4)) ||
-            (rc = ws->vals_in.reserve(M * 4)) || (rc = ws->vals_out.reserve(M * 4)))
+        if ((rc = ws->keys_out.reserve(M * 4)) || (rc = ws->vals_out.reserve(M * 4)) ||
+            (!r.dense && ((rc = ws->keys_in.reserve(M * 4)) || (rc = ws->vals_in.reserve(M * 4)))))
             return rc;
-        if ((rc = ws->sort_tmp.reserve(sort_pairs_temp_bytes(M))) || (rc = ws->buckets.reserve((size_t)(nb + 1) * XW * 4))) return rc;
+        if ((rc = ws->sort_tmp.reserve(sort_pairs_temp_bytes(M, r.dense ? cdiv(r.n, 256) : 0))) ||
+            (rc = ws->buckets.reserve((size_t)(nb + 1) * XW * 4)))
+            return rc;
         const u32 T = r.T = cdiv(M, pl.L);
         if ((rc = ws->pkeys[0].reserve((size_t)2 * T * 4)) || (rc = ws->ppts[0].reserve((size_t)2 * T * XW * 4)))
             return rc;
@@ -606,8 +661,8 @@
         while ((1u << end_bit) <= invalid) ++end_bit;
         int end_bit_real = 1;
         while (nb > 1 && (1u << end_bit_real) <= nb - 1) ++end_bit_real;
-        if ((end_bit + 7) / 8 > (end_bit_real + 7) / 8) r.sparse = true;
-        if (r.sparse) end_bit = end_bit_real;
+        if ((end_bit + 7) / 8 > (end_bit_real + 7) / 8 && !r.dense) r.sparse = true;
+        if (r.sparse || r.dense) end_bit = end_bit_real;
         if (msm_knobs().sort_low && !r.sparse && r.batch > 1 && r.nsets == 1 && (seg_keys & (seg_keys - 1)) == 0) {
             int eb = 1;
             while ((1u << eb) <= seg_keys) ++eb;
@@ -639,7 +694,7 @@
         zr.p[2] = ws->timed ? (u32 *)ws->h_clk : nullptr, zr.n[2] = ws->timed ? 4u : 0u;
         const u32 most = zr.n[1] > 4u ? zr.n[1] : 4u;
         hipLaunchKernelGGL((zero_ranges<F>), dim3(most > 256u * 1024u ? 1024u : cdiv(most, 256)), dim3(256), 0, s, zr);
-        enqueue_digits(r, ws->keys_in.as<u32>(), ws->vals_in.as<u32>());
+        if (!r.dense) enqueue_digits(r, ws->keys_in.as<u32>(), ws->vals_in.as<u32>());
         r.batch *= r.nsets;
     }
     static void enqueue_digits(Launch &r, u32 *keys, u32 *vals) {
@@ -664,8 +719,27 @@
                                r.scalar_stride_words, r.seg_keys, r.d_count, nsets, (u32)bs->set_len);
     }
 
+    static int enqueue_dense_front(const Launch &r, void *sort_tmp, u32 *keys_out, u32 *vals_out) {
+        const MsmPlan &pl = r.pl; const BaseSet *const bs = r.bs; hipStream_t s = r.s;
+        const u32 tiles1 = cdiv(r.n, 256);
+        const SortScratch t = sort_scratch(sort_tmp, r.M, tiles1);
+        const DenseFront a{r.d_scalars, bs->d_map, (u32)r.n, (u32)r.n_scalars, pl.c, pl.W, r.scalar_mode,
+                           pl.B, (u32)bs->n, (u32)((size_t)pl.W * bs->n)};
+        const bool to_out = ((r.end_bit + 7) / 8 - 1) % 2 == 0;
+        hipLaunchKernelGGL((digits_hist<FrC>), dim3(tiles1), dim3(256), 0, s, a, tiles1, t.hist);
+        sort_scan_hist(t, tiles1, s);
+        u32 *const k0 = to_out ? keys_out : t.keys, *const v0 = to_out ? vals_out : t.vals;
+        hipLaunchKernelGGL((digits_scatter<FrC>), dim3(tiles1), dim3(256), 0, s, a, tiles1, (const u32 *)t.hist, (const u32 *)t.totals, k0, v0);
+        return sort_pairs(k0, keys_out, v0, vals_out, r.M, r.end_bit, sort_tmp, sort_pairs_temp_bytes(r.M, tiles1), s, nullptr,
+                          0xffffffffu, 0xffffffffu, 1, tiles1);
+    }
+
     int launch_sort(Launch &r) {
         MsmWorkspace *const ws = r.ws;
+        if (r.dense) {
+            r.skeys = ws->keys_out.as<u32>(), r.svals = ws->vals_out.as<u32>();
+            return enqueue_dense_front(r, ws->sort_tmp.p, ws->keys_out.as<u32>(), ws->vals_out.as<u32>());
+        }
         const bool no_sort = (r.nb == 1 || r.per_query) && r.d_count;
         r.skeys = no_sort ? ws->keys_in.as<u32>() : ws->keys_out.as<u32>();
         r.svals = no_sort ? ws->vals_in.as<u32>() : ws->vals_out.as<u32>();
diff --git a/manta_rs_amd/csrc/sort.hip b/manta_rs_amd/csrc/sort.hip
--- a/manta_rs_amd/csrc/sort.hip
+++ b/manta_rs_amd/csrc/sort.hip
@@ -1,14 +1,8 @@
-#include "engine.h"
+#include "sort_scatter.h"
+#include <algorithm>
 #include <cstdlib>
 
 namespace mg {
-
-static constexpr int SORT_TILE = 4096;
-static constexpr int SORT_ITEMS = 16;
-
-__device__ __forceinline__ u32 sort_key(u32 k, u32 lowmask, u32 inv_from) {
-    return (k >= inv_from && lowmask != 0xffffffffu) ? lowmask + 1u : (k & lowmask);
-}
 
 __global__ __launch_bounds__(256) void radix_hist(const u32 *__restrict__ keys, u32 M, int shift, u32 ntiles,
                                                   u32 *__restrict__ hist, const u32 *__restrict__ count, u32 lowmask, u32 inv_from) {
@@ -70,10 +64,6 @@
     totals[threadIdx.x] = part[threadIdx.x] - mine;
 }
 
-#ifndef MG_SCATTER_MASKS
-#define MG_SCATTER_MASKS 1
-#endif
-
 template <bool IDENT>
 __global__ __launch_bounds__(256) void radix_scatter(const u32 *__restrict__ keys_in, const u32 *__restrict__ vals_in,
                                                      u32 *__restrict__ keys_out, u32 *__restrict__ vals_out, u32 M,
@@ -83,152 +73,45 @@
     MG_PRIO_HIGH();
     if (count) M = *count;
     if ((size_t)blockIdx.x * SORT_TILE >= M) return;
-    __shared__ u32 wcount[4][256];
-    __shared__ u32 gbase[256];
-    typedef unsigned long long __attribute__((may_alias)) lane_mask;
-    __shared__ __attribute__((aligned(8))) u32 tile[2 * SORT_TILE];
-    u32 *const sk = tile, *const sv = tile + SORT_TILE;
-    lane_mask *const masks = (lane_mask *)tile;
-    constexpr int HALF = SORT_ITEMS / 2;
-    const int wave = threadIdx.x >> 6, lane = threadIdx.x & 63;
-    const auto digit = [&](u32 key) { return ((IDENT ? key : sort_key(key, lowmask, inv_from)) >> shift) & 255u; };
-#pragma unroll
-    for (int w = 0; w < 4; ++w) {
-        wcount[w][threadIdx.x] = 0;
-        if (MG_SCATTER_MASKS) masks[w * 256 + threadIdx.x] = 0;
-    }
-    __syncthreads();
+    const u32 wave = threadIdx.x >> 6, lane = threadIdx.x & 63;
     const u32 tile0 = blockIdx.x * (u32)SORT_TILE;
-    const u32 base = tile0 + (u32)wave * (SORT_ITEMS * 64) + (u32)lane;
-    const u32 left = M - tile0 > (u32)SORT_TILE ? (u32)SORT_TILE : M - tile0;
-    const u32 mine = (u32)wave * (SORT_ITEMS * 64) + (u32)lane;
-    u32 k[SORT_ITEMS], rk2[HALF];
-#pragma unroll
-    for (int j = 0; j < SORT_ITEMS; ++j) {
-        const bool valid = mine + (u32)j * 64 < left;
-        k[j] = valid ? keys_in[(size_t)base + (size_t)j * 64] : 0u;
-    }
-#if MG_SCATTER_MASKS
-    lane_mask *const wmask = masks + wave * 256;
-    const unsigned long long lane_bit = 1ull << lane;
-    unsigned long long none = 0;
-    asm volatile("" : "+v"(none));
-#pragma unroll
-    for (int j = 0; j < SORT_ITEMS; ++j) {
-        const bool valid = mine + (u32)j * 64 < left;
-        const u32 d = digit(k[j]);
-        if (valid) __hip_atomic_fetch_or(&wmask[d], lane_bit, __ATOMIC_RELAXED, __HIP_MEMORY_SCOPE_WAVEFRONT);
-        __builtin_amdgcn_fence(__ATOMIC_ACQ_REL, "wavefront");
-        __builtin_amdgcn_wave_barrier();
-        const unsigned long long peers = __hip_atomic_load(&wmask[d], __ATOMIC_RELAXED, __HIP_MEMORY_SCOPE_WAVEFRONT);
-        const u32 before = wcount[wave][d];
-        const u32 lo = (u32)peers, hi = (u32)(peers >> 32);
-        const u32 rank = __builtin_amdgcn_mbcnt_hi(hi, __builtin_amdgcn_mbcnt_lo(lo, before));
-        const bool first = valid && rank == before;
-        if (j & 1)
-            rk2[j >> 1] |= rank << 16;
-        else
-            rk2[j >> 1] = rank;
-        asm volatile("" : "+v"(rk2[j >> 1]));
-        __builtin_amdgcn_fence(__ATOMIC_ACQ_REL, "wavefront");
-        __builtin_amdgcn_wave_barrier();
-        if (first) {
-            wcount[wave][d] = (u32)__builtin_popcount(hi) + ((u32)__builtin_popcount(lo) + before);
-            __hip_atomic_store(&wmask[d], none, __ATOMIC_RELAXED, __HIP_MEMORY_SCOPE_WAVEFRONT);
-        }
-        __builtin_amdgcn_fence(__ATOMIC_ACQ_REL, "wavefront");
-        __builtin_amdgcn_wave_barrier();
-    }
-#else
-    const unsigned long long lt_mask = (1ull << lane) - 1ull;
-#pragma unroll
-    for (int j = 0; j < SORT_ITEMS; ++j) {
-        const bool valid = mine + (u32)j * 64 < left;
-        const u32 d = digit(k[j]);
-        unsigned long long peers = __ballot(valid);
-#pragma unroll
-        for (int b = 0; b < 8; ++b) {
-            const bool bit = (d >> b) & 1u;
-            const unsigned long long bb = __ballot(bit);
-            peers &= bit ? bb : ~bb;
-        }
-        const u32 before = wcount[wave][d];
-        const u32 r = (u32)__popcll(peers & lt_mask);
-        if (j & 1)
-            rk2[j >> 1] |= (before + r) << 16;
-        else
-            rk2[j >> 1] = before + r;
-        asm volatile("" : "+v"(rk2[j >> 1]));
-        if (valid && r == 0) wcount[wave][d] = before + (u32)__popcll(peers);
-    }
-#endif
-#pragma unroll
-    for (int j = 0; j < SORT_ITEMS; ++j) asm volatile("" : "+v"(k[j]));
-    u32 v[SORT_ITEMS];
-#pragma unroll
-    for (int j = 0; j < SORT_ITEMS; ++j) v[j] = mine + (u32)j * 64 < left ? vals_in[(size_t)base + (size_t)j * 64] : 0u;
-    __syncthreads();
-    {
-        const u32 d = threadIdx.x;
-        const u32 c0 = wcount[0][d], c1 = wcount[1][d], c2 = wcount[2][d], c3 = wcount[3][d];
-        const u32 tot = c0 + c1 + c2 + c3;
-        gbase[d] = tot;
-        __syncthreads();
-        for (int s = 1; s < 256; s <<= 1) {
-            const u32 x = d >= (u32)s ? gbase[d - s] : 0;
-            __syncthreads();
-            gbase[d] += x;
-            __syncthreads();
-        }
-        const u32 loc = gbase[d] - tot;
-        __syncthreads();
-        wcount[0][d] = loc;
-        wcount[1][d] = loc + c0;
-        wcount[2][d] = loc + c0 + c1;
-        wcount[3][d] = loc + c0 + c1 + c2;
-        gbase[d] = hist[(size_t)d * ntiles + blockIdx.x] + totals[d] - loc;
-    }
-    __syncthreads();
-#pragma unroll
-    for (int j = 0; j < SORT_ITEMS; ++j) {
-        if (mine + (u32)j * 64 < left) {
-            const u32 rank = (j & 1) ? rk2[j >> 1] >> 16 : rk2[j >> 1] & 0xffffu;
-            const u32 lp = wcount[wave][digit(k[j])] + rank;
-            sk[lp] = k[j];
-            sv[lp] = v[j];
-        }
-    }
-    __syncthreads();
-    for (u32 t = threadIdx.x; t < left; t += 256) {
-        const u32 kk = sk[t];
-        const u32 pos = gbase[digit(kk)] + t;
-        keys_out[pos] = kk;
-        vals_out[pos] = sv[t];
-    }
+    const u32 mine = wave * (SORT_ITEMS * 64) + lane;
+    const LoadedPairs in{keys_in, vals_in, M - tile0 > (u32)SORT_TILE ? (u32)SORT_TILE : M - tile0, mine, (size_t)tile0 + mine, shift, lowmask,
+                         inv_from, IDENT};
+    radix_scatter_tile(in, keys_out, vals_out, ntiles, hist, totals);
 }
 
-size_t sort_pairs_temp_bytes(size_t n) {
-    const size_t ntiles = (n + SORT_TILE - 1) / SORT_TILE;
-    return 2 * n * 4  + 256 * ntiles * 4 + 256 * 4 + 256;
+static size_t hist_columns(size_t n, size_t tiles1) { return std::max((n + SORT_TILE - 1) / SORT_TILE, tiles1); }
+size_t sort_pairs_temp_bytes(size_t n, size_t tiles1) {
+    return 2 * n * 4  + 256 * hist_columns(n, tiles1) * 4 + 256 * 4 + 256;
+}
+SortScratch sort_scratch(void *tmp, size_t n, size_t tiles1) {
+    u32 *const tk = (u32 *)tmp, *const hist = tk + 2 * n;
+    return SortScratch{tk, tk + n, hist, hist + (size_t)256 * hist_columns(n, tiles1)};
+}
+void sort_scan_hist(const SortScratch &t, u32 ntiles, hipStream_t s) {
+    hipLaunchKernelGGL(radix_scan_rows, dim3(256), dim3(256), 0, s, t.hist, ntiles, t.totals);
+    hipLaunchKernelGGL(radix_scan_totals, dim3(1), dim3(256), 0, s, t.totals);
 }
 
 bool sort_pairs_takes_device_count(int end_bit) { return end_bit >= 1 && end_bit <= 32; }
 
 int sort_pairs(const u32 *keys_in, u32 *keys_out, const u32 *vals_in, u32 *vals_out, size_t n, int end_bit,
-               void *tmp, size_t tmp_bytes, hipStream_t s, const u32 *d_count, u32 lowmask, u32 inv_from) {
+               void *tmp, size_t tmp_bytes, hipStream_t s, const u32 *d_count, u32 lowmask, u32 inv_from, int first_pass,
+               size_t tiles1) {
     if (n == 0) return MG_OK;
-    if (end_bit < 1 || end_bit > 32 || n >= (1ull << 32) || tmp_bytes < sort_pairs_temp_bytes(n)) return MG_ERR_ARG;
+    if (end_bit < 1 || end_bit > 32 || n >= (1ull << 32) || tmp_bytes < sort_pairs_temp_bytes(n, tiles1) || first_pass < 0) return MG_ERR_ARG;
     const u32 M = (u32)n;
     const u32 ntiles = (u32)((n + SORT_TILE - 1) / SORT_TILE);
     const int passes = (end_bit + 7) / 8;
-    u32 *tk = (u32 *)tmp, *tv = tk + n, *hist = tv + n, *totals = hist + (size_t)256 * ntiles;
+    const SortScratch t = sort_scratch(tmp, n, tiles1);
+    u32 *const tk = t.keys, *const tv = t.vals, *const hist = t.hist, *const totals = t.totals;
     const u32 *ik = keys_in, *iv = vals_in;
-    for (int p = 0; p < passes; ++p) {
+    for (int p = first_pass; p < passes; ++p) {
         const bool to_out = ((passes - 1 - p) % 2) == 0;
         u32 *ok = to_out ? keys_out : tk, *ov = to_out ? vals_out : tv;
         hipLaunchKernelGGL(radix_hist, dim3(ntiles), dim3(256), 0, s, ik, M, 8 * p, ntiles, hist, d_count, lowmask, inv_from);
-        hipLaunchKernelGGL(radix_scan_rows, dim3(256), dim3(256), 0, s, hist, ntiles, totals);
-        hipLaunchKernelGGL(radix_scan_totals, dim3(1), dim3(256), 0, s, totals);
+        sort_scan_hist(t, ntiles, s);
         hipLaunchKernelGGL(lowmask == 0xffffffffu ? radix_scatter<true> : radix_scatter<false>, dim3(ntiles), dim3(256), 0, s, ik, iv, ok, ov, M,
                            8 * p, ntiles, hist, totals, d_count, lowmask, inv_from);
         ik = ok;
diff --git a/manta_rs_amd/csrc/sort_scatter.h b/manta_rs_amd/csrc/sort_scatter.h
--- /dev/null
+++ b/manta_rs_amd/csrc/sort_scatter.h
@@ -0,0 +1,155 @@
+#pragma once
+#include "engine.h"
+
+namespace mg {
+
+static constexpr int SORT_TILE = 4096;
+static constexpr int SORT_ITEMS = 16;
+
+__device__ __forceinline__ u32 sort_key(u32 k, u32 lowmask, u32 inv_from) {
+    return (k >= inv_from && lowmask != 0xffffffffu) ? lowmask + 1u : (k & lowmask);
+}
+
+#ifndef MG_SCATTER_MASKS
+#define MG_SCATTER_MASKS 1
+#endif
+
+struct LoadedPairs {
+    const u32 *__restrict__ keys_in, *__restrict__ vals_in;
+    u32 left, mine;
+    size_t base;
+    int shift;
+    u32 lowmask, inv_from;
+    bool ident;
+    __device__ __forceinline__ bool valid(int j) const { return mine + (u32)j * 64 < left; }
+    __device__ __forceinline__ void keys(u32 (&k)[SORT_ITEMS]) const {
+#pragma unroll
+        for (int j = 0; j < SORT_ITEMS; ++j) k[j] = valid(j) ? keys_in[base + (size_t)j * 64] : 0u;
+    }
+    __device__ __forceinline__ void vals(u32 (&v)[SORT_ITEMS], const u32 (&)[SORT_ITEMS]) const {
+#pragma unroll
+        for (int j = 0; j < SORT_ITEMS; ++j) v[j] = valid(j) ? vals_in[base + (size_t)j * 64] : 0u;
+    }
+    __device__ __forceinline__ u32 digit(u32 word) const { return ((ident ? word : sort_key(word, lowmask, inv_from)) >> shift) & 255u; }
+    __device__ __forceinline__ u32 key(u32 word) const { return word; }
+};
+
+template <class Pairs>
+__device__ __forceinline__ void radix_scatter_tile(const Pairs &in, u32 *__restrict__ keys_out, u32 *__restrict__ vals_out, u32 ntiles,
+                                                   const u32 *__restrict__ hist, const u32 *__restrict__ totals) {
+    __shared__ u32 wcount[4][256];
+    __shared__ u32 gbase[256];
+    typedef unsigned long long __attribute__((may_alias)) lane_mask;
+    __shared__ __attribute__((aligned(8))) u32 tile[2 * SORT_TILE];
+    u32 *const sk = tile, *const sv = tile + SORT_TILE;
+    lane_mask *const masks = (lane_mask *)tile;
+    constexpr int HALF = SORT_ITEMS / 2;
+    const int wave = threadIdx.x >> 6, lane = threadIdx.x & 63;
+#pragma unroll
+    for (int w = 0; w < 4; ++w) {
+        wcount[w][threadIdx.x] = 0;
+        if (MG_SCATTER_MASKS) masks[w * 256 + threadIdx.x] = 0;
+    }
+    __syncthreads();
+    const u32 left = in.left;
+    u32 k[SORT_ITEMS], rk2[HALF];
+    in.keys(k);
+#if MG_SCATTER_MASKS
+    lane_mask *const wmask = masks + wave * 256;
+    const unsigned long long lane_bit = 1ull << lane;
+    unsigned long long none = 0;
+    asm volatile("" : "+v"(none));
+#pragma unroll
+    for (int j = 0; j < SORT_ITEMS; ++j) {
+        const bool valid = in.valid(j);
+        const u32 d = in.digit(k[j]);
+        if (valid) __hip_atomic_fetch_or(&wmask[d], lane_bit, __ATOMIC_RELAXED, __HIP_MEMORY_SCOPE_WAVEFRONT);
+        __builtin_amdgcn_fence(__ATOMIC_ACQ_REL, "wavefront");
+        __builtin_amdgcn_wave_barrier();
+        const unsigned long long peers = __hip_atomic_load(&wmask[d], __ATOMIC_RELAXED, __HIP_MEMORY_SCOPE_WAVEFRONT);
+        const u32 before = wcount[wave][d];
+        const u32 lo = (u32)peers, hi = (u32)(peers >> 32);
+        const u32 rank = __builtin_amdgcn_mbcnt_hi(hi, __builtin_amdgcn_mbcnt_lo(lo, before));
+        const bool first = valid && rank == before;
+        if (j & 1)
+            rk2[j >> 1] |= rank << 16;
+        else
+            rk2[j >> 1] = rank;
+        asm volatile("" : "+v"(rk2[j >> 1]));
+        __builtin_amdgcn_fence(__ATOMIC_ACQ_REL, "wavefront");
+        __builtin_amdgcn_wave_barrier();
+        if (first) {
+            wcount[wave][d] = (u32)__builtin_popcount(hi) + ((u32)__builtin_popcount(lo) + before);
+            __hip_atomic_store(&wmask[d], none, __ATOMIC_RELAXED, __HIP_MEMORY_SCOPE_WAVEFRONT);
+        }
+        __builtin_amdgcn_fence(__ATOMIC_ACQ_REL, "wavefront");
+        __builtin_amdgcn_wave_barrier();
+    }
+#else
+    const unsigned long long lt_mask = (1ull << lane) - 1ull;
+#pragma unroll
+    for (int j = 0; j < SORT_ITEMS; ++j) {
+        const bool valid = in.valid(j);
+        const u32 d = in.digit(k[j]);
+        unsigned long long peers = __ballot(valid);
+#pragma unroll
+        for (int b = 0; b < 8; ++b) {
+            const bool bit = (d >> b) & 1u;
+            const unsigned long long bb = __ballot(bit);
+            peers &= bit ? bb : ~bb;
+        }
+        const u32 before = wcount[wave][d];
+        const u32 r = (u32)__popcll(peers & lt_mask);
+        if (j & 1)
+            rk2[j >> 1] |= (before + r) << 16;
+        else
+            rk2[j >> 1] = before + r;
+        asm volatile("" : "+v"(rk2[j >> 1]));
+        if (valid && r == 0) wcount[wave][d] = before + (u32)__popcll(peers);
+    }
+#endif
+#pragma unroll
+    for (int j = 0; j < SORT_ITEMS; ++j) asm volatile("" : "+v"(k[j]));
+    u32 v[SORT_ITEMS];
+    in.vals(v, k);
+    __syncthreads();
+    {
+        const u32 d = threadIdx.x;
+        const u32 c0 = wcount[0][d], c1 = wcount[1][d], c2 = wcount[2][d], c3 = wcount[3][d];
+        const u32 tot = c0 + c1 + c2 + c3;
+        gbase[d] = tot;
+        __syncthreads();
+        for (int s = 1; s < 256; s <<= 1) {
+            const u32 x = d >= (u32)s ? gbase[d - s] : 0;
+            __syncthreads();
+            gbase[d] += x;
+            __syncthreads();
+        }
+        const u32 loc = gbase[d] - tot;
+        __syncthreads();
+        wcount[0][d] = loc;
+        wcount[1][d] = loc + c0;
+        wcount[2][d] = loc + c0 + c1;
+        wcount[3][d] = loc + c0 + c1 + c2;
+        gbase[d] = hist[(size_t)d * ntiles + blockIdx.x] + totals[d] - loc;
+    }
+    __syncthreads();
+#pragma unroll
+    for (int j = 0; j < SORT_ITEMS; ++j) {
+        if (in.valid(j)) {
+            const u32 rank = (j & 1) ? rk2[j >> 1] >> 16 : rk2[j >> 1] & 0xffffu;
+            const u32 lp = wcount[wave][in.digit(k[j])] + rank;
+            sk[lp] = in.key(k[j]);
+            sv[lp] = v[j];
+        }
+    }
+    __syncthreads();
+    for (u32 t = threadIdx.x; t < left; t += 256) {
+        const u32 kk = sk[t];
+        const u32 pos = gbase[in.digit(kk)] + t;
+        keys_out[pos] = kk;
+        vals_out[pos] = sv[t];
+    }
+}
+
+}
diff --git a/rust/mantagpu-sys/src/lib.rs b/rust/mantagpu-sys/src/lib.rs
--- a/rust/mantagpu-sys/src/lib.rs
+++ b/rust/mantagpu-sys/src/lib.rs
@@ -361,6 +361,20 @@
         keys_out: *mut u32,
         vals_out: *mut u32,
     ) -> c_int;
+    pub fn mg_msm_dense_front_applies(batch: usize, n_sets: usize, windows: c_int, table_mode: c_int, sparse: c_int) -> c_int;
+    pub fn mg_msm_dense_front(
+        curve: mg_curve_t,
+        scalars: *const u64,
+        n_scalars: usize,
+        scalar_flags: c_int,
+        window_bits: c_int,
+        n: usize,
+        map: *const u32,
+        set_len: usize,
+        keys: *mut u32,
+        vals: *mut u32,
+        layout: *mut u32,
+    ) -> c_int;
     pub fn mg_group_ntt(
         curve: mg_curve_t,
         group: c_int,
```

Result: faster. 485.4 Mscalar/s, median of 6 (+1.4%).
